# DeepakSridhar/fgdm

Hardware: AMD Instinct MI355X
Metric: 512x512 images/sec @ 50 DDIM steps, seg-ControlNet+CFG (higher is better)
Workload: dtype f16

## Files before the change

fgdm_amd/csrc/common.h:

```cpp
#pragma once
#include <hip/hip_runtime.h>
#include <stdint.h>

typedef _Float16 half_t;
typedef _Float16 h8 __attribute__((ext_vector_type(8)));
typedef _Float16 h4 __attribute__((ext_vector_type(4)));
typedef _Float16 h2 __attribute__((ext_vector_type(2)));
typedef float f32x16 __attribute__((ext_vector_type(16)));
typedef float f32x4 __attribute__((ext_vector_type(4)));

__device__ __forceinline__ float gelu_f(float x) {
    const float z = fminf(fabsf(x), 6.0f);
    float p = -4.7132482596e-04f;
    p = __builtin_fmaf(p, z, 7.0652551839e-03f);
    p = __builtin_fmaf(p, z, -5.1762067461e-02f);
    p = __builtin_fmaf(p, z, -4.6008771426e-01f);
    p = __builtin_fmaf(p, z, -1.1507295505e+00f);
    p = __builtin_fmaf(p, z, -4.8959157159e-05f - 1.0f);
    const float t = __builtin_amdgcn_exp2f(p);
    return __builtin_fmaf(fabsf(x), 0.5f - t, 0.5f * x);
}

typedef float f32x2 __attribute__((ext_vector_type(2)));
__device__ __forceinline__ f32x2 gelu2_f(f32x2 x) {
    const f32x2 ax = {fabsf(x[0]), fabsf(x[1])};
    const f32x2 z = {fminf(ax[0], 6.0f), fminf(ax[1], 6.0f)};
    auto c = [](float k) { return f32x2{k, k}; };
    f32x2 p = c(-4.7132482596e-04f);
    p = __builtin_elementwise_fma(p, z, c(7.0652551839e-03f));
    p = __builtin_elementwise_fma(p, z, c(-5.1762067461e-02f));
    p = __builtin_elementwise_fma(p, z, c(-4.6008771426e-01f));
    p = __builtin_elementwise_fma(p, z, c(-1.1507295505e+00f));
    p = __builtin_elementwise_fma(p, z, c(-4.8959157159e-05f - 1.0f));
    const f32x2 t = {__builtin_amdgcn_exp2f(p[0]), __builtin_amdgcn_exp2f(p[1])};
    return __builtin_elementwise_fma(ax, c(0.5f) - t, c(0.5f) * x);
}

__device__ __forceinline__ float silu_f(float x, float k = 1.0f) {
    return x * __builtin_amdgcn_rcpf(1.0f + __builtin_amdgcn_exp2f(-1.4426950408889634f * k * x));
}

#define FGDM_OK 0
#define FGDM_ERR_ARG -1
#define FGDM_ERR_HIP -2
#define FGDM_ERR_STATE -3
#define FGDM_ERR_NOMEM -4

enum IgemmMode { IG_LINEAR = 0, IG_CONV3 = 1, IG_CONV3_S2 = 2, IG_CONV3_UP2 = 3, IG_CONV3_S2_BR = 4 };
enum IgemmAct { ACT_NONE = 0, ACT_SILU = 1, ACT_RELU = 2, ACT_GEGLU = 3, ACT_QGELU = 4  };
enum IgemmOut { OUT_F16 = 0, OUT_F32 = 1, OUT_F32_NCHW = 2, OUT_F16_T = 3 };

struct IgemmArgs {
    const half_t* A0;
    const half_t* A1;
    const half_t* Wt;
    const float* bias;
    const float* rowvec;
    const half_t* resid;
    void* out;
    const half_t* zero;
    int C0, C1;
    int B, H, W;
    int Ho, Wo;
    int M, N;
    int K;
    int mode, act, out_kind;
    int ld_out, ld_res;
    int rv_stride;
    int rows_per_sample;
    float scale;
    int force_cfg;
    int splitk;
    float* ws;
    int debug;
    const float* ln_stats;
    const float* ln_u;
    int ln_slots;
    float ln_eps;
    float* stats_out;
    void* out2;
    int split_n, out_kind2, ld_out2;
};

int igemm_launch(const IgemmArgs& a, hipStream_t s);
void igemm_set_force_cfg(int cfg);
void igemm_set_twin_layers(bool on);
void igemm_set_pair_hint(int mult);
int igemm2_launch(const IgemmArgs& a, int cfg, hipStream_t s);
int igemm_stats_slots(const IgemmArgs& a);
int row_stats_slots(int C);
int row_stats_launch(const half_t* x, int rows, int C, float* stats , hipStream_t s);
int igemm_splitk_factor(const IgemmArgs& a);
int igemm_splitk_reduce(const IgemmArgs& a, hipStream_t s);
size_t igemm_npad(int n);

#define GN_PIX_PER_CHUNK 256
void groupnorm_set_group(bool on);
int groupnorm_launch(const half_t* x0, int C0, const half_t* x1, int C1, int B, int HW,
                     const float* gamma, const float* beta, float eps, int silu,
                     half_t* out, float* ws , hipStream_t s);
size_t groupnorm_ws_floats(int B, int HW);
int layernorm_launch(const half_t* x, int rows, int C, const float* gamma, const float* beta, float eps,
                     half_t* out, hipStream_t s);

int attention_launch(const half_t* Q, int ldq, const half_t* K, int ldk, const half_t* Vt, int ldvt,
                     half_t* O, int ldo, int B, int H, int T, int Tk, int d, int q_prescaled, hipStream_t s);
int attention_last_kernel();

int nchw_f32_to_nhwc_f16(const float* x, half_t* y, int B, int C, int HW, int Cpad, hipStream_t s);
int pack_xcat(const float* x, const half_t* cc, half_t* y, int B, int Bc, int Cc, int HW, int Cpad, hipStream_t s);
int f32_to_f16(const float* x, half_t* y, size_t n, hipStream_t s);
int silu_f32_to_f16(const float* x, half_t* y, size_t n, hipStream_t s);
int nhwc_f16_to_nchw_f32(const half_t* x, float* y, int B, int C, int HW, hipStream_t s);
int im2col3x3(const half_t* x, half_t* A, int B, int H, int W, int C, int stride, int Kpad, hipStream_t s);
int avgpool2(const half_t* x, half_t* y, int B, int H, int W, int C, hipStream_t s);
int add_f16(const half_t* a, const half_t* b, half_t* y, size_t n, hipStream_t s);
int add_f16_to_f32(const float* a, const half_t* b, float* y, size_t n, hipStream_t s);
int timestep_embed(const int64_t* t, const float* t_float, half_t* y, int B, int dim, int rows_pad, hipStream_t s);
int vae_prequant(const float* z, const float* wb, float scale, half_t* y, int B, int HW, hipStream_t s);
int vae_moments(const float* h, const float* wb, float* moments, int B, int HW, hipStream_t s);
int posterior_sample(const float* moments, const float* noise, float scale, float* z, int B, int zc, int HW, hipStream_t s);
int softmax_rows(const float* S, half_t* P, int rows, int cols, hipStream_t s);
int image_to_u8(const float* x, uint8_t* y, int B, int C, int HW, int mode, hipStream_t s);
int resize_linear_u8(const uint8_t* src, uint8_t* dst, int B, int H, int W, int C, int Ho, int Wo, hipStream_t s);
int u8_to_hint(const uint8_t* src, float* dst, int B, int HW, int C, hipStream_t s);
int embed_tokens(const int64_t* ids, const float* tok, const float* pos, float* out, int rows, int T, int W, int vocab,
                 hipStream_t s);
int layernorm32_launch(const float* x, int rows, int C, const float* gamma, const float* beta, float eps, half_t* out16,
                       float* out32, hipStream_t s);
int f16_to_f32(const half_t* x, float* y, size_t n, hipStream_t s);
int small_attention_launch(const half_t* qkv, int ld, int koff, int voff, half_t* out, int ldo, int B, int heads, int T,
                           int d, int causal, hipStream_t s);
int transpose_pad_keys(const half_t* v, half_t* vt, int B, int Tk, int C, int Tkpad, hipStream_t s);
int ddim_step(const float* x, const float* e_cond, const float* e_uncond, float cfg_scale,
              float a_t, float a_prev, float sigma_t, float sqrt_one_minus_at, const float* noise,
              float* x_prev, float* pred_x0, float* e_out, size_t n, hipStream_t s);
int plms_combine(const float* e_t, const float* e1, const float* e2, const float* e3, int order,
                 float* e_prime, size_t n, hipStream_t s);
int axpby(const float* a, float ca, const float* b, float cb, float* y, size_t n, hipStream_t s);
int mask_blend(const float* a, const float* b, const float* m, float* y, size_t n, hipStream_t s);
int ancestral_step(const float* x, const float* eps, float sqrt_recip, float sqrt_recipm1, float coef1, float coef2,
                   float std, const float* noise, float* out, size_t n, hipStream_t s);

struct PatchGeom { int B, C, H, W, kh, kw, sh, sw, Ly, Lx; };
int patch_plan(int H, int W, int kh, int kw, int sh, int sw, bool must_cover, int* Ly, int* Lx);
int unfold_crops(const float* x, float* out , const PatchGeom& g, int l0, int n, hipStream_t s);
int fold_accumulate(const float* o, const float* w_pix, const float* w_tie, float* acc, const PatchGeom& g, int l0, int n,
                    hipStream_t s);
int fold_finish(const float* acc, const float* w_pix, const float* w_tie, float* out, const PatchGeom& g, hipStream_t s);
int repeat_words(const void* src, void* dst , size_t words , int reps, hipStream_t s);

#define HIP_TRY(expr) do { hipError_t _e = (expr); if (_e != hipSuccess) return FGDM_ERR_HIP; } while (0)

template <auto Kernel>
int fgdm_dyn_lds(int bytes) {
    constexpr int MAXDEV = 64;
    static bool set[MAXDEV] = {};
    int dev = -1;
    if (hipGetDevice(&dev) != hipSuccess || dev < 0 || dev >= MAXDEV) return FGDM_ERR_HIP;
    if (!set[dev]) {
        HIP_TRY(hipFuncSetAttribute((const void*)Kernel, hipFuncAttributeMaxDynamicSharedMemorySize, bytes));
        set[dev] = true;
    }
    return FGDM_OK;
}

#include <functional>
#define FGDM_MAX_GROUP 5
bool fgdm_recording();
void fgdm_record(std::function<int(hipStream_t)> run);
#define FGDM_GROUP_BLOB sizeof(IgemmArgs)
typedef int (*FgdmGroupFn)(const void* const* args, int n, unsigned grid_x, hipStream_t s);
void fgdm_record(std::function<int(hipStream_t)> run, const void* key, FgdmGroupFn group, const void* args, size_t nbytes,
                 unsigned grid_x, unsigned long long shape);
#define FGDM_LAUNCH(kernel, grid, block, smem, stream, ...)                                                                  \
    do {                                                                                                                     \
        if (fgdm_recording()) {                                                                                              \
// ... 9 lines not shown
```

fgdm_amd/csrc/engine.hip:

```cpp
#include "engine_shared.h"
#include "knobs.h"
#include "replay.h"

#include <algorithm>
#include <array>
#include <cmath>
#include <cstdlib>
#include <cstdio>
#include <cstring>
#include <map>
#include <memory>
#include <string>
#include <unordered_map>
#include <vector>

namespace {

struct Arena {
    struct Blk { char* p; size_t sz; bool free; };
    std::vector<std::vector<Blk>> slabs;
    std::vector<char*> bases;
    size_t slab_bytes = (size_t)4 << 30;
    size_t in_use = 0, peak = 0;
    bool scoped = false;
    std::vector<void*> live;
    void begin_scope() { scoped = true; live.clear(); }
    void end_scope(bool failed) {
        if (failed) { std::vector<void*> l; l.swap(live); scoped = false; for (void* p : l) release(p); }
        scoped = false;
        live.clear();
    }

    ~Arena() { for (char* b : bases) (void)hipFree(b); }
    void* alloc(size_t bytes) {
        bytes = (bytes + 255) & ~(size_t)255;
        if (bytes == 0) bytes = 256;
        for (auto& s : slabs)
            for (size_t i = 0; i < s.size(); ++i)
                if (s[i].free && s[i].sz >= bytes) {
                    if (s[i].sz > bytes) {
                        Blk rest{s[i].p + bytes, s[i].sz - bytes, true};
                        s[i].sz = bytes;
                        s.insert(s.begin() + i + 1, rest);
                    }
                    s[i].free = false;
                    in_use += bytes;
                    peak = std::max(peak, in_use);
                    if (scoped) live.push_back(s[i].p);
                    return s[i].p;
                }
        const size_t sz = std::max(slab_bytes, bytes);
        char* base = nullptr;
        if (hipMalloc(&base, sz) != hipSuccess) return nullptr;
        bases.push_back(base);
        slabs.push_back({Blk{base, sz, true}});
        return alloc(bytes);
    }
    void release(void* p) {
        if (!p) return;
        if (scoped) { auto it = std::find(live.begin(), live.end(), p); if (it != live.end()) { *it = live.back(); live.pop_back(); } }
        for (auto& s : slabs)
            for (size_t i = 0; i < s.size(); ++i)
                if (s[i].p == p && !s[i].free) {
                    s[i].free = true;
                    in_use -= s[i].sz;
                    if (i + 1 < s.size() && s[i + 1].free) { s[i].sz += s[i + 1].sz; s.erase(s.begin() + i + 1); }
                    if (i > 0 && s[i - 1].free) { s[i - 1].sz += s[i].sz; s.erase(s.begin() + i); }
                    return;
                }
    }
};

struct Tensor {
    half_t* p = nullptr;
    int B = 0, H = 0, W = 0, C = 0;
    size_t numel() const { return (size_t)B * H * W * C; }
    int rows() const { return B * H * W; }
};

struct ParamSlot {
    std::vector<int64_t> shape;
    std::vector<float> host;
    bool loaded = false;
    size_t numel() const { size_t n = 1; for (auto d : shape) n *= (size_t)d; return n; }
};

struct GemmW {
    half_t* w = nullptr;
    float* bias = nullptr;
    int N = 0, K = 0;
    bool im2col = false;
    int cin_pad = 0;
    int k_real = 0;
    float* ln_u = nullptr;
    float ln_eps = 1e-5f;
};
struct NormW { float* g = nullptr; float* b = nullptr; int C = 0; };

enum LType { L_CONV, L_RES, L_ATTN, L_DOWN, L_UP };
struct Layer {
    LType type = L_CONV;
    int cin = 0, cout = 0, heads = 0;
    bool down = false;
    std::string pre;
    GemmW conv;
    NormW gn1, gn2; GemmW c1, c2, skip; int emb_off = 0;
    NormW gn, ln1, ln2, ln3;
    GemmW pin, pout, qkv1, o1, q2, k2, v2, o2, ffp, ffo;
};
typedef std::vector<Layer> Block;

struct AdapterBlk { int ic = 0, oc = 0; bool down = false; std::string pre; GemmW in_conv, b1, b2; };

struct Net {
    std::string prefix;
    bool control = false;
    GemmW time0, time2, emb_all;
    int emb_total = 0;
    std::vector<Block> input, output;
    Block middle;
    NormW out_gn; GemmW out_conv;
    bool has_adapter = false;
    GemmW ad_conv_in; std::vector<AdapterBlk> ad_body;
    std::vector<GemmW> xad_conv_in; std::vector<std::vector<AdapterBlk>> xad_body;
    Tensor xad_sum[4]; bool xad_valid = false;
    bool time_adapter = false; Block tad_body;
    std::vector<GemmW> zero_convs; GemmW mid_out;
    std::vector<int> zero_ch;
    GemmW hint_convs[8];
    Tensor guided;
};

struct VRes { int cin = 0, cout = 0; std::string pre; NormW n1, n2; GemmW c1, c2, nin; };
struct VLevel { std::vector<VRes> blocks; bool up = false; std::string up_pre; GemmW upconv; };
struct VAttn { std::string pre; NormW norm; GemmW q, k, v, o; };
struct VDown { std::vector<VRes> blocks; bool down = false; std::string down_pre; GemmW downconv; };
struct VEnc {
    bool on = false;
    GemmW conv_in, conv_out;
    std::vector<VDown> levels;
    VRes mid1, mid2;
    VAttn attn;
    NormW norm_out;
    float* qc = nullptr;
};
struct Vae {
    bool on = false, packed = false;
    std::string prefix;
    int top = 0, factor = 1;
    GemmW conv_in, conv_out;
    VRes mid1, mid2;
    VAttn attn;
    std::vector<VLevel> levels;
    NormW norm_out;
    float* pq = nullptr;
    VEnc enc;
};

struct ClipLayer { std::string pre; NormW ln1, ln2; GemmW qkv, o, fc1, fc2; };
struct Clip {
    bool on = false, packed = false;
    std::string prefix;
    float* tok = nullptr;
    float* pos = nullptr;
    std::vector<ClipLayer> layers;
    NormW final_ln;
};

enum ProfClass { PC_IGEMM = 0, PC_ATTN = 1, PC_NORM = 2, PC_ELEM = 3, PC_COUNT = 4 };
struct Prof final : LaunchTimer {
    bool on = false;
    std::vector<hipEvent_t> pool;
    size_t used = 0;
    struct Rec { int cls; size_t e0, e1; double w; char tag[56]; };
    std::vector<Rec> recs;
    double work[PC_COUNT] = {0, 0, 0, 0};
    double bytes[PC_COUNT] = {0, 0, 0, 0};
    hipEvent_t get() {
        if (used == pool.size()) { hipEvent_t e; if (hipEventCreate(&e) != hipSuccess) return nullptr; pool.push_back(e); }
        return pool[used++];
    }
    int stride = 1;
    long counter = 0;
    bool armed = false;
    void begin(int cls, hipStream_t s, double w, const char* tag = "", double nbytes = 0.0) override {
        if (fgdm_recording()) {
            if (on) fgdm_record_bracket_begin(cls, w, nbytes, tag);
            return;
        }
        armed = false;
        if (!on || (counter++ % stride) != 0) return;
        armed = true;
        hipEvent_t e = get();
        if (!e) return;
        (void)hipEventRecord(e, s);
        Rec r{cls, used - 1, 0, w, {0}};
        snprintf(r.tag, sizeof(r.tag), "%s", tag);
        recs.push_back(r);
        work[cls] += w;
        bytes[cls] += nbytes;
    }
    void end(hipStream_t s) override {
        if (fgdm_recording()) {
            if (on) fgdm_record_bracket_end();
            return;
        }
        if (!on || !armed || recs.empty()) return;
        armed = false;
        hipEvent_t e = get();
        if (!e) return;
        (void)hipEventRecord(e, s);
        recs.back().e1 = used - 1;
    }
};

}

#define CHK0(x) do { int _rc0 = (x); if (_rc0 != FGDM_OK) return _rc0; } while (0)
struct fgdm_engine {
    fgdm_config cfg{};
    int device = -1;
    bool device_ready = false, finalized = false;
    std::string err;
    std::vector<std::string> order;
    std::unordered_map<std::string, ParamSlot> params;
    Net unet;
    std::vector<Net> cns;
    Vae vae;
    Clip clip;
    struct CtxKV { Tensor k, vt; };
    std::unordered_map<const Layer*, CtxKV> ctx_cache;
    int ctx_B = 0, ctx_T = 0;
    int ctx_tokens = 77;
    Tensor ccat;
    Arena arena;
    half_t* zero = nullptr;
    std::unordered_map<std::string, std::vector<void*>> weight_allocs;
    std::unordered_map<std::string, bool> comp_dirty, comp_packed;
    std::string cur_comp;
    bool ln_fold = true;
    hipStream_t s = nullptr;
    std::vector<std::unique_ptr<Arena>> cn_arena;
    Arena* ar = &arena;
    hipStream_t s2 = nullptr;
    hipEvent_t ev_fork = nullptr, ev_join = nullptr;
    bool twin_streams = false;
    bool pair_launch = true;
    int group_max = FGDM_MAX_GROUP;
    bool gn_group = true;
    ReplayStats replay_stats;
    struct Deferred { const GemmW* w; Tensor src; int idx; float scale; Arena* owner; };
    Prof prof;

    int fail(int code, const std::string& m) { err = m; return code; }

    void reg(const std::string& name, std::vector<int64_t> shape) {
        order.push_back(name);
        params[name].shape = std::move(shape);
    }
    void reg_wb(const std::string& pre, std::vector<int64_t> wshape) {
        const int64_t n = wshape[0];
        reg(pre + ".weight", std::move(wshape));
        reg(pre + ".bias", {n});
    }
    void reg_res(const std::string& p, int cin, int cout, int temb) {
        reg_wb(p + "in_layers.0", {cin});
        reg_wb(p + "in_layers.2", {cout, cin, 3, 3});
        reg_wb(p + "emb_layers.1", {cout, temb});
        reg_wb(p + "out_layers.0", {cout});
        reg_wb(p + "out_layers.3", {cout, cout, 3, 3});
        if (cin != cout) reg_wb(p + "skip_connection", {cout, cin, 1, 1});
    }
    void reg_attn(const std::string& p, int ch, int ctx) {
        reg_wb(p + "norm", {ch});
        reg_wb(p + "proj_in", {ch, ch, 1, 1});
        const std::string t = p + "transformer_blocks.0.";
        reg(t + "attn1.to_q.weight", {ch, ch});
        reg(t + "attn1.to_k.weight", {ch, ch});
        reg(t + "attn1.to_v.weight", {ch, ch});
        reg_wb(t + "attn1.to_out.0", {ch, ch});
        reg_wb(t + "ff.net.0.proj", {8 * ch, ch});
        reg_wb(t + "ff.net.2", {ch, 4 * ch});
        reg(t + "attn2.to_q.weight", {ch, ch});
        reg(t + "attn2.to_k.weight", {ch, ctx});
        reg(t + "attn2.to_v.weight", {ch, ctx});
        reg_wb(t + "attn2.to_out.0", {ch, ch});
        reg_wb(t + "norm1", {ch});
        reg_wb(t + "norm2", {ch});
        reg_wb(t + "norm3", {ch});
        reg_wb(p + "proj_out", {ch, ch, 1, 1});
    }
    void reg_block(const std::string& pre, Block& blk, int temb, int ctx) {
        for (size_t j = 0; j < blk.size(); ++j) {
            Layer& l = blk[j];
            l.pre = pre + std::to_string(j) + ".";
            switch (l.type) {
                case L_CONV: reg_wb(l.pre.substr(0, l.pre.size() - 1), {l.cout, l.cin, 3, 3}); break;
                case L_RES: reg_res(l.pre, l.cin, l.cout, temb); break;
                case L_ATTN: reg_attn(l.pre, l.cin, ctx); break;
                case L_DOWN: reg_wb(l.pre + "op", {l.cin, l.cin, 3, 3}); break;
                case L_UP: reg_wb(l.pre + "conv", {l.cin, l.cin, 3, 3}); break;
            }
        }
    }
    static Layer mk(LType t, int cin, int cout, int heads = 0) {
        Layer l; l.type = t; l.cin = cin; l.cout = cout; l.heads = heads; return l;
    }
    bool in_ares(int ds) const {
        for (int i = 0; i < cfg.n_attention_resolutions; ++i) if (cfg.attention_resolutions[i] == ds) return true;
        return false;
    }
    void build_net(Net& n, const std::string& prefix, bool control, int adapter_kind) {
        const bool adapter = adapter_kind == 1;
        n.prefix = prefix; n.control = control; n.has_adapter = adapter_kind != 0; n.time_adapter = adapter_kind == 2;
        const int mc = cfg.model_channels, temb = 4 * mc, ctx = cfg.context_dim, heads = cfg.num_heads;
        reg_wb(prefix + "time_embed.0", {temb, mc});
        reg_wb(prefix + "time_embed.2", {temb, temb});
        if (adapter) {
            static const int chs[4] = {320, 640, 1280, 1280};
            const std::string ap = prefix + "adapter.";
            for (int i = 0; i < 4; ++i)
                for (int j = 0; j < 2; ++j) {
                    AdapterBlk b;
// ... 268 lines not shown
        if (rc != FGDM_OK) return rc;
        comp_packed[comp] = true;
        comp_dirty[comp] = false;
        return FGDM_OK;
    }
    int pack_rows(GemmW& g, const std::vector<std::pair<const float*, int>>& srcs, int K_src, int K,
                  const std::vector<int>& kmap, const std::vector<const float*>& biases, bool geglu,
                  const std::vector<float>& src_scale = {}, const float* ln_gamma = nullptr, const float* ln_beta = nullptr) {
        int N = 0;
        for (auto& s : srcs) N += s.second;
        const size_t npad = igemm_npad(N);
        std::vector<half_t> w(npad * (size_t)K, (half_t)0);
        std::vector<float> bias(npad, 0.f), lnu(ln_gamma ? npad : 0, 0.f);
        std::vector<const float*> rowp(N);
        std::vector<float> bflat(N, 0.f), rscale(N, 1.f);
        int r = 0;
        for (size_t si = 0; si < srcs.size(); ++si)
            for (int i = 0; i < srcs[si].second; ++i, ++r) {
                rowp[r] = srcs[si].first + (size_t)i * K_src;
                if (si < biases.size() && biases[si]) bflat[r] = biases[si][i];
                if (si < src_scale.size()) rscale[r] = src_scale[si];
            }
        for (int pr = 0; pr < N; ++pr) {
            int sr = pr;
            if (geglu) {
                const int grp = pr >> 6, within = pr & 63;
                sr = within < 32 ? grp * 32 + within : N / 2 + grp * 32 + (within - 32);
            }
            const float* src = rowp[sr];
            const float rs = rscale[sr];
            half_t* dst = w.data() + (size_t)pr * K;
            if (ln_gamma) {
                double us = 0.0, cs = 0.0;
                for (int k = 0; k < K; ++k) {
                    dst[k] = (half_t)(src[k] * rs * ln_gamma[k]);
                    us += (double)(float)dst[k];
                    cs += (double)ln_beta[k] * (double)(src[k] * rs);
                }
                lnu[pr] = (float)us;
                bias[pr] = (float)((double)(bflat[sr] * rs) + cs);
                continue;
            }
            if (kmap.empty()) for (int k = 0; k < K; ++k) dst[k] = (half_t)(src[k] * rs);
            else for (int k = 0; k < K; ++k) if (kmap[k] >= 0) dst[k] = (half_t)(src[kmap[k]] * rs);
            bias[pr] = bflat[sr] * rs;
        }
        g.N = N; g.K = K; g.k_real = K_src;
        g.w = upload(w);
        g.bias = upload(bias);
        g.ln_u = ln_gamma ? upload(lnu) : nullptr;
        if (ln_gamma && !kmap.empty()) return fail(FGDM_ERR_ARG, "LayerNorm fold: plain Linear weights only");
        return (g.w && g.bias && (!ln_gamma || g.ln_u)) ? FGDM_OK : fail(FGDM_ERR_NOMEM, "hipMalloc failed while packing weights");
    }
    int pack_linear(GemmW& g, const std::string& pre, bool has_bias, bool geglu = false, float wscale = 1.f,
                    const std::string& ln = std::string()) {
        const ParamSlot* w = slot(pre + ".weight");
        if (!w) return FGDM_ERR_STATE;
        const ParamSlot *lg = nullptr, *lb = nullptr;
        if (!ln.empty()) { lg = slot(ln + ".weight"); lb = slot(ln + ".bias"); if (!lg || !lb) return FGDM_ERR_STATE; }
        const ParamSlot* b = has_bias ? slot(pre + ".bias") : nullptr;
        if (has_bias && !b) return FGDM_ERR_STATE;
        const int N = (int)w->shape[0], K = (int)(w->numel() / w->shape[0]);
        if (K & 63) return fail(FGDM_ERR_ARG, "linear K not a multiple of 64: " + pre);
        if (lg && (int)lg->numel() != K) return fail(FGDM_ERR_ARG, "LayerNorm fold: width mismatch for " + pre);
        return pack_rows(g, {{w->host.data(), N}}, K, K, {}, {b ? b->host.data() : nullptr}, geglu, {wscale},
                         lg ? lg->host.data() : nullptr, lb ? lb->host.data() : nullptr);
    }
    int pack_stack(GemmW& g, const std::vector<std::string>& pres, bool has_bias, const std::vector<float>& scales = {},
                   const std::string& ln = std::string()) {
        const ParamSlot *lg = nullptr, *lb = nullptr;
        if (!ln.empty()) { lg = slot(ln + ".weight"); lb = slot(ln + ".bias"); if (!lg || !lb) return FGDM_ERR_STATE; }
        std::vector<std::pair<const float*, int>> srcs;
        std::vector<const float*> biases;
        int K = 0;
        for (auto& pre : pres) {
            const ParamSlot* w = slot(pre + ".weight");
            if (!w) return FGDM_ERR_STATE;
            K = (int)(w->numel() / w->shape[0]);
            srcs.push_back({w->host.data(), (int)w->shape[0]});
            if (has_bias) { const ParamSlot* b = slot(pre + ".bias"); if (!b) return FGDM_ERR_STATE; biases.push_back(b->host.data()); }
        }
        return pack_rows(g, srcs, K, K, {}, biases, false, scales, lg ? lg->host.data() : nullptr, lb ? lb->host.data() : nullptr);
    }
    int pack_conv3(GemmW& g, const std::string& pre) {
        const ParamSlot* w = slot(pre + ".weight");
        const ParamSlot* b = slot(pre + ".bias");
        if (!w || !b) return FGDM_ERR_STATE;
        const int N = (int)w->shape[0], Cin = (int)w->shape[1];
        int cp = 0;
        const std::vector<int> kmap = conv3_kmap(Cin, &cp);
        g.im2col = (Cin % 64) != 0;
        g.cin_pad = cp;
        return pack_rows(g, {{w->host.data(), N}}, Cin * 9, (int)kmap.size(), kmap, {b->host.data()}, false);
    }
    int pack_norm(NormW& n, const std::string& pre) {
        const ParamSlot* w = slot(pre + ".weight");
        const ParamSlot* b = slot(pre + ".bias");
        if (!w || !b) return FGDM_ERR_STATE;
        n.C = (int)w->shape[0];
        n.g = upload(w->host);
        n.b = upload(b->host);
        return (n.g && n.b) ? FGDM_OK : fail(FGDM_ERR_NOMEM, "hipMalloc failed");
    }
#define CHK(x) do { int _rc = (x); if (_rc != FGDM_OK) return _rc; } while (0)
    int pack_block(Block& blk) {
        for (Layer& l : blk) {
            const std::string& p = l.pre;
            switch (l.type) {
                case L_CONV: CHK(pack_conv3(l.conv, p.substr(0, p.size() - 1))); break;
                case L_DOWN: CHK(pack_conv3(l.conv, p + "op")); break;
                case L_UP: CHK(pack_conv3(l.conv, p + "conv")); break;
                case L_RES:
                    CHK(pack_norm(l.gn1, p + "in_layers.0"));
                    CHK(pack_conv3(l.c1, p + "in_layers.2"));
                    CHK(pack_norm(l.gn2, p + "out_layers.0"));
                    CHK(pack_conv3(l.c2, p + "out_layers.3"));
                    if (l.cin != l.cout) CHK(pack_linear(l.skip, p + "skip_connection", true));
                    break;
                case L_ATTN: {
                    const std::string t = p + "transformer_blocks.0.";
                    CHK(pack_norm(l.gn, p + "norm"));
                    CHK(pack_linear(l.pin, p + "proj_in", true));
                    CHK(pack_linear(l.pout, p + "proj_out", true));
                    const float qs = 1.4426950408889634f / sqrtf((float)(l.cin / l.heads));
                    const std::string n1 = ln_fold ? t + "norm1" : "", n2 = ln_fold ? t + "norm2" : "", n3 = ln_fold ? t + "norm3" : "";
                    if (!ln_fold) { CHK(pack_norm(l.ln1, t + "norm1")); CHK(pack_norm(l.ln2, t + "norm2")); CHK(pack_norm(l.ln3, t + "norm3")); }
                    CHK(pack_stack(l.qkv1, {t + "attn1.to_q", t + "attn1.to_k", t + "attn1.to_v"}, false, {qs, 1.f, 1.f}, n1));
                    CHK(pack_linear(l.o1, t + "attn1.to_out.0", true));
                    CHK(pack_linear(l.q2, t + "attn2.to_q", false, false, qs, n2));
                    CHK(pack_linear(l.k2, t + "attn2.to_k", false));
                    CHK(pack_linear(l.v2, t + "attn2.to_v", false));
                    CHK(pack_linear(l.o2, t + "attn2.to_out.0", true));
                    CHK(pack_linear(l.ffp, t + "ff.net.0.proj", true, true, 1.f, n3));
                    CHK(pack_linear(l.ffo, t + "ff.net.2", true));
                    break;
                }
            }
        }
        return FGDM_OK;
    }
    int pack_net(Net& n) {
        CHK(pack_linear(n.time0, n.prefix + "time_embed.0", true));
        CHK(pack_linear(n.time2, n.prefix + "time_embed.2", true));
        std::vector<std::string> embs;
        int off = 0;
        auto collect = [&](Block& b) {
            for (Layer& l : b) if (l.type == L_RES) { l.emb_off = off; off += l.cout; embs.push_back(l.pre + "emb_layers.1"); }
        };
        for (auto& b : n.input) collect(b);
        collect(n.middle);
        for (auto& b : n.output) collect(b);
        collect(n.tad_body);
        n.emb_total = off;
        CHK(pack_stack(n.emb_all, embs, true));
        for (auto& b : n.input) CHK(pack_block(b));
        CHK(pack_block(n.middle));
        for (auto& b : n.output) CHK(pack_block(b));
        if (!n.control) {
            CHK(pack_norm(n.out_gn, n.prefix + "out.0"));
            CHK(pack_conv3(n.out_conv, n.prefix + "out.2"));
            if (n.time_adapter) CHK(pack_block(n.tad_body));
            if (n.has_adapter) {
                CHK(pack_conv3(n.ad_conv_in, n.prefix + "adapter.conv_in"));
                for (auto& b : n.ad_body) {
                    if (b.ic != b.oc) CHK(pack_linear(b.in_conv, b.pre + "in_conv", true));
                    CHK(pack_conv3(b.b1, b.pre + "block1"));
                    CHK(pack_linear(b.b2, b.pre + "block2", true));
                }
                for (size_t kk = 0; kk < n.xad_body.size(); ++kk) {
                    CHK(pack_conv3(n.xad_conv_in[kk], n.prefix + "adapters." + std::to_string(kk) + ".conv_in"));
                    for (auto& b : n.xad_body[kk]) {
                        if (b.ic != b.oc) CHK(pack_linear(b.in_conv, b.pre + "in_conv", true));
                        CHK(pack_conv3(b.b1, b.pre + "block1"));
                        CHK(pack_linear(b.b2, b.pre + "block2", true));
                    }
                }
            }
        } else {
            n.zero_convs.resize(n.input.size());
            for (size_t i = 0; i < n.input.size(); ++i)
                CHK(pack_linear(n.zero_convs[i], n.prefix + "zero_convs." + std::to_string(i) + ".0", true));
            CHK(pack_linear(n.mid_out, n.prefix + "middle_block_out.0", true));
            for (int k = 0; k < 8; ++k) CHK(pack_conv3(n.hint_convs[k], n.prefix + "input_hint_block." + std::to_string(2 * k)));
        }
        for (auto& name : order)
            if (name.compare(0, n.prefix.size(), n.prefix) == 0) { auto& ps = params[name]; std::vector<float>().swap(ps.host); }
        return FGDM_OK;
    }

    int pack_vres(VRes& r) {
        CHK(pack_norm(r.n1, r.pre + "norm1"));
        CHK(pack_conv3(r.c1, r.pre + "conv1"));
        CHK(pack_norm(r.n2, r.pre + "norm2"));
        CHK(pack_conv3(r.c2, r.pre + "conv2"));
        if (r.cin != r.cout) CHK(pack_linear(r.nin, r.pre + "nin_shortcut", true));
        return FGDM_OK;
    }
    int pack_vattn(VAttn& at) {
        CHK(pack_norm(at.norm, at.pre + "norm"));
        CHK(pack_linear(at.q, at.pre + "q", true));
        CHK(pack_linear(at.k, at.pre + "k", true));
        CHK(pack_linear(at.v, at.pre + "v", true));
        CHK(pack_linear(at.o, at.pre + "proj_out", true));
        return FGDM_OK;
    }
    int pack_pointwise(float** dst, const std::string& pre) {
        const ParamSlot* w = slot(pre + ".weight");
        const ParamSlot* b = slot(pre + ".bias");
        if (!w || !b) return FGDM_ERR_STATE;
        std::vector<float> wb(w->host);
        wb.insert(wb.end(), b->host.begin(), b->host.end());
        *dst = upload(wb);
        return *dst ? FGDM_OK : fail(FGDM_ERR_NOMEM, "hipMalloc failed");
    }
    int pack_vae_encoder() {
        VEnc& en = vae.enc;
        const std::string d = vae.prefix + "encoder.";
        CHK(pack_conv3(en.conv_in, d + "conv_in"));
        for (auto& lv : en.levels) {
            for (auto& r : lv.blocks) CHK(pack_vres(r));
            if (lv.down) CHK(pack_conv3(lv.downconv, lv.down_pre));
        }
        CHK(pack_vres(en.mid1));
        CHK(pack_vattn(en.attn));
        CHK(pack_vres(en.mid2));
        CHK(pack_norm(en.norm_out, d + "norm_out"));
        CHK(pack_conv3(en.conv_out, d + "conv_out"));
        return pack_pointwise(&en.qc, vae.prefix + "quant_conv");
    }
    int pack_vae() {
        Vae& v = vae;
        if (v.enc.on) CHK(pack_vae_encoder());
        const std::string d = v.prefix + "decoder.";
        CHK(pack_conv3(v.conv_in, d + "conv_in"));
        CHK(pack_vres(v.mid1));
        CHK(pack_vattn(v.attn));
        CHK(pack_vres(v.mid2));
        for (auto& lv : v.levels) {
            for (auto& r : lv.blocks) CHK(pack_vres(r));
            if (lv.up) CHK(pack_conv3(lv.upconv, lv.up_pre));
        }
        CHK(pack_norm(v.norm_out, d + "norm_out"));
        CHK(pack_conv3(v.conv_out, d + "conv_out"));
        CHK(pack_pointwise(&v.pq, v.prefix + "post_quant_conv"));
        for (auto& name : order)
            if (name.compare(0, v.prefix.size(), v.prefix) == 0) { auto& ps = params[name]; std::vector<float>().swap(ps.host); }
        v.packed = true;
        return FGDM_OK;
    }

    int pack_clip() {
        Clip& c = clip;
        auto up32 = [&](const std::string& name, float** dst) -> int {
            const ParamSlot* w = slot(name);
            if (!w) return FGDM_ERR_STATE;
            *dst = upload(w->host);
            return *dst ? FGDM_OK : fail(FGDM_ERR_NOMEM, "hipMalloc failed");
        };
        CHK(up32(c.prefix + "embeddings.token_embedding.weight", &c.tok));
        CHK(up32(c.prefix + "embeddings.position_embedding.weight", &c.pos));
        for (ClipLayer& l : c.layers) {
            CHK(pack_norm(l.ln1, l.pre + "layer_norm1"));
            CHK(pack_norm(l.ln2, l.pre + "layer_norm2"));
            CHK(pack_stack(l.qkv, {l.pre + "self_attn.q_proj", l.pre + "self_attn.k_proj", l.pre + "self_attn.v_proj"}, true));
            CHK(pack_linear(l.o, l.pre + "self_attn.out_proj", true));
            CHK(pack_linear(l.fc1, l.pre + "mlp.fc1", true));
            CHK(pack_linear(l.fc2, l.pre + "mlp.fc2", true));
        }
        CHK(pack_norm(c.final_ln, c.prefix + "final_layer_norm"));
        for (auto& name : order)
            if (name.compare(0, c.prefix.size(), c.prefix) == 0) { auto& ps = params[name]; std::vector<float>().swap(ps.host); }
        c.packed = true;
        return FGDM_OK;
    }

    int dcopy(void* dst, const void* src, size_t bytes) {
        auto run = [=](hipStream_t rs) -> int { return hipMemcpyAsync(dst, src, bytes, hipMemcpyDeviceToDevice, rs) == hipSuccess ? FGDM_OK : FGDM_ERR_HIP; };
        if (!fgdm_recording()) return run(s);
        fgdm_record(run);
        return FGDM_OK;
    }
    int dzero(void* dst, size_t bytes) {
        auto run = [=](hipStream_t rs) -> int { return hipMemsetAsync(dst, 0, bytes, rs) == hipSuccess ? FGDM_OK : FGDM_ERR_HIP; };
        if (!fgdm_recording()) return run(s);
        fgdm_record(run);
        return FGDM_OK;
    }
    Tensor talloc(int B, int H, int W, int C) {
        Tensor t; t.B = B; t.H = H; t.W = W; t.C = C;
        t.p = (half_t*)ar->alloc(t.numel() * sizeof(half_t));
        return t;
    }
    void tfree(Tensor& t) { ar->release(t.p); t.p = nullptr; }

    struct LnStats { float* p = nullptr; int slots = 0; };
    struct Epi {
        const LnStats* ln = nullptr;
        LnStats* stats = nullptr;
        int act = ACT_NONE;
        const float* rowvec = nullptr; int rv_stride = 0;
        const half_t* resid = nullptr; int ld_res = 0;
        float scale = 1.f;
        int out_kind = OUT_F16;
        void* out = nullptr;
        int ld_out = 0;
        void* out2 = nullptr; int out_kind2 = OUT_F16, ld_out2 = 0, split_n = 0;
        int rps = 0;
    };
    int gemm(const GemmW& w, int mode, const Tensor& x0, const Tensor* x1, int Ho, int Wo, const Epi& e, Tensor* out) {
        IgemmArgs a{};
        a.A0 = x0.p; a.C0 = x0.C;
        a.A1 = x1 ? x1->p : nullptr; a.C1 = x1 ? x1->C : 0;
        a.Wt = w.w; a.bias = w.bias;
        a.rowvec = e.rowvec; a.rv_stride = e.rv_stride;
        a.resid = e.resid; a.ld_res = e.ld_res;
        a.zero = zero;
        a.B = x0.B; a.H = x0.H; a.W = x0.W; a.Ho = Ho; a.Wo = Wo;
        a.M = x0.B * Ho * Wo;
        a.N = w.N;
        a.K = w.K;
        a.mode = mode; a.act = e.act; a.out_kind = e.out_kind;
        const int nout = e.act == ACT_GEGLU ? w.N / 2 : w.N;
        a.out = e.out ? e.out : (void*)out->p;
        a.ld_out = e.ld_out ? e.ld_out : nout;
        a.rows_per_sample = e.rps ? e.rps : Ho * Wo;
        a.scale = e.scale;
        a.out2 = e.out2; a.out_kind2 = e.out_kind2; a.ld_out2 = e.ld_out2; a.split_n = e.split_n;
        const int taps = mode == IG_LINEAR ? 1 : 9;
        if (taps * (a.C0 + a.C1) != a.K) return fail(FGDM_ERR_ARG, "gemm: K mismatch");
        if (!a.out) return fail(FGDM_ERR_NOMEM, "gemm: null output (workspace exhausted?)");
        char tag[56] = "";
        if (prof.on) snprintf(tag, sizeof(tag), "igemm M%d N%d K%d mode%d act%d out%d l%ds%dr%dv%d", a.M, a.N, a.K, a.mode, a.act, a.out_kind,
                              e.ln ? 1 : 0, e.stats ? 1 : 0, e.resid ? 1 : 0, e.rowvec ? 1 : 0);
        a.splitk = igemm_splitk_factor(a);
        if (a.splitk > 1) {
            a.ws = (float*)ar->alloc((size_t)a.splitk * a.M * a.N * sizeof(float));
            if (!a.ws) return fail(FGDM_ERR_NOMEM, "workspace (split-K partials)");
        }
        if (e.ln) {
            if (!w.ln_u || !e.ln->p || a.splitk > 1) return fail(FGDM_ERR_STATE, "gemm: LayerNorm fold without folded weights / statistics");
            a.ln_stats = e.ln->p; a.ln_slots = e.ln->slots; a.ln_u = w.ln_u; a.ln_eps = w.ln_eps;
        } else if (w.ln_u) {
            return fail(FGDM_ERR_STATE, "gemm: these weights have a LayerNorm folded in; statistics are required");
        }
        if (e.stats) {
            e.stats->slots = igemm_stats_slots(a);
            e.stats->p = (float*)ar->alloc((size_t)a.M * std::max(e.stats->slots, row_stats_slots(nout)) * 2 * sizeof(float));
            if (!e.stats->p) return fail(FGDM_ERR_NOMEM, "workspace (LayerNorm statistics)");
            if (e.stats->slots) a.stats_out = e.stats->p;
        }
        double nbytes = 0.0;
        if (prof.on) {
            const double in_b = 2.0 * ((double)x0.numel() + (x1 ? (double)x1->numel() : 0.0));
            const double out_b = (double)a.M * nout * (e.out_kind == OUT_F16 || e.out_kind == OUT_F16_T ? 2.0 : 4.0);
            nbytes = in_b + 2.0 * (double)w.N * w.K + out_b + (e.resid ? 2.0 * (double)a.M * nout : 0.0);
        }
        prof.begin(PC_IGEMM, s, 2.0 * (double)a.M * (double)w.N * (double)w.k_real, tag, nbytes);
        int rc = igemm_launch(a, s);
        prof.end(s);
        if (a.ws) ar->release(a.ws);
        if (rc == FGDM_OK && e.stats && e.stats->slots == 0) {
            if (a.out_kind != OUT_F16 || a.ld_out != nout) return fail(FGDM_ERR_ARG, "gemm: row statistics need a dense fp16 output");
            e.stats->slots = row_stats_slots(nout);
            prof.begin(PC_NORM, s, 2.0 * (double)a.M * nout, "row_stats");
            rc = row_stats_launch((const half_t*)a.out, a.M, nout, e.stats->p, s);
            prof.end(s);
        }
        return rc == FGDM_OK ? rc : fail(rc, "igemm launch failed");
    }
    int conv3(const GemmW& w, const Tensor& x, const Tensor* x1, int stride, bool up, Epi e, Tensor* out) {
        int Ho = x.H, Wo = x.W, mode = IG_CONV3;
        if (up) { Ho *= 2; Wo *= 2; mode = IG_CONV3_UP2; }
        else if (stride == 2) { Ho = (x.H - 1) / 2 + 1; Wo = (x.W - 1) / 2 + 1; mode = IG_CONV3_S2; }
        else if (stride == FGDM_STRIDE2_PAD_BR) { Ho = (x.H - 2) / 2 + 1; Wo = (x.W - 2) / 2 + 1; mode = IG_CONV3_S2_BR; }
        const bool own_out = (e.out == nullptr);
        if (own_out) { *out = talloc(x.B, Ho, Wo, w.N); if (!out->p) return fail(FGDM_ERR_NOMEM, "workspace"); }
        if (!w.im2col) return gemm(w, mode, x, x1, Ho, Wo, e, out);
        if (up || x1 || x.C != w.cin_pad || stride == FGDM_STRIDE2_PAD_BR) return fail(FGDM_ERR_ARG, "im2col conv path: unsupported combination");
        Tensor A = talloc(1, 1, x.B * Ho * Wo, w.K);
        if (!A.p) return fail(FGDM_ERR_NOMEM, "workspace (im2col)");
        prof.begin(PC_ELEM, s, 2.0 * (double)A.numel() + 2.0 * (double)x.numel());
        bool in_gemm = false;
        const int rc = im2col_conv(x.p, A.p, x.B, x.H, x.W, x.C, stride, w.K, s, [&]() { prof.end(s); },
            [&](half_t* Ap, int Bv, int Hv, int Wv, int Kv, int rps) {
                in_gemm = true;
                Tensor Av; Av.p = Ap; Av.B = Bv; Av.H = Hv; Av.W = Wv; Av.C = Kv;
                if (!e.rps) e.rps = rps;
                return gemm(w, IG_LINEAR, Av, nullptr, Hv, Wv, e, out);
            });
        if (rc != FGDM_OK && !in_gemm) return fail(rc, "im2col failed");
        tfree(A);
        return rc;
    }
    int linear(const GemmW& w, const Tensor& x, Epi e, Tensor* out, const Tensor* x1 = nullptr) {
        if (!e.out) { *out = talloc(x.B, x.H, x.W, e.act == ACT_GEGLU ? w.N / 2 : w.N); if (!out->p) return fail(FGDM_ERR_NOMEM, "workspace"); }
        return gemm(w, IG_LINEAR, x, x1, x.H, x.W, e, out);
    }
    int gnorm(const NormW& n, const Tensor& x, const Tensor* x1, float eps, bool silu, Tensor* out) {
        const int C = x.C + (x1 ? x1->C : 0);
        *out = talloc(x.B, x.H, x.W, C);
        float* ws = (float*)ar->alloc(groupnorm_ws_floats(x.B, x.H * x.W) * sizeof(float));
        if (!out->p || !ws) return fail(FGDM_ERR_NOMEM, "workspace");
        char tag[56] = "";
        if (prof.on) snprintf(tag, sizeof(tag), "groupnorm B%d HW%d C%d", x.B, x.H * x.W, C);
        prof.begin(PC_NORM, s, 4.0 * (double)out->numel(), tag);
        const int rc = groupnorm_launch(x.p, x.C, x1 ? x1->p : nullptr, x1 ? x1->C : 0, x.B, x.H * x.W, n.g, n.b, eps,
                                        silu ? 1 : 0, out->p, ws, s);
        prof.end(s);
        ar->release(ws);
        return rc == FGDM_OK ? rc : fail(rc, "groupnorm launch failed");
    }
    int lnorm(const NormW& n, const Tensor& x, Tensor* out) {
        *out = talloc(x.B, x.H, x.W, x.C);
        if (!out->p) return fail(FGDM_ERR_NOMEM, "workspace");
        char tag[56] = "";
        if (prof.on) snprintf(tag, sizeof(tag), "layernorm rows%d C%d", x.rows(), x.C);
        prof.begin(PC_NORM, s, 4.0 * (double)out->numel(), tag);
        const int rc = layernorm_launch(x.p, x.rows(), x.C, n.g, n.b, 1e-5f, out->p, s);
        prof.end(s);
        return rc == FGDM_OK ? rc : fail(rc, "layernorm launch failed");
    }

    struct EmbCtx { const float* emb_all; int stride; };

    int res_fwd(const Layer& l, const Tensor& x, const Tensor* x1, const EmbCtx& ec, Tensor* out) {
        Tensor g1, h, g2, sk, xp;
        CHK(gnorm(l.gn1, x, x1, 1e-5f, true, &g1));
        const Tensor* xs = &x;
        if (l.down) {
            if (x1) return fail(FGDM_ERR_ARG, "down ResBlock with a concatenated input");
            Tensor gp = talloc(x.B, x.H / 2, x.W / 2, x.C);
            xp = talloc(x.B, x.H / 2, x.W / 2, x.C);
            if (!gp.p || !xp.p) return fail(FGDM_ERR_NOMEM, "workspace");
            if (avgpool2(g1.p, gp.p, x.B, x.H, x.W, x.C, s) != FGDM_OK || avgpool2(x.p, xp.p, x.B, x.H, x.W, x.C, s) != FGDM_OK)
                return fail(FGDM_ERR_ARG, "avgpool2: latent size must be divisible by 8 for the adapter");
            tfree(g1);
            g1 = gp;
            xs = &xp;
        }
        Epi e1; e1.rowvec = ec.emb_all + l.emb_off; e1.rv_stride = ec.stride;
        CHK(conv3(l.c1, g1, nullptr, 1, false, e1, &h));
        tfree(g1);
        CHK(gnorm(l.gn2, h, nullptr, 1e-5f, true, &g2));
        tfree(h);
        Epi e2;
        if (l.cin != l.cout) {
            CHK(linear(l.skip, *xs, Epi{}, &sk, x1));
            e2.resid = sk.p; e2.ld_res = sk.C;
        } else {
            e2.resid = xs->p; e2.ld_res = xs->C;
        }
        CHK(conv3(l.c2, g2, nullptr, 1, false, e2, out));
        tfree(g2);
        if (sk.p) tfree(sk);
        if (xp.p) tfree(xp);
        return FGDM_OK;
    }
// ... 792 lines not shown
        if ((Hh & 7) || (Wh & 7) || B <= 0) return fail(FGDM_ERR_ARG, "hint size must be a multiple of 8");
        Net& n = cns[cn];
        const int mc = cfg.model_channels, Hl = Hh / 8, Wl = Wh / 8;
        if (n.guided.p && (n.guided.B != B || n.guided.H != Hl || n.guided.W != Wl)) { (void)hipFree(n.guided.p); n.guided.p = nullptr; }
        if (!n.guided.p) {
            n.guided.B = B; n.guided.H = Hl; n.guided.W = Wl; n.guided.C = mc;
            if (hipMalloc(&n.guided.p, n.guided.numel() * sizeof(half_t)) != hipSuccess) return fail(FGDM_ERR_NOMEM, "hipMalloc (hint cache)");
        }
        const int hc = n.hint_convs[0].cin_pad;
        const int chunk = std::max(1, std::min(B, (int)(((size_t)512 << 20) / ((size_t)Hh * Wh * 192 * 2 + 1))));
        for (int b0 = 0; b0 < B; b0 += chunk) {
            const int nb = std::min(chunk, B - b0);
            Tensor cur = talloc(nb, Hh, Wh, hc);
            if (!cur.p) return fail(FGDM_ERR_NOMEM, "workspace");
            if (nchw_f32_to_nhwc_f16(hint + (size_t)b0 * cfg.hint_channels * Hh * Wh, cur.p, nb, cfg.hint_channels, Hh * Wh, hc, s) != FGDM_OK)
                return fail(FGDM_ERR_HIP, "layout kernel");
            for (int k = 0; k < 8; ++k) {
                const int stride = (k == 2 || k == 4 || k == 6) ? 2 : 1;
                Epi e;
                e.act = k < 7 ? ACT_SILU : ACT_NONE;
                Tensor nxt;
                if (k == 7) { e.out = n.guided.p + (size_t)b0 * Hl * Wl * mc; e.ld_out = mc; }
                CHK(conv3(n.hint_convs[k], cur, nullptr, stride, false, e, k == 7 ? nullptr : &nxt));
                tfree(cur);
                cur = nxt;
            }
        }
        return FGDM_OK;
    }

    void drop_concat() { if (ccat.p) (void)hipFree(ccat.p); ccat = Tensor{}; }
    int set_concat(const float* cc, int B, int Cc, int H, int W) {
        if (cfg.in_channels == 4) return fail(FGDM_ERR_ARG, "fgdm_set_concat: this engine's UNet takes x alone (in_channels = 4)");
        if (!cc) { drop_concat(); return FGDM_OK; }
        if (Cc != cfg.in_channels - 4) {
            drop_concat();
            return fail(FGDM_ERR_ARG, "fgdm_set_concat: c_concat must have in_channels - 4 = " + std::to_string(cfg.in_channels - 4) + " channels");
        }
        if (B <= 0 || H <= 0 || W <= 0) { drop_concat(); return fail(FGDM_ERR_ARG, "bad shape"); }
        if (ccat.p && (ccat.B != B || ccat.H != H || ccat.W != W)) drop_concat();
        if (!ccat.p) {
            ccat.B = B; ccat.H = H; ccat.W = W; ccat.C = Cc;
            if (hipMalloc(&ccat.p, ccat.numel() * sizeof(half_t)) != hipSuccess) { ccat = Tensor{}; return fail(FGDM_ERR_NOMEM, "hipMalloc (c_concat cache)"); }
        }
        if (nchw_f32_to_nhwc_f16(cc, ccat.p, B, Cc, H * W, Cc, s) != FGDM_OK) return fail(FGDM_ERR_HIP, "layout kernel");
        return FGDM_OK;
    }
};

static std::string g_create_err;

static int make_desc(const fgdm_config* cfg, fgdm_engine** out) {
    fgdm_engine* e = new fgdm_engine();
    e->cfg = *cfg;
    const int rc = e->build();
    if (rc != FGDM_OK) { g_create_err = "unsupported configuration: " + e->err; delete e; return rc; }
    *out = e;
    return FGDM_OK;
}

template <typename F> static int scoped_call(fgdm_engine* e, void* stream, F f) {
    e->s = as_stream(stream);
    e->ar = &e->arena;
    e->arena.begin_scope();
    for (auto& a : e->cn_arena) a->begin_scope();
    const int rc = f();
    e->s = as_stream(stream);
    e->ar = &e->arena;
    if (rc != FGDM_OK && e->s2) (void)hipStreamSynchronize(e->s2);
    e->arena.end_scope(rc != FGDM_OK);
    for (auto& a : e->cn_arena) a->end_scope(rc != FGDM_OK);
    return rc;
}

extern "C" {

int fgdm_create(const fgdm_config* cfg, int device, fgdm_engine** out) {
    if (!cfg || !out) return FGDM_ERR_ARG;
    fgdm_engine* e = nullptr;
    int rc = make_desc(cfg, &e);
    if (rc != FGDM_OK) return rc;
    e->device = device;
    e->ln_fold = knob_on(KNOB_LN_FOLD);
    rc = e->ensure_device();
    if (rc != FGDM_OK) {
        g_create_err = e->err + " [" + hipGetErrorString(hipGetLastError()) + "]";
        delete e;
        return rc;
    }
    e->twin_streams = knob_on(KNOB_TWIN_STREAMS);
    e->pair_launch = knob_on(KNOB_PAIR_LAUNCH);
    e->group_max = std::max(2, std::min(FGDM_MAX_GROUP, knob_int(KNOB_GROUP_MAX)));
    e->gn_group = knob_on(KNOB_GN_GROUP);
    if (e->twin_streams && !e->cns.empty()) {
        if (hipStreamCreateWithFlags(&e->s2, hipStreamNonBlocking) != hipSuccess ||
            hipEventCreateWithFlags(&e->ev_fork, hipEventDisableTiming) != hipSuccess ||
            hipEventCreateWithFlags(&e->ev_join, hipEventDisableTiming) != hipSuccess) {
            g_create_err = "second stream could not be created";
            delete e;
            return FGDM_ERR_HIP;
        }
    }
    for (size_t c = 0; c < e->cns.size(); ++c) {
        e->cn_arena.emplace_back(new Arena());
        if (e->cfg.workspace_bytes > 0) e->cn_arena.back()->slab_bytes = (size_t)e->cfg.workspace_bytes;
    }
    *out = e;
    return FGDM_OK;
}

void fgdm_destroy(fgdm_engine* e) {
    if (!e) return;
    for (hipEvent_t ev : e->prof.pool) (void)hipEventDestroy(ev);
    for (auto& kv : e->weight_allocs) for (void* p : kv.second) (void)hipFree(p);
    if (e->zero) (void)hipFree(e->zero);
    for (auto& n : e->cns) if (n.guided.p) (void)hipFree(n.guided.p);
    e->drop_concat();
    e->drop_context();
    e->drop_adapter_conds();
    if (knob_text(KNOB_PAIR_DEBUG) && e->replay_stats.replayed)
        fprintf(stderr, "[fgdm] grouped twin launches: %ld of %ld replayed launches were fused (%ld problems)\n", e->replay_stats.fused, e->replay_stats.replayed, e->replay_stats.problems);
    if (e->s2) { (void)hipStreamSynchronize(e->s2); (void)hipStreamDestroy(e->s2); }
    if (e->ev_fork) (void)hipEventDestroy(e->ev_fork);
    if (e->ev_join) (void)hipEventDestroy(e->ev_join);
    delete e;
}

const char* fgdm_last_error(const fgdm_engine* e) { return e ? e->err.c_str() : g_create_err.c_str(); }

static fgdm_engine* g_desc = nullptr;
static fgdm_config g_desc_cfg;
static fgdm_engine* desc_for(const fgdm_config* cfg) {
    if (g_desc && memcmp(&g_desc_cfg, cfg, sizeof(*cfg)) == 0) return g_desc;
    if (g_desc) { delete g_desc; g_desc = nullptr; }
    if (make_desc(cfg, &g_desc) != FGDM_OK) return nullptr;
    g_desc_cfg = *cfg;
    return g_desc;
}
int fgdm_param_count(const fgdm_config* cfg) {
    if (!cfg) return FGDM_ERR_ARG;
    fgdm_engine* d = desc_for(cfg);
    return d ? (int)d->order.size() : FGDM_ERR_ARG;
}
int fgdm_param_info(const fgdm_config* cfg, int index, char* name, int name_cap, int64_t* shape, int* ndim) {
    if (!cfg || !name || !shape || !ndim) return FGDM_ERR_ARG;
    fgdm_engine* d = desc_for(cfg);
    if (!d || index < 0 || index >= (int)d->order.size()) return FGDM_ERR_ARG;
    const std::string& n = d->order[index];
    if ((int)n.size() + 1 > name_cap) return FGDM_ERR_ARG;
    memcpy(name, n.c_str(), n.size() + 1);
    const auto& sh = d->params[n].shape;
    *ndim = (int)sh.size();
    for (size_t i = 0; i < sh.size(); ++i) shape[i] = sh[i];
    return FGDM_OK;
}

int fgdm_load_tensor(fgdm_engine* e, const char* key, const void* data, int dtype, const int64_t* shape, int ndim) {
    if (!e || !key || !data || !shape) return FGDM_ERR_ARG;
    auto it = e->params.find(key);
    if (it == e->params.end()) return e->fail(FGDM_ERR_ARG, std::string("unknown parameter key: ") + key);
    ParamSlot& ps = it->second;
    if ((int)ps.shape.size() != ndim) return e->fail(FGDM_ERR_ARG, std::string("rank mismatch for ") + key);
    for (int i = 0; i < ndim; ++i)
        if (ps.shape[i] != shape[i]) return e->fail(FGDM_ERR_ARG, std::string("shape mismatch for ") + key);
    const size_t n = ps.numel();
    ps.host.resize(n);
// ... 332 lines not shown
```

fgdm_amd/csrc/engine_shared.h:

```cpp
#pragma once
#include "common.h"
#include "../../include/fgdm.h"

#include <algorithm>
#include <cmath>
#include <vector>

static int roundup(int x, int m) { return (x + m - 1) / m * m; }

static std::vector<int> conv3_kmap(int Cin, int* cin_pad) {
    const bool implicit = (Cin % 64) == 0;
    const int cp = implicit ? Cin : roundup(Cin, Cin % 8 == 0 ? 8 : 4);
    const int K = implicit ? 9 * Cin : roundup(9 * cp, 64);
    std::vector<int> kmap(K, -1);
    for (int tap = 0; tap < 9; ++tap)
        for (int c = 0; c < Cin; ++c) {
            const int k = implicit ? ((c >> 6) * 9 + tap) * 64 + (c & 63) : tap * cp + c;
            kmap[k] = c * 9 + tap;
        }
    *cin_pad = cp;
    return kmap;
}

template <class After, class Gemm>
static int im2col_conv(const half_t* x, half_t* A, int B, int H, int W, int C, int stride, int K, hipStream_t s,
                       After&& after_im2col, Gemm&& gemm_rows) {
    const int Ho = (H - 1) / stride + 1, Wo = (W - 1) / stride + 1;
    const int rc = im2col3x3(x, A, B, H, W, C, stride, K, s);
    after_im2col();
    if (rc != FGDM_OK) return rc;
    return gemm_rows(A, B, Ho, Wo, K, Ho * Wo);
}

template <class Gemm>
static int vattn_core(const half_t* q, const half_t* k, const half_t* vt, half_t* out, float* S, half_t* P, int B, int T, int C,
                      hipStream_t s, bool* softmax_failed, Gemm&& gemm_rows) {
    *softmax_failed = false;
    for (int b = 0; b < B; ++b) {
        int rc = gemm_rows(k + (size_t)b * T * C, T, C, q + (size_t)b * T * C, T, OUT_F32, (void*)S, T, 1.0f / sqrtf((float)C));
        if (rc != FGDM_OK) return rc;
        if (softmax_rows(S, P, T, T, s) != FGDM_OK) { *softmax_failed = true; return FGDM_ERR_HIP; }
        rc = gemm_rows(vt + (size_t)b * C * T, C, T, P, T, OUT_F16, (void*)(out + (size_t)b * T * C), C, 1.0f);
        if (rc != FGDM_OK) return rc;
    }
    return FGDM_OK;
}

static hipStream_t as_stream(void* p) { return (hipStream_t)p; }

struct TmpDev {
    std::vector<void*> ptrs;
    ~TmpDev() { for (void* p : ptrs) (void)hipFree(p); }
    template <typename T> T* alloc(size_t n) {
        T* d = nullptr;
        if (hipMalloc(&d, n * sizeof(T)) != hipSuccess) return nullptr;
        ptrs.push_back(d);
        return d;
    }
    template <typename T> T* up(const std::vector<T>& h) {
        T* d = alloc<T>(std::max<size_t>(h.size(), 256 / sizeof(T)));
        if (d) (void)hipMemcpy(d, h.data(), h.size() * sizeof(T), hipMemcpyHostToDevice);
        return d;
    }
};
static int plan_splitk(IgemmArgs& a, TmpDev& tmp) {
    a.splitk = igemm_splitk_factor(a);
    if (a.splitk > 1 && !(a.ws = tmp.alloc<float>((size_t)a.splitk * a.M * a.N))) return FGDM_ERR_NOMEM;
    return FGDM_OK;
}
inline half_t* g_zero_page() {
    static half_t* z = nullptr;
    if (!z) { if (hipMalloc(&z, 4096) != hipSuccess) return nullptr; (void)hipMemset(z, 0, 4096); }
    return z;
}
```

fgdm_amd/csrc/igemm.hip:

```cpp
#include "common.h"
#include "knobs.h"
#include <algorithm>

#define LDS_AS __attribute__((address_space(3)))
#define GLB_AS __attribute__((address_space(1)))

__device__ __forceinline__ void glds16(const void* g, void* lds_wave_base) {
    __builtin_amdgcn_global_load_lds((const GLB_AS void*)g, (LDS_AS void*)lds_wave_base, 16, 0, 0);
}


__device__ __forceinline__ float ln_scale(float acc, float mean, float rstd, float u) {
    float t, w;
    asm("v_fma_f32 %0, %1, %2, %3" : "=v"(t) : "v"(-mean), "v"(u), "v"(acc));
    asm("v_mul_f32 %0, %1, %2" : "=v"(w) : "v"(rstd), "v"(t));
    return w;
}

template <int BM, int BN, int WM, int WN>
__global__ __launch_bounds__(WM * WN * 64) void igemm_kernel(const IgemmArgs a) {
    constexpr int T = WM * WN * 64;
    constexpr int TM = BM / WM, TN = BN / WN;
    constexpr int MI = TM / 32, NI = TN / 32;
    constexpr int A_IT = BM * 8 / T, B_IT = BN * 8 / T;
    constexpr int A_BYTES = BM * 128, STAGE = (BM + BN) * 128;
    static_assert(A_IT >= 1 && B_IT >= 1, "tile too small for the thread count");
    extern __shared__ __attribute__((aligned(16))) char smem[];

    const int tid = threadIdx.x, lane = tid & 63;
    const int wave = __builtin_amdgcn_readfirstlane(tid >> 6);
    const int wm = wave / WN, wn = wave % WN;

    const int ntn = (a.N + BN - 1) / BN;
    const int nb = gridDim.x;
    int logical;
    {
        const int bid = blockIdx.x, xcd = bid & 7, q = nb >> 3, r = nb & 7;
        logical = (xcd < r ? xcd * (q + 1) : r * (q + 1) + (xcd - r) * q) + (bid >> 3);
    }
    const int m0 = (logical / ntn) * BM, n0 = (logical % ntn) * BN;

    const int Ctot = a.C0 + a.C1;
    const int cpt = Ctot >> 6;
    const int nk = a.K >> 6;

    int a_pix[A_IT], a_yx[A_IT], a_co[A_IT];
#pragma unroll
    for (int j = 0; j < A_IT; ++j) {
        const int q = j * T + tid, r = q >> 3, s = q & 7;
        a_co[j] = ((s ^ ((r >> 1) & 7)) << 3);
        const int m = m0 + r;
        a_pix[j] = -1;
        a_yx[j] = 0;
        if (m < a.M) {
            if (a.mode == IG_LINEAR) {
                a_pix[j] = m;
            } else {
                const int hw = a.Ho * a.Wo;
                const int b = m / hw, rem = m - b * hw;
                const int oy = rem / a.Wo, ox = rem - oy * a.Wo;
                a_pix[j] = b * a.H * a.W;
                a_yx[j] = (oy << 16) | ox;
            }
        }
    }
    int b_off[B_IT];
#pragma unroll
    for (int j = 0; j < B_IT; ++j) {
        const int q = j * T + tid, r = q >> 3, s = q & 7;
        b_off[j] = (n0 + r) * a.K + ((s ^ ((r >> 1) & 7)) << 3);
    }

    auto stage = [&](int kt, int tap, int cc, int buf) {
        char* As = smem + buf * STAGE;
        char* Bs = As + A_BYTES;
        const half_t* src = a.A0;
        int Cs = a.C0, co = cc << 6;
        if (co >= a.C0) { src = a.A1; Cs = a.C1; co -= a.C0; }
        const int ky = tap / 3, kx = tap - ky * 3;
#pragma unroll
        for (int j = 0; j < A_IT; ++j) {
            const half_t* p = a.zero;
            if (a_pix[j] >= 0) {
                if (a.mode == IG_LINEAR) {
                    p = src + (size_t)a_pix[j] * Cs + co + a_co[j];
                } else {
                    const int oy = a_yx[j] >> 16, ox = a_yx[j] & 0xffff;
                    int iy, ix;
                    bool ok;
                    if (a.mode == IG_CONV3) {
                        iy = oy + ky - 1; ix = ox + kx - 1;
                        ok = (unsigned)iy < (unsigned)a.H && (unsigned)ix < (unsigned)a.W;
                    } else if (a.mode == IG_CONV3_S2) {
                        iy = 2 * oy + ky - 1; ix = 2 * ox + kx - 1;
                        ok = (unsigned)iy < (unsigned)a.H && (unsigned)ix < (unsigned)a.W;
                    } else if (a.mode == IG_CONV3_S2_BR) {
                        iy = 2 * oy + ky; ix = 2 * ox + kx;
                        ok = iy < a.H && ix < a.W;
                    } else {
                        const int uy = oy + ky - 1, ux = ox + kx - 1;
                        ok = (unsigned)uy < (unsigned)(2 * a.H) && (unsigned)ux < (unsigned)(2 * a.W);
                        iy = uy >> 1; ix = ux >> 1;
                    }
                    if (ok) p = src + (size_t)(a_pix[j] + iy * a.W + ix) * Cs + co + a_co[j];
                }
            }
            glds16(p, As + (j * T + wave * 64) * 16);
        }
#pragma unroll
        for (int j = 0; j < B_IT; ++j)
            glds16(a.Wt + (size_t)b_off[j] + ((size_t)kt << 6), Bs + (j * T + wave * 64) * 16);
    };

    f32x16 acc[MI][NI];
#pragma unroll
    for (int i = 0; i < MI; ++i)
#pragma unroll
        for (int j = 0; j < NI; ++j)
#pragma unroll
            for (int r = 0; r < 16; ++r) acc[i][j][r] = 0.f;

    const int lrow = lane & 31, lh = lane >> 5, swz = (lrow >> 1) & 7;
    int koff[4];
#pragma unroll
    for (int ks = 0; ks < 4; ++ks) koff[ks] = lrow * 128 + (((ks * 2 + lh) ^ swz) << 4);

    int tap = 0, cc = 0;
    stage(0, 0, 0, 0);
    for (int kt = 0; kt < nk; ++kt) {
        asm volatile("s_waitcnt vmcnt(0)" ::: "memory");
        __syncthreads();
        if (kt + 1 < nk) {
            if (a.mode == IG_LINEAR) ++cc;
            else if (++tap == 9) { tap = 0; ++cc; }
            stage(kt + 1, tap, cc, (kt + 1) & 1);
        }
        const char* As = smem + (kt & 1) * STAGE + (wm * TM) * 128;
        const char* Bs = smem + (kt & 1) * STAGE + A_BYTES + (wn * TN) * 128;
#pragma unroll
        for (int ks = 0; ks < 4; ++ks) {
            h8 af[MI], bf[NI];
#pragma unroll
            for (int i = 0; i < MI; ++i) af[i] = *(const h8*)(As + i * 32 * 128 + koff[ks]);
#pragma unroll
            for (int j = 0; j < NI; ++j) bf[j] = *(const h8*)(Bs + j * 32 * 128 + koff[ks]);
#pragma unroll
            for (int i = 0; i < MI; ++i)
#pragma unroll
                for (int j = 0; j < NI; ++j)
                    acc[i][j] = __builtin_amdgcn_mfma_f32_32x32x16_f16(af[i], bf[j], acc[i][j], 0, 0, 0);
        }
    }

    if (a.ln_stats) {
#pragma unroll
        for (int i = 0; i < MI; ++i) {
            float sm[16], sq[16];
#pragma unroll
            for (int r = 0; r < 16; ++r) { sm[r] = 0.f; sq[r] = 0.f; }
            for (int p = 0; p < a.ln_slots; ++p) {
#pragma unroll
                for (int r = 0; r < 16; ++r) {
                    const int row = m0 + wm * TM + i * 32 + (r & 3) + 8 * (r >> 2) + 4 * (lane >> 5);
                    if (row < a.M) {
                        const float* sp = a.ln_stats + ((size_t)row * a.ln_slots + p) * 2;
                        sm[r] += sp[0]; sq[r] += sp[1];
                    }
                }
            }
#pragma unroll
            for (int r = 0; r < 16; ++r) {
                const double mu = (double)sm[r] / (double)a.C0;
                double var = (double)sq[r] / (double)a.C0 - mu * mu;
                if (var < 0.0) var = 0.0;
                sm[r] = (float)mu;
                sq[r] = (float)(1.0 / sqrt(var + (double)a.ln_eps));
            }
#pragma unroll
            for (int j = 0; j < NI; ++j) {
                const int pc = n0 + wn * TN + j * 32 + (lane & 31);
                const float un = pc < a.N ? a.ln_u[pc] : 0.f;
#pragma unroll
                for (int r = 0; r < 16; ++r) acc[i][j][r] = ln_scale(acc[i][j][r], sm[r], sq[r], un);
            }
        }
    }
    const int rps = a.rows_per_sample;
    const bool geglu = (a.act == ACT_GEGLU);
    const bool second = a.out2 && n0 >= a.split_n;
    void* const outp = second ? a.out2 : a.out;
    const int okind = second ? a.out_kind2 : a.out_kind, ldo = second ? a.ld_out2 : a.ld_out;
    const int ncol0 = second ? a.split_n : 0, nchan = (a.out2 ? (second ? a.N : a.split_n) : a.N) - ncol0;
#pragma unroll
    for (int i = 0; i < MI; ++i) {
#pragma unroll
        for (int j = 0; j < NI; ++j) {
            if (geglu && (j & 1)) continue;
            const int pcol = n0 + wn * TN + j * 32 + lrow;
            if (pcol >= a.N) continue;
            const float bias = a.bias ? a.bias[pcol] : 0.f;
            float gbias = 0.f;
            if (geglu) gbias = a.bias ? a.bias[pcol + 32] : 0.f;
            const int ocol = geglu ? ((pcol >> 6) << 5) + lrow : pcol - ncol0;
            float rvv[16];
#pragma unroll
            for (int r = 0; r < 16; ++r) {
                const int row = m0 + wm * TM + i * 32 + (r & 3) + 8 * (r >> 2) + 4 * lh;
                rvv[r] = (a.rowvec && row < a.M) ? a.rowvec[(size_t)(row / rps) * a.rv_stride + pcol] : 0.f;
            }
#pragma unroll
            for (int g = 0; g < 4; ++g) {
                const int row0 = m0 + wm * TM + i * 32 + 8 * g + 4 * lh;
                float v[4];
#pragma unroll
                for (int e = 0; e < 4; ++e) {
                    const int row = row0 + e;
                    float x = acc[i][j][g * 4 + e] + bias + rvv[g * 4 + e];
                    if (a.act == ACT_SILU) x = silu_f(x);
                    else if (a.act == ACT_RELU) x = fmaxf(x, 0.f);
                    else if (a.act == ACT_QGELU) x = silu_f(x, 1.702f);
                    else if (geglu) {
                        if constexpr (NI >= 2) x = x * gelu_f(acc[i][j | 1][g * 4 + e] + gbias);
                    }
                    v[e] = x * a.scale;
                }
                if (okind == OUT_F16) {
                    half_t* o = (half_t*)outp;
#pragma unroll
                    for (int e = 0; e < 4; ++e) {
                        const int row = row0 + e;
                        if (row < a.M) {
                            half_t x = (half_t)v[e];
                            if (a.resid) x = (half_t)((float)x + (float)a.resid[(size_t)row * a.ld_res + ocol]);
                            o[(size_t)row * ldo + ocol] = x;
                        }
                    }
                } else if (okind == OUT_F32) {
                    float* o = (float*)outp;
#pragma unroll
                    for (int e = 0; e < 4; ++e)
                        if (row0 + e < a.M) o[(size_t)(row0 + e) * ldo + ocol] = v[e];
                } else {
                    const bool vec = ((rps & 3) == 0) && (row0 + 3 < a.M);
                    if (vec) {
                        const int b = row0 / rps, t = row0 - b * rps;
                        const size_t off = ((size_t)b * nchan + ocol) * ldo + t;
                        if (okind == OUT_F16_T) {
                            h4 pk = {(half_t)v[0], (half_t)v[1], (half_t)v[2], (half_t)v[3]};
                            *(h4*)((half_t*)outp + off) = pk;
                        } else {
                            f32x4 pk = {v[0], v[1], v[2], v[3]};
                            *(f32x4*)((float*)outp + off) = pk;
                        }
                    } else {
#pragma unroll
                        for (int e = 0; e < 4; ++e) {
                            const int row = row0 + e;
                            if (row < a.M) {
                                const int b = row / rps, t = row - b * rps;
                                const size_t off = ((size_t)b * nchan + ocol) * ldo + t;
                                if (okind == OUT_F16_T) ((half_t*)outp)[off] = (half_t)v[e];
                                else ((float*)outp)[off] = v[e];
                            }
                        }
                    }
                }
            }
        }
    }
}

size_t igemm_npad(int n) { return (size_t)((n + 127) / 128) * 128; }

template <int BM, int BN, int WM, int WN>
static int launch_cfg(const IgemmArgs& a, hipStream_t s) {
    constexpr int smem = 2 * (BM + BN) * 128;
    constexpr auto k = igemm_kernel<BM, BN, WM, WN>;
    if (fgdm_dyn_lds<k>(smem) != FGDM_OK) return FGDM_ERR_HIP;
    const int ntm = (a.M + BM - 1) / BM, ntn = (a.N + BN - 1) / BN;
    FGDM_LAUNCH(k, dim3(ntm * ntn), dim3(WM * WN * 64), smem, s, a);
    return hipGetLastError() == hipSuccess ? FGDM_OK : FGDM_ERR_HIP;
}

static int g_force_cfg = 0;
void igemm_set_force_cfg(int cfg) { g_force_cfg = cfg; }
static thread_local int g_pair_mult = 1;
void igemm_set_pair_hint(int mult) { g_pair_mult = mult > 1 ? mult : 1; }

static int pick_force(const IgemmArgs& a) {
    int force = a.force_cfg ? a.force_cfg : g_force_cfg;
    if (a.act == ACT_QGELU) {
        if (force >= 4) force = 0;
        if (force == 0) return 0;
    }
    const bool small_tiles = knob_once(KNOB_IGEMM_SMALL_TILES) != 0;
    const bool other_widths = knob_once(KNOB_IGEMM_OTHER_WIDTHS) != 0;
    if (force == 0) {
        const bool geglu = a.act == ACT_GEGLU;
        if (!geglu && a.N % 320 == 0) {
            const long b256 = (long)((a.M + 255) / 256) * (a.N / 320);
            const long b128 = (long)((a.M + 127) / 128) * (a.N / 320);
            const bool small_m = knob_once(KNOB_IGEMM_SMALL_M) != 0;
            const bool lin64 = a.mode == IG_LINEAR && !(a.K & 31) && !(a.C0 & 31) && !(a.C1 & 31) && small_tiles;
            const long b64 = (long)((a.M + 63) / 64) * (a.N / 160);
            const long b256n = (long)((a.M + 255) / 256) * (a.N / 128);
            if (b256 * g_pair_mult >= 192) force = 4;
            else if (small_m && lin64 && a.K >= 2560 && !(a.N % 128) && !a.ln_stats && !a.stats_out && !a.out2 && b128 >= 96 && b128 * g_pair_mult < 192 &&
                     b64 >= 512 && b256n >= 144 && b256n <= 256) force = 10;
            else if (b128 >= 96 && !(small_m && lin64 && b128 * g_pair_mult < 192 && b64 >= 512)) force = 6;
            else if (lin64 && b64 >= 128) force = 11;
        } else if (geglu && a.N % 256 == 0 && (long)((a.M + 255) / 256) * (a.N / 256) >= 128) {
            force = 5;
        } else if (!geglu && !a.ln_stats && !(a.K & 31) && !(a.C0 & 31) && !(a.C1 & 31) && other_widths) {
            const long rows = (a.M + 255) / 256;
            if (a.N % 256 == 0 && rows * (a.N / 256) >= 192) force = 5;
            else if (a.N == 128 && rows >= 192) force = 10;
        }
    }
    return force;
}

int igemm_stats_slots(const IgemmArgs& a) {
    if (a.out_kind != OUT_F16 || a.act == ACT_GEGLU || a.splitk > 1 || (a.N % 320) || (a.K & 31) || (a.C0 & 31) || (a.C1 & 31)) return 0;
    const int f = pick_force(a);
    if (f < 4) return 0;
    const int tile = (f - 4) & 15;
    const bool stats64 = knob_once(KNOB_IGEMM_STATS64) != 0;
    return (tile == 0 || tile == 2 || tile == 3 || tile == 5 || (tile == 7 && stats64)) ? a.N / 160 : 0;
}

int igemm_launch(const IgemmArgs& a, hipStream_t s) {
    if (a.M <= 0 || a.N <= 0 || a.K <= 0 || (a.K & 63) || (a.C0 & 63) || (a.C1 & 63)) return FGDM_ERR_ARG;
    if (a.act == ACT_GEGLU && (a.N & 63)) return FGDM_ERR_ARG;
    if (a.ln_stats && (a.mode != IG_LINEAR || a.C1 || a.ln_slots <= 0 || !a.ln_u)) return FGDM_ERR_ARG;
    if (a.stats_out && igemm_stats_slots(a) == 0) return FGDM_ERR_ARG;
    if (a.out2 && (a.act == ACT_GEGLU || a.splitk > 1 || a.stats_out || a.split_n <= 0 || a.split_n >= a.N || (a.split_n % 640))) return FGDM_ERR_ARG;
    if (a.splitk > 1) {
        if (!a.ws || a.ln_stats) return FGDM_ERR_ARG;
        const bool fat = (long)((a.M + 255) / 256) * (a.N / 320) * a.splitk >= 192 && !(a.K & 31) && !(a.C0 & 31) && !(a.C1 & 31);
        const int rc = igemm2_launch(a, fat ? 0 : 2, s);
        return rc == FGDM_OK ? igemm_splitk_reduce(a, s) : rc;
    }
    int force = pick_force(a);
    const bool mfma32 = knob_once(KNOB_IGEMM_MFMA32) != 0;
    if (mfma32 && force >= 4 && force <= 6 && !a.force_cfg && !g_force_cfg) force += 3;
    if (force >= 4) return igemm2_launch(a, force - 4, s);
    struct Cfg { int bm, bn; float eff; int per_cu; };
    static const Cfg cfgs[] = {{128, 128, 1.00f, 2}, {128, 64, 0.80f, 3}, {64, 64, 0.62f, 4}};
    int best = 0;
    float best_cost = 1e30f;
    for (int i = 0; i < 3; ++i) {
        const Cfg& c = cfgs[i];
        const long nblk = (long)((a.M + c.bm - 1) / c.bm) * ((a.N + c.bn - 1) / c.bn);
        const long slots = 256L * c.per_cu;
        const float rounds = (float)((nblk + slots - 1) / slots);
        const long conc = std::min<long>(c.per_cu, (nblk + 255) / 256);
        const float cost = rounds * (float)conc * (float)(c.bm * c.bn) / c.eff;
        if (cost < best_cost) { best_cost = cost; best = i; }
    }
    if ((long)((a.M + 127) / 128) * ((a.N + 127) / 128) < 256) best = 2;
    if (a.act == ACT_GEGLU) best = 0;
    if (force >= 1 && force <= 3) best = force - 1;
    switch (best) {
        case 0: return launch_cfg<128, 128, 2, 2>(a, s);
        case 1: return launch_cfg<128, 64, 2, 2>(a, s);
        default: return launch_cfg<64, 64, 2, 2>(a, s);
    }
}
```

fgdm_amd/csrc/igemm2.hip:

```cpp
#include "common.h"
#include "knobs.h"
#include <algorithm>
#include <type_traits>

#pragma clang diagnostic ignored "-Winline-asm"
#define LDS_AS __attribute__((address_space(3)))
#define GLB_AS __attribute__((address_space(1)))

namespace {

__device__ __forceinline__ void glds16(const void* g, unsigned lds_wave_addr) {
    unsigned keep;
    asm volatile("s_mov_b32 %0, m0\n\ts_mov_b32 m0, %2\n\ts_nop 0\n\tglobal_load_lds_dwordx4 %1, off\n\ts_mov_b32 m0, %0"
                 : "=&s"(keep)
                 : "v"(g), "s"(lds_wave_addr)
                 : "memory", "m0");
}
__device__ __forceinline__ void glds16_m0(const void* g, unsigned lds_wave_addr) {
    asm volatile("s_mov_b32 m0, %1\n\ts_nop 0\n\tglobal_load_lds_dwordx4 %0, off" ::"v"(g), "s"(lds_wave_addr) : "memory", "m0");
}
__device__ __forceinline__ void glds16_sv(unsigned voff, const void* sbase, unsigned lds_wave_addr) {
    asm volatile("s_mov_b32 m0, %2\n\ts_nop 0\n\tglobal_load_lds_dwordx4 %0, %1" ::"v"(voff), "s"(sbase), "s"(lds_wave_addr) : "memory", "m0");
}
__device__ __forceinline__ unsigned lds_addr(const void* p) { return (unsigned)(size_t)(LDS_AS const void*)p; }
__device__ __forceinline__ float ln_scale(float acc, float mean, float rstd, float u) {
    float t, w;
    asm("v_fma_f32 %0, %1, %2, %3" : "=v"(t) : "v"(-mean), "v"(u), "v"(acc));
    asm("v_mul_f32 %0, %1, %2" : "=v"(w) : "v"(rstd), "v"(t));
    return w;
}

template <int N> __device__ __forceinline__ void wait_vmcnt() {
    asm volatile("s_waitcnt vmcnt(%0)" ::"n"(N) : "memory");
}

constexpr int BK = 32;
constexpr int ROWB = BK * 2;

constexpr int RV_MAX = 6;

template <int BM> constexpr int halo_px() { return BM == 256 ? 400 : 272; }
template <int BM, int BN, int STAGES, int PIPE> constexpr int ring_bytes() {
    return PIPE == 2 ? 2 * halo_px<BM>() * ROWB + STAGES * BN * ROWB : STAGES * (BM + BN) * ROWB;
}

template <int BM, int BN, int WM, int WN, int STAGES, bool CONV, bool GEGLU, bool SPLIT, int MS, bool LN, int PATH, int PIPE, bool ABL>
__device__ __forceinline__ void igemm2_body(const IgemmArgs& a) {
    constexpr int NW = WM * WN, T = NW * 64;
    constexpr int TM = BM / WM, TN = BN / WN;
    constexpr int MI = TM / MS, NI = TN / MS;
    constexpr int KS = MS == 32 ? 2 : 1;
    constexpr int AR = MS == 32 ? 16 : 4;
    typedef float acc_t __attribute__((ext_vector_type(AR)));
    auto swz_of = [](int r) { return MS == 32 ? ((r >> 2) & 3) : (((r >> 3) & 1) << 1); };
    constexpr int A_INSTR = BM * 4 / 64, B_INSTR = BN * 4 / 64;
    static_assert(A_INSTR % NW == 0, "A tile must split evenly over the waves");
    constexpr int LA = A_INSTR / NW, LB = (B_INSTR + NW - 1) / NW;
    constexpr int LPS = LA + LB;
    constexpr int STAGE_BYTES = (BM + BN) * ROWB;
    constexpr int A_BYTES = BM * ROWB;
    constexpr int RING_BYTES = ring_bytes<BM, BN, STAGES, PIPE>();
    static_assert(TM % 32 == 0 && TN % MS == 0, "wave tile: 32-pixel epilogue passes, MFMA-sized channel tiles");
    static_assert(!GEGLU || TN % 64 == 0, "GEGLU: whole 64-row [32 value | 32 gate] groups per wave");
    extern __shared__ __attribute__((aligned(16))) char smem[];

    const int tid = threadIdx.x, lane = tid & 63;
    const int wave = __builtin_amdgcn_readfirstlane(tid >> 6);
    const int wm = wave / WN, wn = wave % WN;

    const int ntn = (a.N + BN - 1) / BN;
    const int nb = gridDim.x;
    int logical;
    {
        const int bid = blockIdx.x, xcd = bid & 7, q = nb >> 3, r = nb & 7;
        logical = (xcd < r ? xcd * (q + 1) : r * (q + 1) + (xcd - r) * q) + (bid >> 3);
    }
    const int nsplit = SPLIT ? a.splitk : 1;
    int split = 0, m0, n0;
    if (SPLIT) {
        const int ntm = (a.M + BM - 1) / BM;
        const int row = logical % ntm, pair = logical / ntm;
        split = pair % nsplit; n0 = (pair / nsplit) * BN; m0 = row * BM;
    } else {
        m0 = (logical / ntn) * BM; n0 = (logical % ntn) * BN;
    }

    const int nk_all = a.K >> 5;
    const int per = (nk_all + nsplit - 1) / nsplit;
    const int k_begin = split * per;
    const int nk = max(0, min(per, nk_all - k_begin));

    int a_pix[LA], a_yx[LA], a_off[LA];
    int b_off[LB], b_lds[LB];
    const int br = (CONV && a.mode == IG_CONV3_S2_BR) ? 1 : 0;
    const int sy = (CONV && (a.mode == IG_CONV3_S2 || a.mode == IG_CONV3_S2_BR)) ? 2 : 1;
    const int up = (CONV && a.mode == IG_CONV3_UP2) ? 1 : 0;
#pragma unroll
    for (int i = 0; i < LA; ++i) {
        const int q = (wave + i * NW) * 64 + lane, r = q >> 2, s = q & 3;
        a_off[i] = (s ^ swz_of(r)) << 3;
        a_pix[i] = -1; a_yx[i] = 0;
        const int m = m0 + r;
        if (PIPE == 0 && m < a.M) {
            if (!CONV) {
                a_pix[i] = m;
            } else {
                const int hw = a.Ho * a.Wo;
                const int b = m / hw, rem = m - b * hw;
                const int oy = rem / a.Wo, ox = rem - oy * a.Wo;
                a_pix[i] = b * a.H * a.W;
                a_yx[i] = ((oy * sy + br) << 16) | (ox * sy + br);
            }
        }
    }
#pragma unroll
    for (int i = 0; i < LB; ++i) {
        int idx = wave + i * NW;
        if (idx >= B_INSTR) idx = B_INSTR - 1;
        const int q = idx * 64 + lane, r = q >> 2, s = q & 3;
        b_off[i] = (n0 + r) * a.K + ((s ^ swz_of(r)) << 3);
        b_lds[i] = A_BYTES + idx * 1024;
    }
    const unsigned Hu = (unsigned)(a.H << up), Wu = (unsigned)(a.W << up);
    unsigned a_b0[LA], a_b1[LA], a_msk[LA], b_b[LB];
    if constexpr (PIPE == 2) {
#pragma unroll
        for (int i = 0; i < LB; ++i) b_b[i] = (unsigned)b_off[i] * 2u;
    }
    if constexpr (PIPE == 1) {
#pragma unroll
        for (int i = 0; i < LA; ++i) {
            a_b0[i] = a_b1[i] = a_msk[i] = 0;
            const int q = (wave + i * NW) * 64 + lane, r = q >> 2;
            const int m = m0 + r;
            if (m < a.M) {
                unsigned cen = (unsigned)m;
                a_msk[i] = 1;
                if (CONV) {
                    const int hw = a.Ho * a.Wo;
                    const int b = m / hw, rem = m - b * hw;
                    const int oy = (rem / a.Wo) * sy + br, ox = (rem - (rem / a.Wo) * a.Wo) * sy + br;
                    cen = (unsigned)(b * a.H * a.W + (oy >> up) * a.W + (ox >> up));
                    unsigned msk = 0;
#pragma unroll
                    for (int t = 0; t < 9; ++t) {
                        const int uy = oy + t / 3 - 1, ux = ox + t % 3 - 1;
                        if ((unsigned)uy < Hu && (unsigned)ux < Wu) msk |= 1u << t;
                    }
                    if (up) msk |= ((oy & 1) ? 0u : 1u << 16) | ((ox & 1) ? 0u : 1u << 17);
                    a_msk[i] = msk;
                }
                a_b0[i] = (cen * (unsigned)a.C0 + (unsigned)a_off[i]) * 2u;
                a_b1[i] = (cen * (unsigned)a.C1 + (unsigned)a_off[i]) * 2u;
            }
        }
#pragma unroll
        for (int i = 0; i < LB; ++i) b_b[i] = (unsigned)b_off[i] * 2u;
    }

    auto stage_piece = [&](int kt, int tap, int cc, int buf, int p) {
        const unsigned base = __builtin_amdgcn_readfirstlane(lds_addr(smem) + buf * STAGE_BYTES);
        if (p < LA) {
            const int i = p;
            const half_t* src = a.A0;
            int Cs = a.C0, co = cc;
            if (co >= a.C0) { src = a.A1; Cs = a.C1; co -= a.C0; }
            const int ky = tap / 3 - 1, kx = tap - (tap / 3) * 3 - 1;
            const half_t* ptr = a.zero;
            if (!CONV) {
                if (a_pix[i] >= 0) ptr = src + (size_t)a_pix[i] * Cs + co + a_off[i];
            } else {
                const int uy = (a_yx[i] >> 16) + ky, ux = (a_yx[i] & 0xffff) + kx;
                if (a_pix[i] >= 0 && (unsigned)uy < Hu && (unsigned)ux < Wu)
                    ptr = src + (size_t)(a_pix[i] + (uy >> up) * a.W + (ux >> up)) * Cs + co + a_off[i];
            }
            if constexpr (ABL) { if (a.debug & 8) ptr = a.zero; }
            glds16(ptr, base + (wave + i * NW) * 1024);
        } else {
            const int i = p - LA;
            const half_t* ptr = a.Wt + (size_t)b_off[i] + ((size_t)(k_begin + kt) << 5);
            if constexpr (ABL) { if (a.debug & 8) ptr = a.zero; }
            glds16(ptr, base + b_lds[i]);
        }
    };
    auto stage = [&](int kt, int tap, int cc, int buf) {
#pragma unroll
        for (int p = 0; p < LPS; ++p) stage_piece(kt, tap, cc, buf, p);
    };

    acc_t acc[NI][MI];
#pragma unroll
    for (int j = 0; j < NI; ++j)
#pragma unroll
        for (int i = 0; i < MI; ++i)
#pragma unroll
            for (int r = 0; r < AR; ++r) acc[j][i][r] = 0.f;

    const int lrow = lane & (MS - 1), lh = lane / MS, swz = swz_of(lrow);
    const int lq = 4 * lh;
    int koff[KS];
#pragma unroll
    for (int ks = 0; ks < KS; ++ks) koff[ks] = lrow * ROWB + ((((MS == 32 ? ks * 2 : 0) + lh) ^ swz) << 4);

    int tap = 0, cc = k_begin << 5;
    if (CONV) { const int q = k_begin >> 1; tap = q % 9; cc = (q / 9) * 64 + (k_begin & 1) * 32; }
    auto advance = [&]() {
        if (!CONV) { cc += 32; return; }
        if (cc & 32) {
            if (++tap == 9) { tap = 0; cc += 32; } else { cc -= 32; }
        } else {
            cc += 32;
        }
    };
    struct StageSc { const char* sbase; const char* wbase; unsigned lbase; bool s1; int tap; int dyE, dyO, dxE, dxO; };
    auto stage_scalars = [&](int kn, int tap, int cc) {
        StageSc sc;
        sc.s1 = cc >= a.C0;
        const half_t* src = sc.s1 ? a.A1 : a.A0;
        const int Cs = sc.s1 ? a.C1 : a.C0;
        int disp = sc.s1 ? cc - a.C0 : cc;
        const int ky = tap / 3 - 1, kx = tap - (tap / 3) * 3 - 1;
        sc.dyE = sc.dyO = sc.dxE = sc.dxO = 0;
        if (CONV) {
            if (!up) {
                disp += (ky * a.W + kx) * Cs;
            } else {
                sc.dyE = ky < 0 ? -a.W * Cs * 2 : 0; sc.dyO = ky > 0 ? a.W * Cs * 2 : 0;
                sc.dxE = kx < 0 ? -Cs * 2 : 0;       sc.dxO = kx > 0 ? Cs * 2 : 0;
            }
        }
        sc.sbase = (const char*)src + (ptrdiff_t)disp * 2;
        sc.wbase = (const char*)a.Wt + ((size_t)(k_begin + kn) << 6);
        sc.lbase = __builtin_amdgcn_readfirstlane(lds_addr(smem) + (kn & 3) * STAGE_BYTES);
        sc.tap = tap;
        return sc;
    };
    auto lean_piece = [&](const StageSc& sc, int p) {
        bool zsrc = false;
        if constexpr (ABL) zsrc = (a.debug & 8) != 0;
        if (p < LA) {
            unsigned off = sc.s1 ? a_b1[p] : a_b0[p];
            if (CONV && up) off += (unsigned)(((a_msk[p] >> 16) & 1 ? sc.dyE : sc.dyO) + ((a_msk[p] >> 17) & 1 ? sc.dxE : sc.dxO));
            const char* ptr = ((a_msk[p] >> sc.tap) & 1) ? sc.sbase + off : (const char*)a.zero;
            if constexpr (ABL) { if (zsrc) ptr = (const char*)a.zero; }
            glds16_m0(ptr, sc.lbase + (wave + p * NW) * 1024);
        } else if (ABL && zsrc) {
            glds16_m0(a.zero, sc.lbase + b_lds[p - LA]);
        } else {
            glds16_sv(b_b[p - LA], sc.wbase, sc.lbase + b_lds[p - LA]);
        }
    };
    auto advance_bf = [&]() {
        if (!CONV) { cc += 32; return; }
        const bool second = (cc & 32) != 0, wrap = second && tap == 8;
        cc = second ? (wrap ? cc + 32 : cc - 32) : cc + 32;
        tap = second ? (wrap ? 0 : tap + 1) : tap;
    };
#pragma unroll
    for (int s = 0; s < STAGES - 1; ++s) {
        if (PIPE != 2 && s < nk) {
            if constexpr (PIPE == 0) { stage(s, tap, cc, s); advance(); }
            else if constexpr (PIPE == 1) {
                const StageSc sc = stage_scalars(s, tap, cc);
#pragma unroll
                for (int pp = 0; pp < LPS; ++pp) lean_piece(sc, pp);
                advance_bf();
            }
        }
    }

    float* bias_l = (float*)(smem + RING_BYTES);
    float* rv_l = bias_l + BN;
    float* mr_l = rv_l + RV_MAX * BN;
    float* u_l = mr_l + 2 * BM;
    const int rps = a.rows_per_sample;
    const int smp0 = m0 / rps;
    const int last_row = min(m0 + BM, a.M) - 1;
    const int nsmp = a.rowvec ? last_row / rps - smp0 + 1 : 0;
    const bool rv_in_lds = nsmp <= RV_MAX;
    for (int c = tid; c < BN; c += T) bias_l[c] = a.bias ? a.bias[n0 + c] : 0.f;
    if constexpr (LN) {
        for (int c = tid; c < BN; c += T) u_l[c] = a.ln_u[n0 + c];
        for (int r = tid; r < BM; r += T) {
            float mean = 0.f, rstd = 0.f;
            if (m0 + r < a.M) {
                const float* sp = a.ln_stats + (size_t)(m0 + r) * a.ln_slots * 2;
                float sm = 0.f, sq = 0.f;
                for (int p = 0; p < a.ln_slots; ++p) { sm += sp[2 * p]; sq += sp[2 * p + 1]; }
                const double mu = (double)sm / (double)a.C0;
                double var = (double)sq / (double)a.C0 - mu * mu;
                if (var < 0.0) var = 0.0;
                mean = (float)mu;
                rstd = (float)(1.0 / sqrt(var + (double)a.ln_eps));
            }
            mr_l[2 * r] = mean; mr_l[2 * r + 1] = rstd;
        }
    }
    if (a.rowvec && rv_in_lds)
        for (int c = tid; c < nsmp * BN; c += T) {
            const int sidx = c / BN, ch = c - sidx * BN;
            rv_l[c] = a.rowvec[(size_t)(smp0 + sidx) * a.rv_stride + n0 + ch];
        }

    if constexpr (PIPE == 0) {
        auto wait_stage = [&](int k_needed) {
            const int younger = min(nk - 1 - k_needed, STAGES - 2);
            if (STAGES >= 4 && younger >= 2) wait_vmcnt<2 * LPS>();
            else if (STAGES >= 3 && younger == 1) wait_vmcnt<LPS>();
            else wait_vmcnt<0>();
        };
        for (int kt = 0; kt < nk; ++kt) {
            wait_stage(kt);
            __builtin_amdgcn_s_waitcnt(0xC07F);
            __builtin_amdgcn_s_barrier();
            bool refill = kt + STAGES - 1 < nk;
            if constexpr (ABL) refill = refill && !(a.debug & 1);
            if (refill) { stage(kt + STAGES - 1, tap, cc, (kt + STAGES - 1) % STAGES); advance(); }
            const char* As = smem + (kt % STAGES) * STAGE_BYTES + (wm * TM) * ROWB;
            const char* Bs = smem + (kt % STAGES) * STAGE_BYTES + A_BYTES + (wn * TN) * ROWB;
            h8 xf[KS][MI], wf[KS][NI];
#pragma unroll
            for (int ks = 0; ks < KS; ++ks) {
#pragma unroll
                for (int i = 0; i < MI; ++i) xf[ks][i] = *(const h8*)(As + i * MS * ROWB + koff[ks]);
#pragma unroll
                for (int j = 0; j < NI; ++j) wf[ks][j] = *(const h8*)(Bs + j * MS * ROWB + koff[ks]);
            }
            __builtin_amdgcn_sched_barrier(0);
#pragma unroll
            for (int ks = 0; ks < KS; ++ks)
#pragma unroll
                for (int j = 0; j < NI; ++j)
#pragma unroll
                    for (int i = 0; i < MI; ++i) {
                        if constexpr (MS == 32) acc[j][i] = __builtin_amdgcn_mfma_f32_32x32x16_f16(wf[ks][j], xf[ks][i], acc[j][i], 0, 0, 0);
                        else acc[j][i] = __builtin_amdgcn_mfma_f32_16x16x32_f16(wf[ks][j], xf[ks][i], acc[j][i], 0, 0, 0);
                    }
        }
    } else if constexpr (PIPE == 2) {
        static_assert(CONV && MS == 16 && STAGES == 4 && !ABL, "halo loop: 3x3 stride-1 convolution on the 16x16x32 MFMA");
        constexpr int RW = NI % 5 == 0 ? 5 : 4, WD = 3;
        static_assert(NI % RW == 0 && WD < RW && NI >= RW, "W ring");
        constexpr int HB = halo_px<BM>() * ROWB, HPCS = halo_px<BM>() / 16;
        constexpr int LH = (HPCS + NW - 1) / NW;
        constexpr int WST = BN * ROWB;
        const int Wd = a.W, Pp = Wd + 2, hwp = a.H * a.W;
        const bool whole = hwp < BM;
        const int RS = whole ? a.H : BM / Wd, HP1 = (RS + 2) * Pp, NSL = whole ? BM / hwp : 1, NPX = NSL * HP1;
        const int bimg = m0 / hwp, y0 = whole ? 0 : (m0 - bimg * hwp) / Wd;
        const int nsub = nk / 9, sub0 = k_begin / 9;
        unsigned h_pix[LH], h_pc[LH];
        bool h_ok[LH];
#pragma unroll
        for (int u = 0; u < LH; ++u) {
            const int q = (wave + u * NW) * 64 + lane, hp = q >> 2, sp = q & 3;
            const int img = hp / HP1, rem = hp - img * HP1, hr = rem / Pp, hx = rem - hr * Pp, y = y0 + hr - 1, x = hx - 1;
            h_ok[u] = hp < NPX && (unsigned)x < (unsigned)Wd && (unsigned)y < (unsigned)a.H && bimg + img < a.B;
            h_pix[u] = h_ok[u] ? (unsigned)((bimg + img) * hwp + y * Wd + x) : 0u;
            h_pc[u] = (unsigned)((sp ^ ((hp >> 2) & 3)) << 4);
        }
        const unsigned lds_h = __builtin_amdgcn_readfirstlane(lds_addr(smem)), lds_w = lds_h + 2 * HB;
        auto issue_halo = [&](int sub) {
            const int cch = (sub0 + sub) << 5;
            const bool s1 = cch >= a.C0;
            const char* sb = s1 ? (const char*)(a.A1 + (cch - a.C0)) : (const char*)(a.A0 + cch);
            const unsigned rowb = (unsigned)(s1 ? a.C1 : a.C0) * 2u;
            const unsigned lb = lds_h + (unsigned)(sub & 1) * HB;
#pragma unroll
            for (int u = 0; u < LH; ++u)
                if (wave + u * NW < HPCS) {
                    const char* ptr = h_ok[u] ? sb + (h_pix[u] * rowb + h_pc[u]) : (const char*)a.zero;
                    glds16_m0(ptr, lb + (unsigned)(wave + u * NW) * 1024u);
                }
        };
        auto w_src = [&](int sub, int tp) { const int sa = sub0 + sub; return (const char*)a.Wt + ((size_t)(((sa >> 1) * 9 + tp) * 64 + (sa & 1) * 32) << 1); };
        auto issue_w = [&](int kn, int sub, int tp, int p) { glds16_sv(b_b[p], w_src(sub, tp), lds_w + (unsigned)(kn & 3) * WST + (unsigned)(b_lds[p] - A_BYTES)); };
        int hpc[MI];
#pragma unroll
// ... 128 lines not shown
            step(std::true_type{}, kt, xa, xb);
            ++kt;
#pragma unroll
            for (int i = 0; i < MI; ++i) xa[i] = xb[i];
        }
        if (kt < nk) step(std::false_type{}, kt, xa, xb);
        if (kt + 1 < nk) step(std::false_type{}, kt + 1, xb, xa);
        if (kt + 2 < nk) step(std::false_type{}, kt + 2, xa, xb);
        wait_vmcnt<0>();
    }

    if constexpr (SPLIT) {
        float* wsp = a.ws + (size_t)split * a.M * a.N;
#pragma unroll
        for (int i = 0; i < MI; ++i) {
            const int row = m0 + wm * TM + i * MS + lrow;
            if (row >= a.M) continue;
#pragma unroll
            for (int j = 0; j < NI; ++j)
#pragma unroll
                for (int g = 0; g < AR / 4; ++g) {
                    const int col = n0 + wn * TN + j * MS + (MS == 32 ? 8 * g : 0) + lq;
                    f32x4 pk = {acc[j][i][g * 4], acc[j][i][g * 4 + 1], acc[j][i][g * 4 + 2], acc[j][i][g * 4 + 3]};
                    *(f32x4*)(wsp + (size_t)row * a.N + col) = pk;
                }
        }
        return;
    } else {
    if (ABL && (a.debug & 4)) {
        float sink = 0.f;
#pragma unroll
        for (int j = 0; j < NI; ++j)
#pragma unroll
            for (int i = 0; i < MI; ++i) sink += acc[j][i][0] + acc[j][i][AR - 1];
        if (sink == 12345.678f) ((float*)a.out)[0] = sink;
        return;
    }
    asm volatile("s_waitcnt lgkmcnt(0)" ::: "memory");
    __builtin_amdgcn_s_barrier();
    if constexpr (LN) {
        const float* uw = u_l + wn * TN;
#pragma unroll
        for (int j = 0; j < NI; ++j)
#pragma unroll
            for (int g = 0; g < AR / 4; ++g) {
                const f32x4 uq = *(const f32x4*)(uw + j * MS + (MS == 32 ? 8 * g : 0) + lq);
#pragma unroll
                for (int i = 0; i < MI; ++i) {
                    const int trow = wm * TM + i * MS + lrow;
                    const float mean = mr_l[2 * trow], rstd = mr_l[2 * trow + 1];
#pragma unroll
                    for (int e = 0; e < 4; ++e) acc[j][i][g * 4 + e] = ln_scale(acc[j][i][g * 4 + e], mean, rstd, uq[e]);
                }
            }
    }
    constexpr int OUT_TN = GEGLU ? TN / 2 : TN;
    constexpr int PITCH = OUT_TN * 2 + 8;
    constexpr int CPR = OUT_TN / 8;
    constexpr int WB_IT = (32 * CPR + 63) / 64;
    static_assert(!GEGLU || NI % 2 == 0, "GEGLU needs value/gate tile pairs");
    constexpr bool TR = PATH == 1 && LN && !GEGLU;
    constexpr int TPITCH = 32 * 2 + 16;
    constexpr int CST_BYTES = TR && OUT_TN * TPITCH > 32 * PITCH ? OUT_TN * TPITCH : 32 * PITCH;
    static_assert(NW * CST_BYTES <= RING_BYTES, "epilogue staging must fit in the ring");
    char* cst = smem + wave * CST_BYTES;
    const bool second = a.out2 && n0 >= a.split_n;
    void* const outp = second ? a.out2 : a.out;
    const int okind = second ? a.out_kind2 : a.out_kind, ldo = second ? a.ld_out2 : a.ld_out;
    const int ncol0 = second ? a.split_n : 0, nend = a.out2 ? (second ? a.N : a.split_n) : a.N;
    const bool tr = TR && okind == OUT_F16_T;
    const int ocol0 = GEGLU ? ((n0 + wn * TN) >> 1) : (n0 + wn * TN - ncol0);
    const int nvalid = GEGLU ? a.N / 2 : nend - ncol0;
    const float* bw = bias_l + wn * TN;

    constexpr int PT = 32 / MS;
    constexpr int NG = AR / 4;
#pragma unroll
    for (int ip = 0; ip < TM / 32; ++ip) {
#pragma unroll
      for (int hf = 0; hf < PT; ++hf) {
        const int i = ip * PT + hf;
        const int prow = hf * MS + lrow;
        const int row = m0 + wm * TM + ip * 32 + prow;
        const int bsmp = (a.rowvec && row < a.M) ? row / rps : smp0;
        const float* rw = rv_l + (bsmp - smp0) * BN + wn * TN;
#pragma unroll
        for (int j = 0; j < NI; ++j) {
            if (GEGLU && (MS == 32 ? (j & 1) : (j & 2))) continue;
#pragma unroll
            for (int g = 0; g < NG; ++g) {
                const int wc = j * MS + (MS == 32 ? 8 * g : 0) + lq;
                const f32x4 bq = *(const f32x4*)(bw + wc);
                float v[4];
#pragma unroll
                for (int e = 0; e < 4; ++e) v[e] = acc[j][i][g * 4 + e] + bq[e];
                if (PATH == 2 || (PATH == 0 && a.rowvec)) {
                    if (PATH == 2 || rv_in_lds) {
                        const f32x4 rq = *(const f32x4*)(rw + wc);
#pragma unroll
                        for (int e = 0; e < 4; ++e) v[e] += rq[e];
                    } else if (row < a.M) {
#pragma unroll
                        for (int e = 0; e < 4; ++e) v[e] += a.rowvec[(size_t)bsmp * a.rv_stride + n0 + wn * TN + wc + e];
                    }
                }
                if (PATH == 0 && a.act == ACT_SILU) {
#pragma unroll
                    for (int e = 0; e < 4; ++e) v[e] = silu_f(v[e]);
                } else if (PATH == 0 && a.act == ACT_RELU) {
#pragma unroll
                    for (int e = 0; e < 4; ++e) v[e] = fmaxf(v[e], 0.f);
                }
                if constexpr (GEGLU) {
                    constexpr int GJ = MS == 32 ? 1 : 2;
                    const f32x4 gq = *(const f32x4*)(bw + wc + 32);
                    const f32x2 g01 = gelu2_f(f32x2{acc[j + GJ][i][g * 4] + gq[0], acc[j + GJ][i][g * 4 + 1] + gq[1]});
                    const f32x2 g23 = gelu2_f(f32x2{acc[j + GJ][i][g * 4 + 2] + gq[2], acc[j + GJ][i][g * 4 + 3] + gq[3]});
                    v[0] *= g01[0]; v[1] *= g01[1]; v[2] *= g23[0]; v[3] *= g23[1];
                }
#pragma unroll
                for (int e = 0; e < 4; ++e) v[e] *= a.scale;
                const int oc = !GEGLU ? wc : (MS == 32 ? (j >> 1) * 32 + 8 * g + lq : (j >> 2) * 32 + (j & 1) * 16 + lq);
                if (TR && tr) {
#pragma unroll
                    for (int e = 0; e < 4; ++e) *(half_t*)(cst + (oc + e) * TPITCH + prow * 2) = (half_t)v[e];
                } else if (PATH != 0 || okind == OUT_F16) {
                    h4 pk = {(half_t)v[0], (half_t)v[1], (half_t)v[2], (half_t)v[3]};
                    *(h4*)(cst + prow * PITCH + oc * 2) = pk;
                } else if (row < a.M && ocol0 + oc < nvalid) {
                    const int ch = ocol0 + oc;
                    if (okind == OUT_F32) {
                        f32x4 pk = {v[0], v[1], v[2], v[3]};
                        *(f32x4*)((float*)outp + (size_t)row * ldo + ch) = pk;
                    } else {
                        const int b = row / rps, t = row - b * rps;
#pragma unroll
                        for (int e = 0; e < 4; ++e) {
                            const size_t off = ((size_t)b * nvalid + ch + e) * ldo + t;
                            if (okind == OUT_F16_T) ((half_t*)outp)[off] = (half_t)v[e];
                            else ((float*)outp)[off] = v[e];
                        }
                    }
                }
            }
        }
      }
        if (TR && tr) {
            asm volatile("s_waitcnt lgkmcnt(0)" ::: "memory");
            const int row0 = m0 + wm * TM + ip * 32;
            const int b = row0 / rps, t0 = row0 - b * rps;
            constexpr int TT = OUT_TN * 4;
            if (row0 < a.M) {
#pragma unroll
                for (int it = 0; it < (TT + 63) / 64; ++it) {
                    const int task = lane + it * 64, c = task >> 2, q = task & 3;
                    if (task < TT && ocol0 + c < nvalid) {
                        const h8 val = *(const h8*)(cst + c * TPITCH + q * 16);
                        *(h8*)((half_t*)outp + ((size_t)b * nvalid + ocol0 + c) * ldo + t0 + q * 8) = val;
                    }
                }
            }
            asm volatile("s_waitcnt lgkmcnt(0)" ::: "memory");
        } else if (PATH != 0 || okind == OUT_F16) {
            asm volatile("s_waitcnt lgkmcnt(0)" ::: "memory");
            h8 v[WB_IT], rr[WB_IT];
            size_t goff[WB_IT];
            bool ok[WB_IT];
#pragma unroll
            for (int it = 0; it < WB_IT; ++it) {
                const int c = lane + it * 64;
                const int pr = c / CPR, ck = c - pr * CPR;
                const int grow = m0 + wm * TM + ip * 32 + pr;
                const int gcol = ocol0 + ck * 8;
                ok[it] = c < 32 * CPR && grow < a.M && gcol < nvalid;
                goff[it] = (size_t)grow * ldo + gcol;
                if (ok[it]) {
                    const char* sp = cst + pr * PITCH + ck * 16;
                    const h4 lo = *(const h4*)sp, hi = *(const h4*)(sp + 8);
                    v[it] = h8{lo[0], lo[1], lo[2], lo[3], hi[0], hi[1], hi[2], hi[3]};
                    if (a.resid) rr[it] = *(const h8*)(a.resid + (size_t)grow * a.ld_res + gcol);
                }
            }
            bool want_stats = false;
            constexpr bool HALF = OUT_TN == 80 && WN == 2 && TM == 32 && !GEGLU;
            if constexpr (OUT_TN == 160 || HALF) want_stats = a.stats_out != nullptr;
            float* tab = (float*)cst;
            if (want_stats) asm volatile("s_waitcnt lgkmcnt(0)" ::: "memory");
#pragma unroll
            for (int it = 0; it < WB_IT; ++it) {
                if (ok[it]) {
                    if (a.resid) v[it] = v[it] + rr[it];
                    *(h8*)((half_t*)outp + goff[it]) = v[it];
                }
                if (want_stats) {
                    const int c = lane + it * 64;
                    if (c < 32 * CPR) {
                        float sm = 0.f, sq = 0.f;
                        if (ok[it]) {
#pragma unroll
                            for (int e = 0; e < 8; ++e) { const float f = (float)v[it][e]; sm += f; sq += f * f; }
                        }
                        tab[2 * c] = sm; tab[2 * c + 1] = sq;
                    }
                }
            }
            asm volatile("s_waitcnt lgkmcnt(0)" ::: "memory");
            if constexpr (HALF) {
                if (want_stats) {
                    __builtin_amdgcn_s_barrier();
                    if (wn == 0 && lane < 32) {
                        const float* tab1 = (const float*)(smem + (wave + 1) * CST_BYTES);
                        const int grow = m0 + wm * TM + ip * 32 + lane;
                        float sm = 0.f, sq = 0.f;
#pragma unroll
                        for (int k = 0; k < CPR; ++k) { sm += tab[2 * (lane * CPR + k)]; sq += tab[2 * (lane * CPR + k) + 1]; }
#pragma unroll
                        for (int k = 0; k < CPR; ++k) { sm += tab1[2 * (lane * CPR + k)]; sq += tab1[2 * (lane * CPR + k) + 1]; }
                        if (grow < a.M) {
                            float* dst = a.stats_out + ((size_t)grow * (a.N / 160) + n0 / 160) * 2;
                            dst[0] = sm; dst[1] = sq;
                        }
                    }
                    asm volatile("s_waitcnt lgkmcnt(0)" ::: "memory");
                }
            } else
            if (want_stats) {
                if (lane < 32) {
                    const int grow = m0 + wm * TM + ip * 32 + lane;
                    float sm = 0.f, sq = 0.f;
#pragma unroll
                    for (int k = 0; k < CPR; ++k) { sm += tab[2 * (lane * CPR + k)]; sq += tab[2 * (lane * CPR + k) + 1]; }
                    if (grow < a.M) {
                        float* dst = a.stats_out + ((size_t)grow * (a.N / 160) + (n0 + wn * TN) / 160) * 2;
                        dst[0] = sm; dst[1] = sq;
                    }
                }
                asm volatile("s_waitcnt lgkmcnt(0)" ::: "memory");
            }
        }
    }
    }
}

template <int BM, int BN, int WM, int WN, int STAGES, bool CONV, bool GEGLU, bool SPLIT, int MS, bool LN, int PATH, int PIPE, bool ABL>
__global__ __launch_bounds__(WM * WN * 64) void igemm2_kernel(const IgemmArgs a) {
    igemm2_body<BM, BN, WM, WN, STAGES, CONV, GEGLU, SPLIT, MS, LN, PATH, PIPE, ABL>(a);
}
struct IgemmArgsG { IgemmArgs g[FGDM_MAX_GROUP]; };
template <int BM, int BN, int WM, int WN, int STAGES, bool CONV, bool GEGLU, bool SPLIT, int MS, bool LN, int PATH, int PIPE, bool ABL>
__global__ __launch_bounds__(WM * WN * 64) void igemm2_pair_kernel(const IgemmArgsG p) {
    igemm2_body<BM, BN, WM, WN, STAGES, CONV, GEGLU, SPLIT, MS, LN, PATH, PIPE, ABL>(p.g[blockIdx.y]);
}

template <bool LN>
__global__ __launch_bounds__(512) void igemm2_geglu_persist_kernel(const IgemmArgs a, int ntiles, int contiguous) {
    constexpr int BM = 256, BN = 256, WM = 4, WN = 2, NW = 8, T = 512, STAGES = 4, MS = 16;
    constexpr int TM = BM / WM, TN = BN / WN, MI = TM / MS, NI = TN / MS, AR = 4;
    typedef float acc_t __attribute__((ext_vector_type(AR)));
    constexpr int LA = BM * 4 / 64 / NW, LB = BN * 4 / 64 / NW, LPS = LA + LB;
    constexpr int STAGE_BYTES = (BM + BN) * ROWB, A_BYTES = BM * ROWB, RING_BYTES = STAGES * STAGE_BYTES;
    constexpr int OPS_FLOATS = BN + 2 * BM + BN;
    extern __shared__ __attribute__((aligned(16))) char smem[];
    auto swz_of = [](int r) { return ((r >> 3) & 1) << 1; };

    const int tid = threadIdx.x, lane = tid & 63;
    const int wave = __builtin_amdgcn_readfirstlane(tid >> 6);
    const int wm = wave / WN, wn = wave % WN;
    const int ntn = a.N / BN;
    const int nk = a.K >> 5;
    const int xcd = blockIdx.x & 7, G8 = gridDim.x >> 3, tq = ntiles >> 3, tr = ntiles & 7;
    const int x_first = xcd < tr ? xcd * (tq + 1) : tr * (tq + 1) + (xcd - tr) * tq, x_count = tq + (xcd < tr ? 1 : 0);
    const int per = (x_count + G8 - 1) / G8, jw = blockIdx.x >> 3;
    const int t_first = contiguous ? x_first + jw * per : x_first + jw;
    const int t_count = contiguous ? min(per, x_count - jw * per) : (x_count - jw + G8 - 1) / G8;
    const int t_step = contiguous ? 1 : G8;
    int local = 0;
    if (t_count <= 0) return;

    const int lrow = lane & (MS - 1), lh = lane / MS, lq = 4 * lh;
    const int koff = lrow * ROWB + ((lh ^ swz_of(lrow)) << 4);
    unsigned a_b0[LA], a_ok[LA], b_b[LB];
    int b_lds[LB];
    auto setup = [&](int m0x, int n0x) {
#pragma unroll
        for (int i = 0; i < LA; ++i) {
            const int q = (wave + i * NW) * 64 + lane, r = q >> 2, sp = q & 3, m = m0x + r;
            a_ok[i] = m < a.M ? 1u : 0u;
            a_b0[i] = a_ok[i] ? ((unsigned)m * (unsigned)a.C0 + (unsigned)((sp ^ swz_of(r)) << 3)) * 2u : 0u;
        }
#pragma unroll
        for (int i = 0; i < LB; ++i) {
            const int idx = wave + i * NW, q = idx * 64 + lane, r = q >> 2, sp = q & 3;
            b_b[i] = ((unsigned)(n0x + r) * (unsigned)a.K + (unsigned)((sp ^ swz_of(r)) << 3)) * 2u;
            b_lds[i] = A_BYTES + idx * 1024;
        }
    };
    const unsigned lds0 = __builtin_amdgcn_readfirstlane(lds_addr(smem));
    auto issue_stage = [&](int kn) {
        const char* sbase = (const char*)a.A0 + ((size_t)kn << 6);
        const char* wbase = (const char*)a.Wt + ((size_t)kn << 6);
        const unsigned lbase = lds0 + (unsigned)(kn & 3) * STAGE_BYTES;
#pragma unroll
        for (int p2 = 0; p2 < LA; ++p2) glds16_m0(a_ok[p2] ? sbase + a_b0[p2] : (const char*)a.zero, lbase + (unsigned)(wave + p2 * NW) * 1024u);
#pragma unroll
        for (int p2 = 0; p2 < LB; ++p2) glds16_sv(b_b[p2], wbase, lbase + (unsigned)b_lds[p2]);
    };
    float* const ops = (float*)(smem + RING_BYTES);
    auto stage_ops = [&](int m0x, int n0x, int set, bool same_rows) {
        float* bias_l = ops + set * OPS_FLOATS, *mr_l = bias_l + BN, *u_l = mr_l + 2 * BM;
        for (int c = tid; c < BN; c += T) bias_l[c] = a.bias ? a.bias[n0x + c] : 0.f;
        if constexpr (LN) {
            for (int c = tid; c < BN; c += T) u_l[c] = a.ln_u[n0x + c];
            if (same_rows) {
                const float* prev = ops + (set ^ 1) * OPS_FLOATS + BN;
                for (int r = tid; r < 2 * BM; r += T) mr_l[r] = prev[r];
            } else
            for (int r = tid; r < BM; r += T) {
                float mean = 0.f, rstd = 0.f;
                if (m0x + r < a.M) {
                    const float* sp = a.ln_stats + (size_t)(m0x + r) * a.ln_slots * 2;
                    float sm = 0.f, sq = 0.f;
                    for (int p2 = 0; p2 < a.ln_slots; ++p2) { sm += sp[2 * p2]; sq += sp[2 * p2 + 1]; }
                    const double mu = (double)sm / (double)a.C0;
                    double var = (double)sq / (double)a.C0 - mu * mu;
                    if (var < 0.0) var = 0.0;
                    mean = (float)mu;
                    rstd = (float)(1.0 / sqrt(var + (double)a.ln_eps));
                }
                mr_l[2 * r] = mean; mr_l[2 * r + 1] = rstd;
            }
        }
    };
// ... 90 lines not shown
            m0 = (logical / ntn) * BM; n0 = (logical % ntn) * BN;
            setup(m0, n0);
            if (nk > 0) issue_stage(0);
            if (nk > 1) issue_stage(1);
        }
        const float* bias_l = ops + set * OPS_FLOATS, *mr_l = bias_l + BN, *u_l = mr_l + 2 * BM;
        if constexpr (LN) {
            const float* uw = u_l + wn * TN;
#pragma unroll
            for (int j = 0; j < NI; ++j) {
                const f32x4 uq = *(const f32x4*)(uw + j * MS + lq);
#pragma unroll
                for (int i = 0; i < MI; ++i) {
                    const int trow = wm * TM + i * MS + lrow;
                    const float mean = mr_l[2 * trow], rstd = mr_l[2 * trow + 1];
#pragma unroll
                    for (int e = 0; e < 4; ++e) acc[j][i][e] = ln_scale(acc[j][i][e], mean, rstd, uq[e]);
                }
            }
        }
        constexpr int OUT_TN = TN / 2, PITCH = OUT_TN * 2 + 8, CPR = OUT_TN / 8, WB_IT = (32 * CPR + 63) / 64, CST_BYTES = 32 * PITCH;
        static_assert(NW * CST_BYTES <= 2 * STAGE_BYTES, "epilogue staging must fit ring slots 2 and 3");
        char* cst = smem + 2 * STAGE_BYTES + wave * CST_BYTES;
        const int ocol0 = (n0c + wn * TN) >> 1, nvalid = a.N / 2;
        const float* bw = bias_l + wn * TN;
#pragma unroll
        for (int ip = 0; ip < TM / 32; ++ip) {
#pragma unroll
            for (int hf = 0; hf < 2; ++hf) {
                const int i = ip * 2 + hf;
                const int prow = hf * MS + lrow;
#pragma unroll
                for (int j = 0; j < NI; ++j) {
                    if (j & 2) continue;
                    const int wc = j * MS + lq;
                    const f32x4 bq = *(const f32x4*)(bw + wc);
                    float v[4];
#pragma unroll
                    for (int e = 0; e < 4; ++e) v[e] = acc[j][i][e] + bq[e];
                    const f32x4 gq = *(const f32x4*)(bw + wc + 32);
                    const f32x2 g01 = gelu2_f(f32x2{acc[j + 2][i][0] + gq[0], acc[j + 2][i][1] + gq[1]});
                    const f32x2 g23 = gelu2_f(f32x2{acc[j + 2][i][2] + gq[2], acc[j + 2][i][3] + gq[3]});
                    v[0] *= g01[0]; v[1] *= g01[1]; v[2] *= g23[0]; v[3] *= g23[1];
#pragma unroll
                    for (int e = 0; e < 4; ++e) v[e] *= a.scale;
                    const int oc = (j >> 2) * 32 + (j & 1) * 16 + lq;
                    const h4 pk = {(half_t)v[0], (half_t)v[1], (half_t)v[2], (half_t)v[3]};
                    *(h4*)(cst + prow * PITCH + oc * 2) = pk;
                }
            }
            asm volatile("s_waitcnt lgkmcnt(0)" ::: "memory");
#pragma unroll
            for (int it = 0; it < WB_IT; ++it) {
                const int c = lane + it * 64, pr = c / CPR, ck = c - pr * CPR;
                const int grow = m0c + wm * TM + ip * 32 + pr, gcol = ocol0 + ck * 8;
                if (c < 32 * CPR && grow < a.M && gcol < nvalid) {
                    const char* sp = cst + pr * PITCH + ck * 16;
                    const h4 lo = *(const h4*)sp, hi = *(const h4*)(sp + 8);
                    *(h8*)((half_t*)a.out + (size_t)grow * a.ld_out + gcol) = h8{lo[0], lo[1], lo[2], lo[3], hi[0], hi[1], hi[2], hi[3]};
                }
            }
            asm volatile("s_waitcnt lgkmcnt(0)" ::: "memory");
        }
        if (!more) break;
        set ^= 1;
        stage_ops(m0, n0, set, m0 == m0c);
        asm volatile("s_waitcnt lgkmcnt(0)" ::: "memory");
        __builtin_amdgcn_s_barrier();
        if (nk > 2) issue_stage(2);
        first = false;
    }
}

template <bool LN>
int launch_geglu_persist(const IgemmArgs& a, int ntiles, int contiguous, hipStream_t s) {
    constexpr int smem = 4 * (256 + 256) * ROWB + 2 * (256 + 2 * 256 + 256) * 4;
    static_assert(smem <= 160 * 1024, "LDS budget");
    constexpr auto k = igemm2_geglu_persist_kernel<LN>;
    if (fgdm_dyn_lds<k>(smem) != FGDM_OK) return FGDM_ERR_HIP;
    FGDM_LAUNCH(k, dim3(256), dim3(512), smem, s, a, ntiles, contiguous);
    return hipGetLastError() == hipSuccess ? FGDM_OK : FGDM_ERR_HIP;
}

template <int BM, int BN, int WM, int WN, int STAGES, bool CONV, bool GEGLU, bool SPLIT, int MS, bool LN, int PATH, int PIPE, bool ABL>
int launch2p(const IgemmArgs& a, hipStream_t s) {
    constexpr int ring = ring_bytes<BM, BN, STAGES, PIPE>();
    constexpr int smem = ring + (1 + RV_MAX) * BN * 4 + (2 * BM + BN) * 4;
    static_assert(smem <= 160 * 1024, "LDS budget");
    constexpr auto k = igemm2_kernel<BM, BN, WM, WN, STAGES, CONV, GEGLU, SPLIT, MS, LN, PATH, PIPE, ABL>;
    if (fgdm_dyn_lds<k>(smem) != FGDM_OK) return FGDM_ERR_HIP;
    const int ntm = (a.M + BM - 1) / BM, ntn = (a.N + BN - 1) / BN;
    const unsigned gx = (unsigned)(ntm * ntn * (SPLIT ? a.splitk : 1));
    if (fgdm_recording()) {
        auto single = [=](hipStream_t rs) -> int {
            hipLaunchKernelGGL(k, dim3(gx), dim3(WM * WN * 64), smem, rs, a);
            return hipGetLastError() == hipSuccess ? FGDM_OK : FGDM_ERR_HIP;
        };
        if constexpr (PIPE != 0 && PATH != 0 && !SPLIT && !ABL && MS == 16) {
            constexpr auto kp = igemm2_pair_kernel<BM, BN, WM, WN, STAGES, CONV, GEGLU, SPLIT, MS, LN, PATH, PIPE, ABL>;
            if (fgdm_dyn_lds<kp>(smem) != FGDM_OK) return FGDM_ERR_HIP;
            static_assert(sizeof(IgemmArgs) <= FGDM_GROUP_BLOB, "the recorded blob holds an IgemmArgs");
            FgdmGroupFn pf = [](const void* const* av, int n, unsigned grid_x, hipStream_t rs) -> int {
                if (n < 2 || n > FGDM_MAX_GROUP) return FGDM_ERR_ARG;
                IgemmArgsG pg;
                for (int i = 0; i < FGDM_MAX_GROUP; ++i) pg.g[i] = *(const IgemmArgs*)av[i < n ? i : 0];
                hipLaunchKernelGGL((igemm2_pair_kernel<BM, BN, WM, WN, STAGES, CONV, GEGLU, SPLIT, MS, LN, PATH, PIPE, ABL>), dim3(grid_x, n),
                                   dim3(WM * WN * 64), smem, rs, pg);
                return hipGetLastError() == hipSuccess ? FGDM_OK : FGDM_ERR_HIP;
            };
            fgdm_record(single, (const void*)kp, pf, &a, sizeof(a), gx, 0);
        } else {
            fgdm_record(single);
        }
        return FGDM_OK;
    }
    hipLaunchKernelGGL(k, dim3(gx), dim3(WM * WN * 64), smem, s, a);
    return hipGetLastError() == hipSuccess ? FGDM_OK : FGDM_ERR_HIP;
}
template <int BM, bool GEGLU, bool LN>
int epilogue_path(const IgemmArgs& a) {
    if (a.out_kind != OUT_F16 || !(a.act == ACT_NONE || GEGLU)) return 0;
    if (a.out2 && a.out_kind2 != OUT_F16) {
        const bool staged = LN && a.out_kind2 == OUT_F16_T && a.rows_per_sample % 32 == 0 && a.M % 32 == 0 && a.ld_out2 % 8 == 0 &&
                            ((size_t)a.out2 & 15) == 0;
        if (!staged || a.rowvec) return 0;
    }
    if (!a.rowvec) return 1;
    return (BM - 1) / a.rows_per_sample + 2 <= RV_MAX ? 2 : 0;
}
template <int BM, int BN, int WM, int WN, int STAGES, bool CONV, bool GEGLU, bool SPLIT, int MS, bool LN, bool FAST, int PIPE>
int launch2(const IgemmArgs& a, hipStream_t s) {
    const bool fast_on = knob_once(KNOB_IGEMM_EPI_PATHS) != 0;
    if constexpr (FAST && !SPLIT && !LN) {
        if (a.debug)
            return epilogue_path<BM, GEGLU, LN>(a) == 1 ? launch2p<BM, BN, WM, WN, STAGES, CONV, GEGLU, SPLIT, MS, LN, 1, (PIPE == 2 ? 1 : PIPE), true>(a, s)
                                                        : FGDM_ERR_ARG;
    }
    if (a.debug) return FGDM_ERR_ARG;
    if constexpr (SPLIT) return launch2p<BM, BN, WM, WN, STAGES, CONV, GEGLU, SPLIT, MS, LN, 0, PIPE, false>(a, s);
    if constexpr (FAST && !SPLIT) {
        switch (fast_on ? epilogue_path<BM, GEGLU, LN>(a) : 0) {
            case 1: return launch2p<BM, BN, WM, WN, STAGES, CONV, GEGLU, SPLIT, MS, LN, 1, PIPE, false>(a, s);
            case 2: if constexpr (!GEGLU && !LN) return launch2p<BM, BN, WM, WN, STAGES, CONV, GEGLU, SPLIT, MS, LN, 2, PIPE, false>(a, s);
            default: break;
        }
    }
    return launch2p<BM, BN, WM, WN, STAGES, CONV, GEGLU, SPLIT, MS, LN, 0, 0, false>(a, s);
}
template <int BM, int BN, bool GEGLU, int MS, int PIPE, int WM, int WN>
int launch2m(const IgemmArgs& a, hipStream_t s) {
    constexpr int PL = PIPE == 2 ? 1 : PIPE;
    return a.mode == IG_LINEAR ? launch2<BM, BN, WM, WN, 4, false, GEGLU, false, MS, false, MS == 16, PL>(a, s)
                               : launch2<BM, BN, WM, WN, 4, true, GEGLU, false, MS, false, MS == 16, (GEGLU ? PL : PIPE)>(a, s);
}
template <int BM, int BN, bool GEGLU, int MS, int PIPE, int WM, int WN>
int launch2ln(const IgemmArgs& a, hipStream_t s) {
    return launch2<BM, BN, WM, WN, 4, false, GEGLU, false, MS, true, MS == 16, (PIPE == 2 ? 1 : PIPE)>(a, s);
}
template <int BM, int BN, int MS, int PIPE, int WM = 4, int WN = 2>
int launch_tile(const IgemmArgs& a, hipStream_t s) {
    const bool g = a.act == ACT_GEGLU;
    if (a.ln_stats) {
        if constexpr (BN == 256) { if (g) return launch2ln<BM, BN, true, MS, PIPE, WM, WN>(a, s); }
        if constexpr (BN == 128) return FGDM_ERR_ARG;
        else return launch2ln<BM, BN, false, MS, PIPE, WM, WN>(a, s);
    }
    if constexpr (BN == 256) { if (g) return launch2m<BM, BN, true, MS, PIPE, WM, WN>(a, s); }
    return launch2m<BM, BN, false, MS, PIPE, WM, WN>(a, s);
}

__global__ __launch_bounds__(256) void splitk_reduce_kernel(const IgemmArgs a) {
    const size_t total4 = (size_t)a.M * a.N / 4, plane = (size_t)a.M * a.N;
    for (size_t i = (size_t)blockIdx.x * 256 + threadIdx.x; i < total4; i += (size_t)gridDim.x * 256) {
        const size_t e0 = i * 4;
        const int row = (int)(e0 / a.N), col = (int)(e0 - (size_t)row * a.N);
        f32x4 v = *(const f32x4*)(a.ws + e0);
        for (int s = 1; s < a.splitk; ++s) {
            const f32x4 u = *(const f32x4*)(a.ws + (size_t)s * plane + e0);
            v[0] += u[0]; v[1] += u[1]; v[2] += u[2]; v[3] += u[3];
        }
        h4 r = {(half_t)0, (half_t)0, (half_t)0, (half_t)0};
        if (a.resid) r = *(const h4*)(a.resid + (size_t)row * a.ld_res + col);
        h4 o;
#pragma unroll
        for (int e = 0; e < 4; ++e) {
            float x = v[e] + (a.bias ? a.bias[col + e] : 0.f);
            if (a.rowvec) x += a.rowvec[(size_t)(row / a.rows_per_sample) * a.rv_stride + col + e];
            if (a.act == ACT_SILU) x = silu_f(x);
            else if (a.act == ACT_RELU) x = fmaxf(x, 0.f);
            else if (a.act == ACT_QGELU) x = silu_f(x, 1.702f);
            const half_t y = (half_t)(x * a.scale);
            o[e] = a.resid ? (half_t)((float)y + (float)r[e]) : y;
        }
        *(h4*)((half_t*)a.out + (size_t)row * a.ld_out + col) = o;
    }
}

}

static thread_local bool g_twin_layers = false;
void igemm_set_twin_layers(bool on) { g_twin_layers = on; }

int igemm_splitk_factor(const IgemmArgs& a) {
    if (a.force_cfg || a.act == ACT_GEGLU || a.out_kind != OUT_F16 || a.N % 320 || (a.K & 31)) return 1;
    const int nk = a.K >> 5;
    const bool fat = knob_once(KNOB_SPLITK_FAT) != 0;
    if (fat && a.rows_per_sample > 64 && a.rows_per_sample <= 256 && (nk >= 540 || (nk >= 360 && !g_twin_layers))) return 2;
    if (a.rows_per_sample > 64 || nk < 96) return 1;
    return (fat && nk >= 360) ? 8 : 4;
}
int igemm_splitk_reduce(const IgemmArgs& a, hipStream_t s) {
    const size_t total4 = (size_t)a.M * a.N / 4;
    const int grid = (int)std::min<size_t>(2048, (total4 + 255) / 256);
    FGDM_LAUNCH(splitk_reduce_kernel, dim3(grid), dim3(256), 0, s, a);
    return hipGetLastError() == hipSuccess ? FGDM_OK : FGDM_ERR_HIP;
}

static bool halo_geometry(const IgemmArgs& a) {
    if (a.mode != IG_CONV3 || a.Ho != a.H || a.Wo != a.W || (a.C0 & 63) || (a.C1 & 63) || (a.K % 288) || a.debug) return false;
    if ((a.W == 16 || a.W == 32 || a.W == 64) && (a.H * a.W) % 256 == 0) return true;
    return a.W == 8 && a.H == 8;
}

int igemm2_launch(const IgemmArgs& a, int cfg, hipStream_t s) {
    if ((a.K & 31) || (a.C0 & 31) || (a.C1 & 31)) return FGDM_ERR_ARG;
    const int pipe_default = knob_once(KNOB_IGEMM_PIPE);
    const int tile = cfg & 15, psel = cfg >> 4;
    const size_t px = a.mode == IG_LINEAR ? (size_t)a.M : (size_t)a.B * a.H * a.W;
    const bool small = px * (size_t)std::max(a.C0, a.C1) * 2 < (1ull << 32) && (size_t)(a.N + 320) * a.K * 2 < (1ull << 32);
    const bool pipe = (psel == 0 ? pipe_default != 0 : psel == 2) && small;
    const bool halo = knob_once(KNOB_IGEMM_HALO) != 0 && pipe && halo_geometry(a);
    const int bn = (tile == 1 || tile == 4) ? 256 : tile == 6 ? 128 : tile == 7 ? 160 : 320;
    if (a.N % bn) return FGDM_ERR_ARG;
    if (a.act == ACT_GEGLU && bn != 256) return FGDM_ERR_ARG;
    if (a.splitk > 1) {
        if ((tile != 2 && tile != 0) || a.ln_stats) return FGDM_ERR_ARG;
        const int nk_all = a.K >> 5;
        if (halo && nk_all % a.splitk == 0 && (nk_all / a.splitk) % 9 == 0)
            return tile == 0 ? launch2<256, 320, 4, 2, 4, true, false, true, 16, false, false, 2>(a, s)
                             : launch2<128, 320, 4, 2, 4, true, false, true, 16, false, false, 2>(a, s);
        if (tile == 0 && pipe)
            return a.mode == IG_LINEAR ? launch2<256, 320, 4, 2, 4, false, false, true, 16, false, false, 1>(a, s)
                                       : launch2<256, 320, 4, 2, 4, true, false, true, 16, false, false, 1>(a, s);
        if (pipe)
            return a.mode == IG_LINEAR ? launch2<128, 320, 4, 2, 4, false, false, true, 16, false, false, 1>(a, s)
                                       : launch2<128, 320, 4, 2, 4, true, false, true, 16, false, false, 1>(a, s);
        return a.mode == IG_LINEAR ? launch2<128, 320, 4, 2, 4, false, false, true, 16, false, false, 0>(a, s)
                                   : launch2<128, 320, 4, 2, 4, true, false, true, 16, false, false, 0>(a, s);
    }
    if (a.ln_stats && a.mode != IG_LINEAR) return FGDM_ERR_ARG;
    const int persist_mode = knob_once(KNOB_IGEMM_PERSIST);
    const bool persist_on = persist_mode != 0;
    if (persist_on && tile == 1 && pipe && a.act == ACT_GEGLU && a.mode == IG_LINEAR && !a.C1 && a.out_kind == OUT_F16 && !a.rowvec &&
        !a.resid && !a.out2 && !a.stats_out && !a.debug && a.N % 256 == 0) {
        const int ntiles = ((a.M + 255) / 256) * (a.N / 256);
        if (ntiles > 256) return a.ln_stats ? launch_geglu_persist<true>(a, ntiles, persist_mode == 2, s) : launch_geglu_persist<false>(a, ntiles, persist_mode == 2, s);
    }
    switch (tile) {
        case 0: return halo ? launch_tile<256, 320, 16, 2>(a, s) : pipe ? launch_tile<256, 320, 16, 1>(a, s) : launch_tile<256, 320, 16, 0>(a, s);
        case 1: return pipe ? launch_tile<256, 256, 16, 1>(a, s) : launch_tile<256, 256, 16, 0>(a, s);
        case 2: return halo ? launch_tile<128, 320, 16, 2>(a, s) : pipe ? launch_tile<128, 320, 16, 1>(a, s) : launch_tile<128, 320, 16, 0>(a, s);
        case 3: return launch_tile<256, 320, 32, 0>(a, s);
        case 4: return launch_tile<256, 256, 32, 0>(a, s);
        case 5: return launch_tile<128, 320, 32, 0>(a, s);
        case 6: return pipe ? launch_tile<256, 128, 16, 1>(a, s) : launch_tile<256, 128, 16, 0>(a, s);
        case 7: return a.mode != IG_LINEAR ? FGDM_ERR_ARG : pipe ? launch_tile<64, 160, 16, 1, 2, 2>(a, s) : launch_tile<64, 160, 16, 0, 2, 2>(a, s);
        default: return FGDM_ERR_ARG;
    }
}
```

fgdm_amd/csrc/knobs.h:

```cpp
#pragma once
#include "common.h"
#include <array>
#include <cstdlib>

#define FGDM_STR_(x) #x
#define FGDM_STR(x) FGDM_STR_(x)

#define FGDM_KNOBS(X)                                                                                                          \
    X(ATTN_PP, "FGDM_ATTN_PP", "1", "0: the four-wave attention kernel where the eight-wave ping-pong one would run")           \
    X(ATTN_DQ, "FGDM_ATTN_DQ", "3", "long self-attention, d = 40: 3 = two-strand kernel, 32-wide V^T P^T; 1 = 16-wide; 0 = off") \
    X(ATTN_DQ80, "FGDM_ATTN_DQ80", "1", "0: the ping-pong kernel instead of the two-strand one at d = 80")                      \
    X(ATTN_ABL, "FGDM_ATTN_ABL", "0", "ablation instantiations of the two-strand kernel (tools/bench_attention.py only)")       \
    X(ATTN_CROSS, "FGDM_ATTN_CROSS", "4", "query chunks per wave of the text-token kernel (65 - 96 keys); 0 = off")             \
    X(ATTN_CROSS_LONG, "FGDM_ATTN_CROSS_LONG", "8", "query chunks per wave of the key-resident kernel (97 - 256 keys); 0 = off") \
    X(IGEMM_EPI_PATHS, "FGDM_IGEMM_EPI_PATHS", "1", "0: the general GEMM epilogue instead of the host-selected straight-line paths") \
    X(IGEMM_HALO, "FGDM_IGEMM_HALO", "1", "0: per-tap K loop instead of the halo-tile loop (stride-1 3x3 convolutions, split K too)") \
    X(IGEMM_MFMA32, "FGDM_IGEMM_MFMA32", "0", "1: automatic tile choices take the 32x32x16 MFMA instantiations")                \
    X(IGEMM_OTHER_WIDTHS, "FGDM_IGEMM_OTHER_WIDTHS", "1", "0: widths 128 / 256 / 512 back on the 2-stage kernel")               \
    X(IGEMM_PERSIST, "FGDM_IGEMM_PERSIST", "1", "GEGLU projections: 1 = persistent, tiles round-robin; 2 = contiguous runs; 0 = off") \
    X(IGEMM_PIPE, "FGDM_IGEMM_PIPE", "1", "0: the phase-locked K loop instead of the software-pipelined one")                   \
    X(IGEMM_SMALL_M, "FGDM_IGEMM_SMALL_M", "1", "0: linears with a thin 128-row grid stay on 128 x 320 tiles")                  \
    X(IGEMM_SMALL_TILES, "FGDM_IGEMM_SMALL_TILES", "1", "0: the 8x8 level's linears back on the 2-stage kernel")                \
    X(IGEMM_STATS64, "FGDM_IGEMM_STATS64", "1", "0: the 64 x 160 tile leaves the LayerNorm partial sums to the row-statistics pass") \
    X(SPLITK_FAT, "FGDM_SPLITK_FAT", "1", "0: split K four ways on 128 x 320 tiles at the 8x8 level only")                      \
    X(PAIR_FAT_TILES, "FGDM_PAIR_FAT_TILES", "1", "0: grouped launches keep the tile a single problem would take")              \
    X(GN_REG, "FGDM_GN_REG", "1024", "largest pixel count per sample of the register-resident GroupNorm; 0 = off")              \
    X(GN_REG_NG, "FGDM_GN_REG_NG", "4", "widest slice of the register-resident GroupNorm, in groups")                           \
    X(GN_FUSED_MAXKB, "FGDM_GN_FUSED_MAXKB", "64", "largest LDS slice (KB) of the single-kernel GroupNorm; 0 = always two kernels") \
    X(GN_CHUNK, "FGDM_GN_CHUNK", FGDM_STR(GN_PIX_PER_CHUNK), "pixels per partial-sum chunk of the two-kernel GroupNorm (multiples of 64)") \
    X(LN_FOLD, "FGDM_LN_FOLD", "1", "fgdm_create; 0: the transformer blocks' LayerNorms as kernels of their own")               \
    X(TWIN_STREAMS, "FGDM_TWIN_STREAMS", "0", "fgdm_create; 1: the ControlNets on a second stream next to the UNet encoder")    \
    X(PAIR_LAUNCH, "FGDM_PAIR_LAUNCH", "1", "fgdm_create; 0: no grouped launches of twin layers")                               \
    X(GROUP_MAX, "FGDM_GROUP_MAX", FGDM_STR(FGDM_MAX_GROUP), "fgdm_create; problems per grouped launch, clamped to [2, FGDM_MAX_GROUP]") \
    X(GN_GROUP, "FGDM_GN_GROUP", "1", "fgdm_create; 0: single-pass GroupNorm launches stay out of the grouped launches")        \
    X(PAIR_DEBUG, "FGDM_PAIR_DEBUG", nullptr, "set (to anything): fgdm_destroy prints how many replayed launches were fused")   \
    X(PROF_DUMP, "FGDM_PROF_DUMP", nullptr, "path: fgdm_profile_end writes the per-shape time table there")                     \
    X(BENCH_DATA_SCALE, "FGDM_BENCH_DATA_SCALE", "1", "atof; scale of the random operands of fgdm_bench_igemm / _attention")

enum Knob {
#define X(id, name, dflt, meaning) KNOB_##id,
    FGDM_KNOBS(X)
#undef X
    KNOB_COUNT
};
struct KnobDef { const char* name; const char* dflt; const char* meaning; };
inline constexpr KnobDef KNOB_TABLE[KNOB_COUNT] = {
#define X(id, name, dflt, meaning) {name, dflt, meaning},
    FGDM_KNOBS(X)
#undef X
};

inline const char* knob_text(Knob k) {
    const char* v = getenv(KNOB_TABLE[k].name);
    return v ? v : KNOB_TABLE[k].dflt;
}
inline int knob_int(Knob k) { return atoi(knob_text(k)); }
inline bool knob_on(Knob k) { return knob_int(k) != 0; }
inline int knob_once(Knob k) {
    static const std::array<int, KNOB_COUNT> v = [] {
        std::array<int, KNOB_COUNT> a{};
        for (int i = 0; i < KNOB_COUNT; ++i)
            if (KNOB_TABLE[i].dflt) a[i] = knob_int((Knob)i);
        return a;
    }();
    return v[k];
}
```

fgdm_amd/csrc/ops_abi.hip:

```cpp
#include "engine_shared.h"
#include "replay_plan.h"

static int op_pack(IgemmArgs& a, TmpDev& tmp, const float* w, const float* bias, int N, int K, int Ks, bool geglu,
                   const int* kmap = nullptr, const float* gamma = nullptr, const float* beta = nullptr) {
    auto host = [](const float* d, size_t n, std::vector<float>& v) { v.resize(n); return hipMemcpy(v.data(), d, n * sizeof(float), hipMemcpyDefault) == hipSuccess; };
    std::vector<float> wh, bh(N, 0.f), g, bt;
    if (!host(w, (size_t)N * Ks, wh) || (bias && !host(bias, N, bh))) return FGDM_ERR_HIP;
    if (gamma && (!host(gamma, K, g) || !host(beta, K, bt))) return FGDM_ERR_HIP;
    const size_t npad = igemm_npad(N);
    std::vector<half_t> pk(npad * (size_t)K, (half_t)0);
    std::vector<float> bp(npad, 0.f), u(gamma ? npad : 0, 0.f);
    for (int pr = 0; pr < N; ++pr) {
        int sr = pr;
        if (geglu) { const int grp = pr >> 6, within = pr & 63; sr = within < 32 ? grp * 32 + within : N / 2 + grp * 32 + (within - 32); }
        const float* row = &wh[(size_t)sr * Ks];
        double us = 0.0, cs = 0.0;
        for (int k = 0; k < K; ++k) {
            const int ks = kmap ? kmap[k] : k;
            if (ks < 0) continue;
            const half_t wq = (half_t)(gamma ? row[ks] * g[k] : row[ks]);
            pk[(size_t)pr * K + k] = wq;
            if (gamma) { us += (double)(float)wq; cs += (double)bt[k] * (double)row[ks]; }
        }
        bp[pr] = gamma ? (float)((double)bh[sr] + cs) : bh[sr];
        if (gamma) u[pr] = (float)us;
    }
    a.Wt = tmp.up(pk); a.bias = tmp.up(bp);
    if (gamma) a.ln_u = tmp.up(u);
    return a.Wt && a.bias && (!gamma || a.ln_u) ? FGDM_OK : FGDM_ERR_NOMEM;
}

static int op_gemm_rows(IgemmArgs& a, const half_t* A, int B, int Ho, int Wo, int K, int rps, TmpDev& tmp, hipStream_t s) {
    a.A0 = A; a.C0 = K; a.A1 = nullptr; a.C1 = 0;
    a.zero = g_zero_page();
    if (!a.zero) return FGDM_ERR_NOMEM;
    a.B = B; a.H = Ho; a.W = Wo; a.Ho = Ho; a.Wo = Wo;
    a.M = B * Ho * Wo; a.K = K; a.mode = IG_LINEAR; a.rows_per_sample = rps;
    if (plan_splitk(a, tmp) != FGDM_OK) return FGDM_ERR_NOMEM;
    return igemm_launch(a, s);
}

static int op_conv3_im2col(const half_t* x, int Cin, const float* w, const float* bias, const float* rowvec, const half_t* resid,
                           int B, int H, int W, int Cout, int stride, int act, float scale, void* out, hipStream_t s) {
    int cp = 0;
    const std::vector<int> kmap = conv3_kmap(Cin, &cp);
    const int K = (int)kmap.size(), Ho = (H - 1) / stride + 1, Wo = (W - 1) / stride + 1;
    TmpDev tmp;
    IgemmArgs a{};
    const int prc = op_pack(a, tmp, w, bias, Cout, K, Cin * 9, false, kmap.data());
    if (prc != FGDM_OK) return prc;
    half_t* A = tmp.alloc<half_t>((size_t)B * Ho * Wo * K);
    if (!A) return FGDM_ERR_NOMEM;
    a.rowvec = rowvec; a.rv_stride = Cout;
    a.resid = resid; a.ld_res = Cout;
    a.N = Cout; a.act = act; a.out_kind = OUT_F16; a.out = out; a.ld_out = Cout; a.scale = scale;
    const int rc = im2col_conv(x, A, B, H, W, cp, stride, K, s, []() {},
        [&](half_t* Ap, int Bv, int Hv, int Wv, int Kv, int rps) { return op_gemm_rows(a, Ap, Bv, Hv, Wv, Kv, rps, tmp, s); });
    (void)hipStreamSynchronize(s);
    return rc;
}

extern "C" {

int fgdm_op_conv2d(const void* x0, int C0, const void* x1, int C1, const float* w, const float* bias, const float* rowvec,
                   const void* resid, int B, int H, int W, int Cout, int ksize, int stride, int upsample, int act,
                   float scale, void* out, void* stream) {
    if (!x0 || !w || !out || (ksize != 1 && ksize != 3)) return FGDM_ERR_ARG;
    if (stride == FGDM_STRIDE2_PAD_BR && (ksize != 3 || upsample)) return FGDM_ERR_ARG;
    hipStream_t s = as_stream(stream);
    const int Cin = C0 + C1, taps = ksize * ksize, K = taps * Cin;
    if (B <= 0 || H <= 0 || W <= 0 || Cout <= 0 || C0 <= 0 || C1 < 0) return FGDM_ERR_ARG;
    if (Cin & 63) {
        if (ksize != 3 || C1 || x1 || upsample || (stride != 1 && stride != 2)) return FGDM_ERR_ARG;
        return op_conv3_im2col((const half_t*)x0, C0, w, bias, rowvec, (const half_t*)resid, B, H, W, Cout, stride, act, scale, out, s);
    }
    std::vector<int> kmap(K);
    for (int tap = 0; tap < taps; ++tap)
        for (int c = 0; c < Cin; ++c) kmap[taps == 9 ? ((c >> 6) * 9 + tap) * 64 + (c & 63) : c] = c * taps + tap;
    TmpDev tmp;
    IgemmArgs a{};
    const int prc = op_pack(a, tmp, w, bias, Cout, K, K, false, kmap.data());
    if (prc != FGDM_OK) return prc;
    a.A0 = (const half_t*)x0; a.C0 = C0; a.A1 = (const half_t*)x1; a.C1 = C1;
    a.zero = g_zero_page();
    if (!a.zero) return FGDM_ERR_NOMEM;
    a.rowvec = rowvec; a.rv_stride = Cout;
    a.resid = (const half_t*)resid; a.ld_res = Cout;
    a.B = B; a.H = H; a.W = W;
    a.Ho = H; a.Wo = W; a.mode = IG_LINEAR;
    if (ksize == 3) {
        a.mode = IG_CONV3;
        if (upsample) { a.Ho = 2 * H; a.Wo = 2 * W; a.mode = IG_CONV3_UP2; }
        else if (stride == 2) { a.Ho = (H - 1) / 2 + 1; a.Wo = (W - 1) / 2 + 1; a.mode = IG_CONV3_S2; }
        else if (stride == FGDM_STRIDE2_PAD_BR) {
            if (H < 2 || W < 2) return FGDM_ERR_ARG;
            a.Ho = (H - 2) / 2 + 1; a.Wo = (W - 2) / 2 + 1; a.mode = IG_CONV3_S2_BR;
        }
    }
    a.M = B * a.Ho * a.Wo; a.N = Cout; a.K = K;
    a.act = act; a.out_kind = OUT_F16; a.out = out; a.ld_out = Cout;
    a.rows_per_sample = a.Ho * a.Wo; a.scale = scale;
    if (plan_splitk(a, tmp) != FGDM_OK) return FGDM_ERR_NOMEM;
    const int rc = igemm_launch(a, s);
    (void)hipStreamSynchronize(s);
    return rc;
}

int fgdm_op_linear(const void* x, const float* w, const float* bias, const void* resid, int M, int K, int N, int act,
                   int out_kind, int rows_per_sample, int ld_out, void* out, void* stream) {
    if (!x || !w || !out || (K & 63)) return FGDM_ERR_ARG;
    hipStream_t s = as_stream(stream);
    TmpDev tmp;
    IgemmArgs a{};
    const int prc = op_pack(a, tmp, w, bias, N, K, K, act == ACT_GEGLU);
    if (prc != FGDM_OK) return prc;
    a.A0 = (const half_t*)x; a.C0 = K;
    a.zero = g_zero_page();
    if (!a.zero) return FGDM_ERR_NOMEM;
    const int nout = act == ACT_GEGLU ? N / 2 : N;
    a.resid = (const half_t*)resid; a.ld_res = nout;
    a.B = 1; a.H = 1; a.W = M; a.Ho = 1; a.Wo = M;
    a.M = M; a.N = N; a.K = K; a.mode = IG_LINEAR; a.act = act; a.out_kind = out_kind;
    a.out = out; a.ld_out = ld_out ? ld_out : nout;
    a.rows_per_sample = rows_per_sample ? rows_per_sample : M; a.scale = 1.f;
    const int rc = igemm_launch(a, s);
    (void)hipStreamSynchronize(s);
    return rc;
}

int fgdm_op_linear_ln_linear(const void* x, const float* w1, const float* b1, const void* resid, const float* gamma,
                             const float* beta, const float* w2, const float* b2, int M, int K1, int C, int N2, int act2,
                             void* h_out, void* y_out, int* slots_used, void* stream) {
    if (!x || !w1 || !gamma || !beta || !w2 || !h_out || !y_out || (K1 & 63) || (C & 63)) return FGDM_ERR_ARG;
    hipStream_t s = as_stream(stream);
    TmpDev tmp;
    IgemmArgs a{}, b{};
    int rc = op_pack(a, tmp, w1, b1, C, K1, K1, false);
    if (rc == FGDM_OK) rc = op_pack(b, tmp, w2, b2, N2, C, C, act2 == ACT_GEGLU, nullptr, gamma, beta);
    if (rc != FGDM_OK) return rc;
    a.A0 = (const half_t*)x; a.C0 = K1; a.zero = g_zero_page();
    a.resid = (const half_t*)resid; a.ld_res = C;
    a.B = 1; a.H = 1; a.W = M; a.Ho = 1; a.Wo = M; a.M = M; a.N = C; a.K = K1; a.mode = IG_LINEAR; a.act = ACT_NONE;
    a.out_kind = OUT_F16; a.out = h_out; a.ld_out = C; a.rows_per_sample = M; a.scale = 1.f;
    if (!a.zero) return FGDM_ERR_NOMEM;
    int slots = igemm_stats_slots(a);
    float* stats = tmp.alloc<float>((size_t)M * std::max(slots, row_stats_slots(C)) * 2);
    if (!stats) return FGDM_ERR_NOMEM;
    if (slots) a.stats_out = stats;
    rc = igemm_launch(a, s);
    if (rc == FGDM_OK && !slots) { slots = row_stats_slots(C); rc = row_stats_launch((const half_t*)h_out, M, C, stats, s); }
    if (slots_used) *slots_used = a.stats_out ? slots : -slots;
    if (rc != FGDM_OK) { (void)hipStreamSynchronize(s); return rc; }
    b.A0 = (const half_t*)h_out; b.C0 = C; b.zero = a.zero;
    b.ln_stats = stats; b.ln_slots = slots; b.ln_eps = 1e-5f;
    const int nout = act2 == ACT_GEGLU ? N2 / 2 : N2;
    b.B = 1; b.H = 1; b.W = M; b.Ho = 1; b.Wo = M; b.M = M; b.N = N2; b.K = C; b.mode = IG_LINEAR; b.act = act2;
    b.out_kind = OUT_F16; b.out = y_out; b.ld_out = nout; b.rows_per_sample = M; b.scale = 1.f;
    rc = igemm_launch(b, s);
// ... 142 lines not shown
```

Measured before the change: 8.027.

## Compute VAE upsample convs as four 2x2 sub-pixel phase GEMMs

Adds an IG_CONV2_UP2P igemm mode. A nearest-2x upsample followed by a 3x3 conv becomes four phase-specific 2x2 convs over the low-resolution input, with weights pre-summed per phase at pack time. This cuts the K dimension from 9*Cin to 4*Cin and removes redundant reads of duplicated pixels. The cost is scattered output rows through an LDS row map, a disabled vector NCHW store path, and different rounding from the summed f16 weights. It is enabled by default only for the VAE decoder upsamplers, while the UNet path stays off via a constexpr flag.

```diff
diff --git a/fgdm_amd/csrc/common.h b/fgdm_amd/csrc/common.h
--- a/fgdm_amd/csrc/common.h
+++ b/fgdm_amd/csrc/common.h
@@ -46,7 +46,7 @@
 #define FGDM_ERR_STATE -3
 #define FGDM_ERR_NOMEM -4
 
-enum IgemmMode { IG_LINEAR = 0, IG_CONV3 = 1, IG_CONV3_S2 = 2, IG_CONV3_UP2 = 3, IG_CONV3_S2_BR = 4 };
+enum IgemmMode { IG_LINEAR = 0, IG_CONV3 = 1, IG_CONV3_S2 = 2, IG_CONV3_UP2 = 3, IG_CONV3_S2_BR = 4, IG_CONV2_UP2P = 5 };
 enum IgemmAct { ACT_NONE = 0, ACT_SILU = 1, ACT_RELU = 2, ACT_GEGLU = 3, ACT_QGELU = 4  };
 enum IgemmOut { OUT_F16 = 0, OUT_F32 = 1, OUT_F32_NCHW = 2, OUT_F16_T = 3 };
 
@@ -82,6 +82,8 @@
     int split_n, out_kind2, ld_out2;
 };
 
+__host__ __device__ inline int igemm_tile_rows(const IgemmArgs& a) { return a.mode == IG_CONV2_UP2P ? a.B * a.H * a.W : a.M; }
+inline int igemm_row_tiles(const IgemmArgs& a, int BM) { return (igemm_tile_rows(a) + BM - 1) / BM * (a.mode == IG_CONV2_UP2P ? 4 : 1); }
 int igemm_launch(const IgemmArgs& a, hipStream_t s);
 void igemm_set_force_cfg(int cfg);
 void igemm_set_twin_layers(bool on);
@@ -92,7 +94,7 @@
 int row_stats_launch(const half_t* x, int rows, int C, float* stats , hipStream_t s);
 int igemm_splitk_factor(const IgemmArgs& a);
 int igemm_splitk_reduce(const IgemmArgs& a, hipStream_t s);
-size_t igemm_npad(int n);
+__host__ __device__ inline size_t igemm_npad(int n) { return (size_t)((n + 127) / 128) * 128; }
 
 #define GN_PIX_PER_CHUNK 256
 void groupnorm_set_group(bool on);
diff --git a/fgdm_amd/csrc/engine.hip b/fgdm_amd/csrc/engine.hip
--- a/fgdm_amd/csrc/engine.hip
+++ b/fgdm_amd/csrc/engine.hip
@@ -92,6 +92,7 @@
     bool im2col = false;
     int cin_pad = 0;
     int k_real = 0;
+    bool up2p = false;
     float* ln_u = nullptr;
     float ln_eps = 1e-5f;
 };
@@ -239,6 +240,7 @@
     std::unordered_map<std::string, bool> comp_dirty, comp_packed;
     std::string cur_comp;
     bool ln_fold = true;
+    bool up2_phase = true;
     hipStream_t s = nullptr;
     std::vector<std::unique_ptr<Arena>> cn_arena;
     Arena* ar = &arena;
@@ -673,11 +675,22 @@
         }
         return pack_rows(g, srcs, K, K, {}, biases, false, scales, lg ? lg->host.data() : nullptr, lb ? lb->host.data() : nullptr);
     }
-    int pack_conv3(GemmW& g, const std::string& pre) {
+    int pack_conv3(GemmW& g, const std::string& pre, bool up = false) {
         const ParamSlot* w = slot(pre + ".weight");
         const ParamSlot* b = slot(pre + ".bias");
         if (!w || !b) return FGDM_ERR_STATE;
         const int N = (int)w->shape[0], Cin = (int)w->shape[1];
+        g.up2p = up && up2_phase && (Cin % 64) == 0;
+        if (g.up2p) {
+            std::vector<float> bias(igemm_npad(N), 0.f);
+            std::copy(b->host.begin(), b->host.begin() + N, bias.begin());
+            g.im2col = false; g.cin_pad = Cin;
+            g.N = N; g.K = g.k_real = 4 * Cin;
+            g.w = upload(up2_phase_pack(w->host.data(), N, Cin));
+            g.bias = upload(bias);
+            g.ln_u = nullptr;
+            return (g.w && g.bias) ? FGDM_OK : fail(FGDM_ERR_NOMEM, "hipMalloc failed while packing weights");
+        }
         int cp = 0;
         const std::vector<int> kmap = conv3_kmap(Cin, &cp);
         g.im2col = (Cin % 64) != 0;
@@ -694,13 +707,14 @@
         return (n.g && n.b) ? FGDM_OK : fail(FGDM_ERR_NOMEM, "hipMalloc failed");
     }
 #define CHK(x) do { int _rc = (x); if (_rc != FGDM_OK) return _rc; } while (0)
+    static constexpr bool UP2P_UNET = false;
     int pack_block(Block& blk) {
         for (Layer& l : blk) {
             const std::string& p = l.pre;
             switch (l.type) {
                 case L_CONV: CHK(pack_conv3(l.conv, p.substr(0, p.size() - 1))); break;
                 case L_DOWN: CHK(pack_conv3(l.conv, p + "op")); break;
-                case L_UP: CHK(pack_conv3(l.conv, p + "conv")); break;
+                case L_UP: CHK(pack_conv3(l.conv, p + "conv", UP2P_UNET)); break;
                 case L_RES:
                     CHK(pack_norm(l.gn1, p + "in_layers.0"));
                     CHK(pack_conv3(l.c1, p + "in_layers.2"));
@@ -829,7 +843,7 @@
         CHK(pack_vres(v.mid2));
         for (auto& lv : v.levels) {
             for (auto& r : lv.blocks) CHK(pack_vres(r));
-            if (lv.up) CHK(pack_conv3(lv.upconv, lv.up_pre));
+            if (lv.up) CHK(pack_conv3(lv.upconv, lv.up_pre, true));
         }
         CHK(pack_norm(v.norm_out, d + "norm_out"));
         CHK(pack_conv3(v.conv_out, d + "conv_out"));
@@ -917,7 +931,7 @@
         a.rows_per_sample = e.rps ? e.rps : Ho * Wo;
         a.scale = e.scale;
         a.out2 = e.out2; a.out_kind2 = e.out_kind2; a.ld_out2 = e.ld_out2; a.split_n = e.split_n;
-        const int taps = mode == IG_LINEAR ? 1 : 9;
+        const int taps = mode == IG_LINEAR ? 1 : mode == IG_CONV2_UP2P ? 4 : 9;
         if (taps * (a.C0 + a.C1) != a.K) return fail(FGDM_ERR_ARG, "gemm: K mismatch");
         if (!a.out) return fail(FGDM_ERR_NOMEM, "gemm: null output (workspace exhausted?)");
         char tag[56] = "";
@@ -961,9 +975,10 @@
     }
     int conv3(const GemmW& w, const Tensor& x, const Tensor* x1, int stride, bool up, Epi e, Tensor* out) {
         int Ho = x.H, Wo = x.W, mode = IG_CONV3;
-        if (up) { Ho *= 2; Wo *= 2; mode = IG_CONV3_UP2; }
+        if (up) { Ho *= 2; Wo *= 2; mode = w.up2p ? IG_CONV2_UP2P : IG_CONV3_UP2; }
         else if (stride == 2) { Ho = (x.H - 1) / 2 + 1; Wo = (x.W - 1) / 2 + 1; mode = IG_CONV3_S2; }
         else if (stride == FGDM_STRIDE2_PAD_BR) { Ho = (x.H - 2) / 2 + 1; Wo = (x.W - 2) / 2 + 1; mode = IG_CONV3_S2_BR; }
+        if (w.up2p && !up) return fail(FGDM_ERR_STATE, "conv3: these weights are packed for an Upsample");
         const bool own_out = (e.out == nullptr);
         if (own_out) { *out = talloc(x.B, Ho, Wo, w.N); if (!out->p) return fail(FGDM_ERR_NOMEM, "workspace"); }
         if (!w.im2col) return gemm(w, mode, x, x1, Ho, Wo, e, out);
@@ -1922,6 +1937,7 @@
     if (rc != FGDM_OK) return rc;
     e->device = device;
     e->ln_fold = knob_on(KNOB_LN_FOLD);
+    e->up2_phase = knob_on(KNOB_UP2_PHASE);
     rc = e->ensure_device();
     if (rc != FGDM_OK) {
         g_create_err = e->err + " [" + hipGetErrorString(hipGetLastError()) + "]";
diff --git a/fgdm_amd/csrc/engine_shared.h b/fgdm_amd/csrc/engine_shared.h
--- a/fgdm_amd/csrc/engine_shared.h
+++ b/fgdm_amd/csrc/engine_shared.h
@@ -20,6 +20,29 @@
         }
     *cin_pad = cp;
     return kmap;
+}
+
+static std::vector<half_t> up2_phase_pack(const float* w, int N, int Cin) {
+    static const int lo[2][2] = {{0, 1}, {0, 2}}, hi[2][2] = {{0, 2}, {1, 2}};
+    const size_t npad = igemm_npad(N), K = (size_t)4 * Cin;
+    std::vector<half_t> out(4 * npad * K, (half_t)0);
+    for (int p = 0; p < 4; ++p) {
+        const int a = p >> 1, b = p & 1;
+        for (int n = 0; n < N; ++n) {
+            half_t* dst = out.data() + ((size_t)p * npad + n) * K;
+            for (int c = 0; c < Cin; ++c) {
+                const float* src = w + ((size_t)n * Cin + c) * 9;
+                for (int t = 0; t < 4; ++t) {
+                    const int ty = t >> 1, tx = t & 1;
+                    float sum = 0.f;
+                    for (int ky = lo[a][ty]; ky <= hi[a][ty]; ++ky)
+                        for (int kx = lo[b][tx]; kx <= hi[b][tx]; ++kx) sum += src[ky * 3 + kx];
+                    dst[(size_t)((c >> 6) * 4 + t) * 64 + (c & 63)] = (half_t)sum;
+                }
+            }
+        }
+    }
+    return out;
 }
 
 template <class After, class Gemm>
diff --git a/fgdm_amd/csrc/igemm.hip b/fgdm_amd/csrc/igemm.hip
--- a/fgdm_amd/csrc/igemm.hip
+++ b/fgdm_amd/csrc/igemm.hip
@@ -38,7 +38,12 @@
         const int bid = blockIdx.x, xcd = bid & 7, q = nb >> 3, r = nb & 7;
         logical = (xcd < r ? xcd * (q + 1) : r * (q + 1) + (xcd - r) * q) + (bid >> 3);
     }
-    const int m0 = (logical / ntn) * BM, n0 = (logical % ntn) * BN;
+    const bool ph = a.mode == IG_CONV2_UP2P;
+    const int phase = ph ? (logical / ntn) & 3 : 0, pa = phase >> 1, pb = phase & 1;
+    const int m0 = (ph ? logical / (4 * ntn) : logical / ntn) * BM, n0 = (logical % ntn) * BN;
+    const int Mrows = igemm_tile_rows(a);
+    const int ntap = ph ? 4 : 9;
+    const half_t* const Wt = a.Wt + (ph ? (size_t)phase * igemm_npad(a.N) * a.K : (size_t)0);
 
     const int Ctot = a.C0 + a.C1;
     const int cpt = Ctot >> 6;
@@ -52,9 +57,15 @@
         const int m = m0 + r;
         a_pix[j] = -1;
         a_yx[j] = 0;
-        if (m < a.M) {
+        if (m < Mrows) {
             if (a.mode == IG_LINEAR) {
                 a_pix[j] = m;
+            } else if (ph) {
+                const int hw = a.H * a.W;
+                const int b = m / hw, rem = m - b * hw;
+                const int iy = rem / a.W, ix = rem - iy * a.W;
+                a_pix[j] = b * hw;
+                a_yx[j] = (iy << 16) | ix;
             } else {
                 const int hw = a.Ho * a.Wo;
                 const int b = m / hw, rem = m - b * hw;
@@ -77,7 +88,7 @@
         const half_t* src = a.A0;
         int Cs = a.C0, co = cc << 6;
         if (co >= a.C0) { src = a.A1; Cs = a.C1; co -= a.C0; }
-        const int ky = tap / 3, kx = tap - ky * 3;
+        const int ky = ph ? pa + (tap >> 1) : tap / 3, kx = ph ? pb + (tap & 1) : tap - (tap / 3) * 3;
 #pragma unroll
         for (int j = 0; j < A_IT; ++j) {
             const half_t* p = a.zero;
@@ -88,7 +99,7 @@
                     const int oy = a_yx[j] >> 16, ox = a_yx[j] & 0xffff;
                     int iy, ix;
                     bool ok;
-                    if (a.mode == IG_CONV3) {
+                    if (a.mode == IG_CONV3 || ph) {
                         iy = oy + ky - 1; ix = ox + kx - 1;
                         ok = (unsigned)iy < (unsigned)a.H && (unsigned)ix < (unsigned)a.W;
                     } else if (a.mode == IG_CONV3_S2) {
@@ -109,7 +120,7 @@
         }
 #pragma unroll
         for (int j = 0; j < B_IT; ++j)
-            glds16(a.Wt + (size_t)b_off[j] + ((size_t)kt << 6), Bs + (j * T + wave * 64) * 16);
+            glds16(Wt + (size_t)b_off[j] + ((size_t)kt << 6), Bs + (j * T + wave * 64) * 16);
     };
 
     f32x16 acc[MI][NI];
@@ -132,7 +143,7 @@
         __syncthreads();
         if (kt + 1 < nk) {
             if (a.mode == IG_LINEAR) ++cc;
-            else if (++tap == 9) { tap = 0; ++cc; }
+            else if (++tap == ntap) { tap = 0; ++cc; }
             stage(kt + 1, tap, cc, (kt + 1) & 1);
         }
         const char* As = smem + (kt & 1) * STAGE + (wm * TM) * 128;
@@ -185,8 +196,17 @@
             }
         }
     }
-    const int rps = a.rows_per_sample;
+    const int rps = ph ? a.H * a.W : a.rows_per_sample;
     const bool geglu = (a.act == ACT_GEGLU);
+    if (ph) {
+        __syncthreads();
+        for (int r = tid; r < BM; r += T) {
+            const int m = min(m0 + r, Mrows - 1), ni = m / a.W, jx = m - ni * a.W;
+            ((int*)smem)[r] = (2 * ni + pa) * a.Wo + 2 * jx + pb;
+        }
+        __syncthreads();
+    }
+    auto orow_of = [&](int row) { return ph ? ((const int*)smem)[row - m0] : row; };
     const bool second = a.out2 && n0 >= a.split_n;
     void* const outp = second ? a.out2 : a.out;
     const int okind = second ? a.out_kind2 : a.out_kind, ldo = second ? a.ld_out2 : a.ld_out;
@@ -206,7 +226,7 @@
 #pragma unroll
             for (int r = 0; r < 16; ++r) {
                 const int row = m0 + wm * TM + i * 32 + (r & 3) + 8 * (r >> 2) + 4 * lh;
-                rvv[r] = (a.rowvec && row < a.M) ? a.rowvec[(size_t)(row / rps) * a.rv_stride + pcol] : 0.f;
+                rvv[r] = (a.rowvec && row < Mrows) ? a.rowvec[(size_t)(row / rps) * a.rv_stride + pcol] : 0.f;
             }
 #pragma unroll
             for (int g = 0; g < 4; ++g) {
@@ -228,8 +248,8 @@
                     half_t* o = (half_t*)outp;
 #pragma unroll
                     for (int e = 0; e < 4; ++e) {
-                        const int row = row0 + e;
-                        if (row < a.M) {
+                        const int row = orow_of(row0 + e);
+                        if (row0 + e < Mrows) {
                             half_t x = (half_t)v[e];
                             if (a.resid) x = (half_t)((float)x + (float)a.resid[(size_t)row * a.ld_res + ocol]);
                             o[(size_t)row * ldo + ocol] = x;
@@ -239,9 +259,9 @@
                     float* o = (float*)outp;
 #pragma unroll
                     for (int e = 0; e < 4; ++e)
-                        if (row0 + e < a.M) o[(size_t)(row0 + e) * ldo + ocol] = v[e];
+                        if (row0 + e < Mrows) o[(size_t)orow_of(row0 + e) * ldo + ocol] = v[e];
                 } else {
-                    const bool vec = ((rps & 3) == 0) && (row0 + 3 < a.M);
+                    const bool vec = !ph && ((rps & 3) == 0) && (row0 + 3 < a.M);
                     if (vec) {
                         const int b = row0 / rps, t = row0 - b * rps;
                         const size_t off = ((size_t)b * nchan + ocol) * ldo + t;
@@ -255,9 +275,9 @@
                     } else {
 #pragma unroll
                         for (int e = 0; e < 4; ++e) {
-                            const int row = row0 + e;
-                            if (row < a.M) {
-                                const int b = row / rps, t = row - b * rps;
+                            const int row = orow_of(row0 + e);
+                            if (row0 + e < Mrows) {
+                                const int b = row / a.rows_per_sample, t = row - b * a.rows_per_sample;
                                 const size_t off = ((size_t)b * nchan + ocol) * ldo + t;
                                 if (okind == OUT_F16_T) ((half_t*)outp)[off] = (half_t)v[e];
                                 else ((float*)outp)[off] = v[e];
@@ -270,14 +290,12 @@
     }
 }
 
-size_t igemm_npad(int n) { return (size_t)((n + 127) / 128) * 128; }
-
 template <int BM, int BN, int WM, int WN>
 static int launch_cfg(const IgemmArgs& a, hipStream_t s) {
     constexpr int smem = 2 * (BM + BN) * 128;
     constexpr auto k = igemm_kernel<BM, BN, WM, WN>;
     if (fgdm_dyn_lds<k>(smem) != FGDM_OK) return FGDM_ERR_HIP;
-    const int ntm = (a.M + BM - 1) / BM, ntn = (a.N + BN - 1) / BN;
+    const int ntm = igemm_row_tiles(a, BM), ntn = (a.N + BN - 1) / BN;
     FGDM_LAUNCH(k, dim3(ntm * ntn), dim3(WM * WN * 64), smem, s, a);
     return hipGetLastError() == hipSuccess ? FGDM_OK : FGDM_ERR_HIP;
 }
@@ -321,7 +339,7 @@
 }
 
 int igemm_stats_slots(const IgemmArgs& a) {
-    if (a.out_kind != OUT_F16 || a.act == ACT_GEGLU || a.splitk > 1 || (a.N % 320) || (a.K & 31) || (a.C0 & 31) || (a.C1 & 31)) return 0;
+    if (a.mode == IG_CONV2_UP2P || a.out_kind != OUT_F16 || a.act == ACT_GEGLU || a.splitk > 1 || (a.N % 320) || (a.K & 31) || (a.C0 & 31) || (a.C1 & 31)) return 0;
     const int f = pick_force(a);
     if (f < 4) return 0;
     const int tile = (f - 4) & 15;
@@ -332,6 +350,8 @@
 int igemm_launch(const IgemmArgs& a, hipStream_t s) {
     if (a.M <= 0 || a.N <= 0 || a.K <= 0 || (a.K & 63) || (a.C0 & 63) || (a.C1 & 63)) return FGDM_ERR_ARG;
     if (a.act == ACT_GEGLU && (a.N & 63)) return FGDM_ERR_ARG;
+    if (a.mode == IG_CONV2_UP2P && (a.A1 || a.C1 || a.resid || a.splitk > 1 || a.stats_out || a.out2 || a.ln_stats || a.act == ACT_GEGLU ||
+                                    a.K != 4 * a.C0 || a.Ho != 2 * a.H || a.Wo != 2 * a.W || a.M != a.B * a.Ho * a.Wo)) return FGDM_ERR_ARG;
     if (a.ln_stats && (a.mode != IG_LINEAR || a.C1 || a.ln_slots <= 0 || !a.ln_u)) return FGDM_ERR_ARG;
     if (a.stats_out && igemm_stats_slots(a) == 0) return FGDM_ERR_ARG;
     if (a.out2 && (a.act == ACT_GEGLU || a.splitk > 1 || a.stats_out || a.split_n <= 0 || a.split_n >= a.N || (a.split_n % 640))) return FGDM_ERR_ARG;
diff --git a/fgdm_amd/csrc/igemm2.hip b/fgdm_amd/csrc/igemm2.hip
--- a/fgdm_amd/csrc/igemm2.hip
+++ b/fgdm_amd/csrc/igemm2.hip
@@ -44,11 +44,14 @@
     return PIPE == 2 ? 2 * halo_px<BM>() * ROWB + STAGES * BN * ROWB : STAGES * (BM + BN) * ROWB;
 }
 
-template <int BM, int BN, int WM, int WN, int STAGES, bool CONV, bool GEGLU, bool SPLIT, int MS, bool LN, int PATH, int PIPE, bool ABL>
+template <int BM, int BN, int WM, int WN, int STAGES, int CONV, bool GEGLU, bool SPLIT, int MS, bool LN, int PATH, int PIPE, bool ABL>
 __device__ __forceinline__ void igemm2_body(const IgemmArgs& a) {
     constexpr int NW = WM * WN, T = NW * 64;
     constexpr int TM = BM / WM, TN = BN / WN;
     constexpr int MI = TM / MS, NI = TN / MS;
+    constexpr bool PH = CONV == 2;
+    constexpr int NT = PH ? 4 : 9;
+    static_assert(!(PH && (SPLIT || LN || GEGLU || PIPE == 2)), "phase form: plain epilogue, per-tap loops");
     constexpr int KS = MS == 32 ? 2 : 1;
     constexpr int AR = MS == 32 ? 16 : 4;
     typedef float acc_t __attribute__((ext_vector_type(AR)));
@@ -81,9 +84,14 @@
         const int ntm = (a.M + BM - 1) / BM;
         const int row = logical % ntm, pair = logical / ntm;
         split = pair % nsplit; n0 = (pair / nsplit) * BN; m0 = row * BM;
+    } else if (PH) {
+        m0 = (logical / (4 * ntn)) * BM; n0 = (logical % ntn) * BN;
     } else {
         m0 = (logical / ntn) * BM; n0 = (logical % ntn) * BN;
     }
+    const int phase = PH ? (logical / ntn) & 3 : 0, pa = phase >> 1, pb = phase & 1;
+    const int Mrows = PH ? a.B * a.H * a.W : a.M;
+    const half_t* const Wt = PH ? a.Wt + (size_t)phase * igemm_npad(a.N) * a.K : a.Wt;
 
     const int nk_all = a.K >> 5;
     const int per = (nk_all + nsplit - 1) / nsplit;
@@ -101,9 +109,15 @@
         a_off[i] = (s ^ swz_of(r)) << 3;
         a_pix[i] = -1; a_yx[i] = 0;
         const int m = m0 + r;
-        if (PIPE == 0 && m < a.M) {
+        if (PIPE == 0 && m < Mrows) {
             if (!CONV) {
                 a_pix[i] = m;
+            } else if (PH) {
+                const int hw = a.H * a.W;
+                const int b = m / hw, rem = m - b * hw;
+                const int iy = rem / a.W, ix = rem - iy * a.W;
+                a_pix[i] = b * hw;
+                a_yx[i] = ((iy + pa) << 16) | (ix + pb);
             } else {
                 const int hw = a.Ho * a.Wo;
                 const int b = m / hw, rem = m - b * hw;
@@ -133,10 +147,21 @@
             a_b0[i] = a_b1[i] = a_msk[i] = 0;
             const int q = (wave + i * NW) * 64 + lane, r = q >> 2;
             const int m = m0 + r;
-            if (m < a.M) {
+            if (m < Mrows) {
                 unsigned cen = (unsigned)m;
                 a_msk[i] = 1;
-                if (CONV) {
+                if constexpr (PH) {
+                    const int hw = a.H * a.W;
+                    const int rem = m - (m / hw) * hw;
+                    const int iy = rem / a.W, ix = rem - iy * a.W;
+                    unsigned msk = 0;
+#pragma unroll
+                    for (int t = 0; t < 4; ++t) {
+                        const int uy = iy + pa + (t >> 1) - 1, ux = ix + pb + (t & 1) - 1;
+                        if ((unsigned)uy < Hu && (unsigned)ux < Wu) msk |= 1u << t;
+                    }
+                    a_msk[i] = msk;
+                } else if (CONV) {
                     const int hw = a.Ho * a.Wo;
                     const int b = m / hw, rem = m - b * hw;
                     const int oy = (rem / a.Wo) * sy + br, ox = (rem - (rem / a.Wo) * a.Wo) * sy + br;
@@ -165,7 +190,7 @@
             const half_t* src = a.A0;
             int Cs = a.C0, co = cc;
             if (co >= a.C0) { src = a.A1; Cs = a.C1; co -= a.C0; }
-            const int ky = tap / 3 - 1, kx = tap - (tap / 3) * 3 - 1;
+            const int ky = PH ? (tap >> 1) - 1 : tap / 3 - 1, kx = PH ? (tap & 1) - 1 : tap - (tap / 3) * 3 - 1;
             const half_t* ptr = a.zero;
             if (!CONV) {
                 if (a_pix[i] >= 0) ptr = src + (size_t)a_pix[i] * Cs + co + a_off[i];
@@ -178,7 +203,7 @@
             glds16(ptr, base + (wave + i * NW) * 1024);
         } else {
             const int i = p - LA;
-            const half_t* ptr = a.Wt + (size_t)b_off[i] + ((size_t)(k_begin + kt) << 5);
+            const half_t* ptr = Wt + (size_t)b_off[i] + ((size_t)(k_begin + kt) << 5);
             if constexpr (ABL) { if (a.debug & 8) ptr = a.zero; }
             glds16(ptr, base + b_lds[i]);
         }
@@ -203,11 +228,11 @@
     for (int ks = 0; ks < KS; ++ks) koff[ks] = lrow * ROWB + ((((MS == 32 ? ks * 2 : 0) + lh) ^ swz) << 4);
 
     int tap = 0, cc = k_begin << 5;
-    if (CONV) { const int q = k_begin >> 1; tap = q % 9; cc = (q / 9) * 64 + (k_begin & 1) * 32; }
+    if (CONV) { const int q = k_begin >> 1; tap = q % NT; cc = (q / NT) * 64 + (k_begin & 1) * 32; }
     auto advance = [&]() {
         if (!CONV) { cc += 32; return; }
         if (cc & 32) {
-            if (++tap == 9) { tap = 0; cc += 32; } else { cc -= 32; }
+            if (++tap == NT) { tap = 0; cc += 32; } else { cc -= 32; }
         } else {
             cc += 32;
         }
@@ -219,7 +244,7 @@
         const half_t* src = sc.s1 ? a.A1 : a.A0;
         const int Cs = sc.s1 ? a.C1 : a.C0;
         int disp = sc.s1 ? cc - a.C0 : cc;
-        const int ky = tap / 3 - 1, kx = tap - (tap / 3) * 3 - 1;
+        const int ky = PH ? pa + (tap >> 1) - 1 : tap / 3 - 1, kx = PH ? pb + (tap & 1) - 1 : tap - (tap / 3) * 3 - 1;
         sc.dyE = sc.dyO = sc.dxE = sc.dxO = 0;
         if (CONV) {
             if (!up) {
@@ -230,7 +255,7 @@
             }
         }
         sc.sbase = (const char*)src + (ptrdiff_t)disp * 2;
-        sc.wbase = (const char*)a.Wt + ((size_t)(k_begin + kn) << 6);
+        sc.wbase = (const char*)Wt + ((size_t)(k_begin + kn) << 6);
         sc.lbase = __builtin_amdgcn_readfirstlane(lds_addr(smem) + (kn & 3) * STAGE_BYTES);
         sc.tap = tap;
         return sc;
@@ -252,7 +277,7 @@
     };
     auto advance_bf = [&]() {
         if (!CONV) { cc += 32; return; }
-        const bool second = (cc & 32) != 0, wrap = second && tap == 8;
+        const bool second = (cc & 32) != 0, wrap = second && tap == NT - 1;
         cc = second ? (wrap ? cc + 32 : cc - 32) : cc + 32;
         tap = second ? (wrap ? 0 : tap + 1) : tap;
     };
@@ -273,9 +298,9 @@
     float* rv_l = bias_l + BN;
     float* mr_l = rv_l + RV_MAX * BN;
     float* u_l = mr_l + 2 * BM;
-    const int rps = a.rows_per_sample;
+    const int rps = PH ? a.H * a.W : a.rows_per_sample;
     const int smp0 = m0 / rps;
-    const int last_row = min(m0 + BM, a.M) - 1;
+    const int last_row = min(m0 + BM, Mrows) - 1;
     const int nsmp = a.rowvec ? last_row / rps - smp0 + 1 : 0;
     const bool rv_in_lds = nsmp <= RV_MAX;
     for (int c = tid; c < BN; c += T) bias_l[c] = a.bias ? a.bias[n0 + c] : 0.f;
@@ -294,6 +319,13 @@
                 rstd = (float)(1.0 / sqrt(var + (double)a.ln_eps));
             }
             mr_l[2 * r] = mean; mr_l[2 * r + 1] = rstd;
+        }
+    }
+    int* orow_l = (int*)mr_l;
+    if constexpr (PH) {
+        for (int r = tid; r < BM; r += T) {
+            const int m = min(m0 + r, Mrows - 1), ni = m / a.W, jx = m - ni * a.W;
+            orow_l[r] = (2 * ni + pa) * a.Wo + 2 * jx + pb;
         }
     }
     if (a.rowvec && rv_in_lds)
@@ -588,7 +620,7 @@
         const int i = ip * PT + hf;
         const int prow = hf * MS + lrow;
         const int row = m0 + wm * TM + ip * 32 + prow;
-        const int bsmp = (a.rowvec && row < a.M) ? row / rps : smp0;
+        const int bsmp = (a.rowvec && row < Mrows) ? row / rps : smp0;
         const float* rw = rv_l + (bsmp - smp0) * BN + wn * TN;
 #pragma unroll
         for (int j = 0; j < NI; ++j) {
@@ -605,7 +637,7 @@
                         const f32x4 rq = *(const f32x4*)(rw + wc);
 #pragma unroll
                         for (int e = 0; e < 4; ++e) v[e] += rq[e];
-                    } else if (row < a.M) {
+                    } else if (row < Mrows) {
 #pragma unroll
                         for (int e = 0; e < 4; ++e) v[e] += a.rowvec[(size_t)bsmp * a.rv_stride + n0 + wn * TN + wc + e];
                     }
@@ -633,13 +665,14 @@
                 } else if (PATH != 0 || okind == OUT_F16) {
                     h4 pk = {(half_t)v[0], (half_t)v[1], (half_t)v[2], (half_t)v[3]};
                     *(h4*)(cst + prow * PITCH + oc * 2) = pk;
-                } else if (row < a.M && ocol0 + oc < nvalid) {
+                } else if (row < Mrows && ocol0 + oc < nvalid) {
                     const int ch = ocol0 + oc;
+                    const int orow = PH ? orow_l[wm * TM + ip * 32 + prow] : row;
                     if (okind == OUT_F32) {
                         f32x4 pk = {v[0], v[1], v[2], v[3]};
-                        *(f32x4*)((float*)outp + (size_t)row * ldo + ch) = pk;
+                        *(f32x4*)((float*)outp + (size_t)orow * ldo + ch) = pk;
                     } else {
-                        const int b = row / rps, t = row - b * rps;
+                        const int b = orow / a.rows_per_sample, t = orow - b * a.rows_per_sample;
 #pragma unroll
                         for (int e = 0; e < 4; ++e) {
                             const size_t off = ((size_t)b * nvalid + ch + e) * ldo + t;
@@ -678,8 +711,9 @@
                 const int pr = c / CPR, ck = c - pr * CPR;
                 const int grow = m0 + wm * TM + ip * 32 + pr;
                 const int gcol = ocol0 + ck * 8;
-                ok[it] = c < 32 * CPR && grow < a.M && gcol < nvalid;
-                goff[it] = (size_t)grow * ldo + gcol;
+                ok[it] = c < 32 * CPR && grow < Mrows && gcol < nvalid;
+                if constexpr (PH) goff[it] = (size_t)orow_l[wm * TM + ip * 32 + (c < 32 * CPR ? pr : 0)] * ldo + gcol;
+                else goff[it] = (size_t)grow * ldo + gcol;
                 if (ok[it]) {
                     const char* sp = cst + pr * PITCH + ck * 16;
                     const h4 lo = *(const h4*)sp, hi = *(const h4*)(sp + 8);
@@ -748,12 +782,12 @@
     }
 }
 
-template <int BM, int BN, int WM, int WN, int STAGES, bool CONV, bool GEGLU, bool SPLIT, int MS, bool LN, int PATH, int PIPE, bool ABL>
+template <int BM, int BN, int WM, int WN, int STAGES, int CONV, bool GEGLU, bool SPLIT, int MS, bool LN, int PATH, int PIPE, bool ABL>
 __global__ __launch_bounds__(WM * WN * 64) void igemm2_kernel(const IgemmArgs a) {
     igemm2_body<BM, BN, WM, WN, STAGES, CONV, GEGLU, SPLIT, MS, LN, PATH, PIPE, ABL>(a);
 }
 struct IgemmArgsG { IgemmArgs g[FGDM_MAX_GROUP]; };
-template <int BM, int BN, int WM, int WN, int STAGES, bool CONV, bool GEGLU, bool SPLIT, int MS, bool LN, int PATH, int PIPE, bool ABL>
+template <int BM, int BN, int WM, int WN, int STAGES, int CONV, bool GEGLU, bool SPLIT, int MS, bool LN, int PATH, int PIPE, bool ABL>
 __global__ __launch_bounds__(WM * WN * 64) void igemm2_pair_kernel(const IgemmArgsG p) {
     igemm2_body<BM, BN, WM, WN, STAGES, CONV, GEGLU, SPLIT, MS, LN, PATH, PIPE, ABL>(p.g[blockIdx.y]);
 }
@@ -1010,21 +1044,21 @@
     return hipGetLastError() == hipSuccess ? FGDM_OK : FGDM_ERR_HIP;
 }
 
-template <int BM, int BN, int WM, int WN, int STAGES, bool CONV, bool GEGLU, bool SPLIT, int MS, bool LN, int PATH, int PIPE, bool ABL>
+template <int BM, int BN, int WM, int WN, int STAGES, int CONV, bool GEGLU, bool SPLIT, int MS, bool LN, int PATH, int PIPE, bool ABL>
 int launch2p(const IgemmArgs& a, hipStream_t s) {
     constexpr int ring = ring_bytes<BM, BN, STAGES, PIPE>();
     constexpr int smem = ring + (1 + RV_MAX) * BN * 4 + (2 * BM + BN) * 4;
     static_assert(smem <= 160 * 1024, "LDS budget");
     constexpr auto k = igemm2_kernel<BM, BN, WM, WN, STAGES, CONV, GEGLU, SPLIT, MS, LN, PATH, PIPE, ABL>;
     if (fgdm_dyn_lds<k>(smem) != FGDM_OK) return FGDM_ERR_HIP;
-    const int ntm = (a.M + BM - 1) / BM, ntn = (a.N + BN - 1) / BN;
+    const int ntm = igemm_row_tiles(a, BM), ntn = (a.N + BN - 1) / BN;
     const unsigned gx = (unsigned)(ntm * ntn * (SPLIT ? a.splitk : 1));
     if (fgdm_recording()) {
         auto single = [=](hipStream_t rs) -> int {
             hipLaunchKernelGGL(k, dim3(gx), dim3(WM * WN * 64), smem, rs, a);
             return hipGetLastError() == hipSuccess ? FGDM_OK : FGDM_ERR_HIP;
         };
-        if constexpr (PIPE != 0 && PATH != 0 && !SPLIT && !ABL && MS == 16) {
+        if constexpr (PIPE != 0 && PATH != 0 && !SPLIT && !ABL && MS == 16 && CONV != 2) {
             constexpr auto kp = igemm2_pair_kernel<BM, BN, WM, WN, STAGES, CONV, GEGLU, SPLIT, MS, LN, PATH, PIPE, ABL>;
             if (fgdm_dyn_lds<kp>(smem) != FGDM_OK) return FGDM_ERR_HIP;
             static_assert(sizeof(IgemmArgs) <= FGDM_GROUP_BLOB, "the recorded blob holds an IgemmArgs");
@@ -1054,12 +1088,13 @@
         if (!staged || a.rowvec) return 0;
     }
     if (!a.rowvec) return 1;
-    return (BM - 1) / a.rows_per_sample + 2 <= RV_MAX ? 2 : 0;
-}
-template <int BM, int BN, int WM, int WN, int STAGES, bool CONV, bool GEGLU, bool SPLIT, int MS, bool LN, bool FAST, int PIPE>
+    const int rps = a.mode == IG_CONV2_UP2P ? a.H * a.W : a.rows_per_sample;
+    return (BM - 1) / rps + 2 <= RV_MAX ? 2 : 0;
+}
+template <int BM, int BN, int WM, int WN, int STAGES, int CONV, bool GEGLU, bool SPLIT, int MS, bool LN, bool FAST, int PIPE>
 int launch2(const IgemmArgs& a, hipStream_t s) {
     const bool fast_on = knob_once(KNOB_IGEMM_EPI_PATHS) != 0;
-    if constexpr (FAST && !SPLIT && !LN) {
+    if constexpr (FAST && !SPLIT && !LN && CONV != 2) {
         if (a.debug)
             return epilogue_path<BM, GEGLU, LN>(a) == 1 ? launch2p<BM, BN, WM, WN, STAGES, CONV, GEGLU, SPLIT, MS, LN, 1, (PIPE == 2 ? 1 : PIPE), true>(a, s)
                                                         : FGDM_ERR_ARG;
@@ -1069,7 +1104,7 @@
     if constexpr (FAST && !SPLIT) {
         switch (fast_on ? epilogue_path<BM, GEGLU, LN>(a) : 0) {
             case 1: return launch2p<BM, BN, WM, WN, STAGES, CONV, GEGLU, SPLIT, MS, LN, 1, PIPE, false>(a, s);
-            case 2: if constexpr (!GEGLU && !LN) return launch2p<BM, BN, WM, WN, STAGES, CONV, GEGLU, SPLIT, MS, LN, 2, PIPE, false>(a, s);
+            case 2: if constexpr (!GEGLU && !LN && CONV != 2) return launch2p<BM, BN, WM, WN, STAGES, CONV, GEGLU, SPLIT, MS, LN, 2, PIPE, false>(a, s);
             default: break;
         }
     }
@@ -1078,12 +1113,14 @@
 template <int BM, int BN, bool GEGLU, int MS, int PIPE, int WM, int WN>
 int launch2m(const IgemmArgs& a, hipStream_t s) {
     constexpr int PL = PIPE == 2 ? 1 : PIPE;
-    return a.mode == IG_LINEAR ? launch2<BM, BN, WM, WN, 4, false, GEGLU, false, MS, false, MS == 16, PL>(a, s)
-                               : launch2<BM, BN, WM, WN, 4, true, GEGLU, false, MS, false, MS == 16, (GEGLU ? PL : PIPE)>(a, s);
+    if constexpr (!GEGLU && BM != 64) { if (a.mode == IG_CONV2_UP2P) return launch2<BM, BN, WM, WN, 4, 2, false, false, MS, false, MS == 16, PL>(a, s); }
+    if (a.mode == IG_CONV2_UP2P) return FGDM_ERR_ARG;
+    return a.mode == IG_LINEAR ? launch2<BM, BN, WM, WN, 4, 0, GEGLU, false, MS, false, MS == 16, PL>(a, s)
+                               : launch2<BM, BN, WM, WN, 4, 1, GEGLU, false, MS, false, MS == 16, (GEGLU ? PL : PIPE)>(a, s);
 }
 template <int BM, int BN, bool GEGLU, int MS, int PIPE, int WM, int WN>
 int launch2ln(const IgemmArgs& a, hipStream_t s) {
-    return launch2<BM, BN, WM, WN, 4, false, GEGLU, false, MS, true, MS == 16, (PIPE == 2 ? 1 : PIPE)>(a, s);
+    return launch2<BM, BN, WM, WN, 4, 0, GEGLU, false, MS, true, MS == 16, (PIPE == 2 ? 1 : PIPE)>(a, s);
 }
 template <int BM, int BN, int MS, int PIPE, int WM = 4, int WN = 2>
 int launch_tile(const IgemmArgs& a, hipStream_t s) {
@@ -1130,7 +1167,7 @@
 void igemm_set_twin_layers(bool on) { g_twin_layers = on; }
 
 int igemm_splitk_factor(const IgemmArgs& a) {
-    if (a.force_cfg || a.act == ACT_GEGLU || a.out_kind != OUT_F16 || a.N % 320 || (a.K & 31)) return 1;
+    if (a.force_cfg || a.mode == IG_CONV2_UP2P || a.act == ACT_GEGLU || a.out_kind != OUT_F16 || a.N % 320 || (a.K & 31)) return 1;
     const int nk = a.K >> 5;
     const bool fat = knob_once(KNOB_SPLITK_FAT) != 0;
     if (fat && a.rows_per_sample > 64 && a.rows_per_sample <= 256 && (nk >= 540 || (nk >= 360 && !g_twin_layers))) return 2;
@@ -1165,16 +1202,16 @@
         if ((tile != 2 && tile != 0) || a.ln_stats) return FGDM_ERR_ARG;
         const int nk_all = a.K >> 5;
         if (halo && nk_all % a.splitk == 0 && (nk_all / a.splitk) % 9 == 0)
-            return tile == 0 ? launch2<256, 320, 4, 2, 4, true, false, true, 16, false, false, 2>(a, s)
-                             : launch2<128, 320, 4, 2, 4, true, false, true, 16, false, false, 2>(a, s);
+            return tile == 0 ? launch2<256, 320, 4, 2, 4, 1, false, true, 16, false, false, 2>(a, s)
+                             : launch2<128, 320, 4, 2, 4, 1, false, true, 16, false, false, 2>(a, s);
         if (tile == 0 && pipe)
-            return a.mode == IG_LINEAR ? launch2<256, 320, 4, 2, 4, false, false, true, 16, false, false, 1>(a, s)
-                                       : launch2<256, 320, 4, 2, 4, true, false, true, 16, false, false, 1>(a, s);
+            return a.mode == IG_LINEAR ? launch2<256, 320, 4, 2, 4, 0, false, true, 16, false, false, 1>(a, s)
+                                       : launch2<256, 320, 4, 2, 4, 1, false, true, 16, false, false, 1>(a, s);
         if (pipe)
-            return a.mode == IG_LINEAR ? launch2<128, 320, 4, 2, 4, false, false, true, 16, false, false, 1>(a, s)
-                                       : launch2<128, 320, 4, 2, 4, true, false, true, 16, false, false, 1>(a, s);
-        return a.mode == IG_LINEAR ? launch2<128, 320, 4, 2, 4, false, false, true, 16, false, false, 0>(a, s)
-                                   : launch2<128, 320, 4, 2, 4, true, false, true, 16, false, false, 0>(a, s);
+            return a.mode == IG_LINEAR ? launch2<128, 320, 4, 2, 4, 0, false, true, 16, false, false, 1>(a, s)
+                                       : launch2<128, 320, 4, 2, 4, 1, false, true, 16, false, false, 1>(a, s);
+        return a.mode == IG_LINEAR ? launch2<128, 320, 4, 2, 4, 0, false, true, 16, false, false, 0>(a, s)
+                                   : launch2<128, 320, 4, 2, 4, 1, false, true, 16, false, false, 0>(a, s);
     }
     if (a.ln_stats && a.mode != IG_LINEAR) return FGDM_ERR_ARG;
     const int persist_mode = knob_once(KNOB_IGEMM_PERSIST);
diff --git a/fgdm_amd/csrc/knobs.h b/fgdm_amd/csrc/knobs.h
--- a/fgdm_amd/csrc/knobs.h
+++ b/fgdm_amd/csrc/knobs.h
@@ -28,6 +28,7 @@
     X(GN_REG_NG, "FGDM_GN_REG_NG", "4", "widest slice of the register-resident GroupNorm, in groups")                           \
     X(GN_FUSED_MAXKB, "FGDM_GN_FUSED_MAXKB", "64", "largest LDS slice (KB) of the single-kernel GroupNorm; 0 = always two kernels") \
     X(GN_CHUNK, "FGDM_GN_CHUNK", FGDM_STR(GN_PIX_PER_CHUNK), "pixels per partial-sum chunk of the two-kernel GroupNorm (multiples of 64)") \
+    X(UP2_PHASE, "FGDM_UP2_PHASE", "1", "fgdm_create, op / bench entries: every call; 0: Upsample convs as one 9-tap conv, not four 2x2 phases (changes bits)") \
     X(LN_FOLD, "FGDM_LN_FOLD", "1", "fgdm_create; 0: the transformer blocks' LayerNorms as kernels of their own")               \
     X(TWIN_STREAMS, "FGDM_TWIN_STREAMS", "0", "fgdm_create; 1: the ControlNets on a second stream next to the UNet encoder")    \
     X(PAIR_LAUNCH, "FGDM_PAIR_LAUNCH", "1", "fgdm_create; 0: no grouped launches of twin layers")                               \
diff --git a/fgdm_amd/csrc/ops_abi.hip b/fgdm_amd/csrc/ops_abi.hip
--- a/fgdm_amd/csrc/ops_abi.hip
+++ b/fgdm_amd/csrc/ops_abi.hip
@@ -1,4 +1,5 @@
 #include "engine_shared.h"
+#include "knobs.h"
 #include "replay_plan.h"
 
 static int op_pack(IgemmArgs& a, TmpDev& tmp, const float* w, const float* bias, int N, int K, int Ks, bool geglu,
@@ -74,6 +75,26 @@
         if (ksize != 3 || C1 || x1 || upsample || (stride != 1 && stride != 2)) return FGDM_ERR_ARG;
         return op_conv3_im2col((const half_t*)x0, C0, w, bias, rowvec, (const half_t*)resid, B, H, W, Cout, stride, act, scale, out, s);
     }
+    const bool up2p = ksize == 3 && upsample && knob_on(KNOB_UP2_PHASE);
+    if (up2p) {
+        if (x1 || C1 || resid || stride != 1) return FGDM_ERR_ARG;
+        std::vector<float> wh((size_t)Cout * Cin * 9), bh(igemm_npad(Cout), 0.f);
+        if (hipMemcpy(wh.data(), w, wh.size() * sizeof(float), hipMemcpyDefault) != hipSuccess) return FGDM_ERR_HIP;
+        if (bias && hipMemcpy(bh.data(), bias, Cout * sizeof(float), hipMemcpyDefault) != hipSuccess) return FGDM_ERR_HIP;
+        TmpDev tmp;
+        IgemmArgs a{};
+        a.Wt = tmp.up(up2_phase_pack(wh.data(), Cout, Cin)); a.bias = tmp.up(bh); a.zero = g_zero_page();
+        if (!a.Wt || !a.bias || !a.zero) return FGDM_ERR_NOMEM;
+        a.A0 = (const half_t*)x0; a.C0 = C0;
+        a.rowvec = rowvec; a.rv_stride = Cout;
+        a.B = B; a.H = H; a.W = W; a.Ho = 2 * H; a.Wo = 2 * W; a.mode = IG_CONV2_UP2P;
+        a.M = B * a.Ho * a.Wo; a.N = Cout; a.K = 4 * Cin;
+        a.act = act; a.out_kind = OUT_F16; a.out = out; a.ld_out = Cout;
+        a.rows_per_sample = a.Ho * a.Wo; a.scale = scale;
+        const int rc = igemm_launch(a, s);
+        (void)hipStreamSynchronize(s);
+        return rc;
+    }
     std::vector<int> kmap(K);
     for (int tap = 0; tap < taps; ++tap)
         for (int c = 0; c < Cin; ++c) kmap[taps == 9 ? ((c >> 6) * 9 + tap) * 64 + (c & 63) : c] = c * taps + tap;
```

Measured after the change: 8.026, median of 2. Within noise of the previous version (-0.0%).
